# muzishen/IMAGDressing

Hardware: AMD Instinct MI355X
Metric: 512x512 50-step images/sec (whole node) (higher is better)
Workload: dtype bf16

## Files before the change

imagdressing_amd/_lib.py:

```python
from __future__ import annotations

import ctypes as C
import os

_HERE = os.path.dirname(os.path.abspath(__file__))
LIB_PATH = os.environ.get("IMD_LIB_PATH") or os.path.join(_HERE, "libimagdressing_hip.so")

ABI_VERSION = 9

u16p = C.POINTER(C.c_uint16)
f32p = C.POINTER(C.c_float)


class _Sized(C.Structure):

    def __init__(self, *args, **kw):
        super().__init__(*args, **kw)
        self.struct_bytes = C.sizeof(self)


class HeadsDest(C.Structure):
    _fields_ = [("ptr", C.c_void_p), ("kind", C.c_int), ("DP", C.c_int), ("L", C.c_int), ("scale", C.c_float)]


class ConvGemmParams(_Sized):
    _fields_ = [("struct_bytes", C.c_uint32), 
        ("x", C.c_void_p), ("w", C.c_void_p), ("out", C.c_void_p),
        ("M", C.c_int), ("N", C.c_int), ("K", C.c_int),
        ("Cin", C.c_int), ("taps", C.c_int), ("Hin", C.c_int), ("Win", C.c_int), ("Hout", C.c_int),
        ("Wout", C.c_int), ("stride", C.c_int), ("ups", C.c_int),
        ("x_pix_stride", C.c_int), ("out_ld", C.c_int), ("res_ld", C.c_int),
        ("bias", C.c_void_p), ("rowvec", C.c_void_p), ("rowvec_stride", C.c_int),
        ("res", C.c_void_p), ("out_scale", C.c_float), ("act", C.c_int), ("out_f32", C.c_int),
        ("mode", C.c_int), ("hC", C.c_int), ("hH", C.c_int), ("hD", C.c_int),
        ("hd", HeadsDest * 3), ("dtype", C.c_int), ("split_k", C.c_int), ("splitk_ws", C.c_void_p),
        ("x_bytes", C.c_uint32), ("w_bytes", C.c_uint32), ("flags", C.c_int),
        ("gn_a", C.c_void_p), ("gn_b", C.c_void_p), ("gn_silu", C.c_int), ("pad_br_only", C.c_int),
        ("splitk_counters", C.c_void_p),
        ("gn_stats_out", C.c_void_p), ("gn_stats_groups", C.c_int),
        ("gn_in_partial", C.c_void_p), ("gn_in_gamma", C.c_void_p), ("gn_in_beta", C.c_void_p),
        ("gn_in_nparts", C.c_int), ("gn_in_groups", C.c_int), ("gn_in_silu", C.c_int), ("gn_in_eps", C.c_float),
        ("gn_out_gamma", C.c_void_p), ("gn_out_beta", C.c_void_p), ("gn_out_eps", C.c_float), ("gn_out_silu", C.c_int), ("gn_out_groups", C.c_int), ("res_rows", C.c_int),
    ]


class FfParams(_Sized):
    _fields_ = [("struct_bytes", C.c_uint32), ("x", C.c_void_p), ("w1", C.c_void_p), ("b1", C.c_void_p), ("w2", C.c_void_p), ("b2", C.c_void_p), ("out", C.c_void_p),
                ("M", C.c_int), ("C", C.c_int), ("inner", C.c_int), ("x_ld", C.c_int), ("out_ld", C.c_int), ("ln", C.c_int),
                ("ln_eps", C.c_float), ("dtype", C.c_int)]


class XattnParams(_Sized):
    _fields_ = [("struct_bytes", C.c_uint32), ("x", C.c_void_p), ("w", C.c_void_p), ("bq", C.c_void_p), ("bo", C.c_void_p), ("kv", C.c_void_p),
                ("out", C.c_void_p), ("M", C.c_int), ("C", C.c_int), ("heads", C.c_int), ("L", C.c_int), ("rows_per_image", C.c_int),
                ("kv_bdiv", C.c_int), ("text_rows", C.c_int), ("x_ld", C.c_int), ("out_ld", C.c_int), ("q_scale", C.c_float),
                ("ln_eps", C.c_float), ("dtype", C.c_int)]


class AttnParams(_Sized):
    _fields_ = [("struct_bytes", C.c_uint32), 
        ("q", C.c_void_p), ("k1", C.c_void_p), ("v1t", C.c_void_p), ("k2", C.c_void_p), ("v2t", C.c_void_p),
        ("scale2", C.c_void_p), ("out", C.c_void_p),
        ("B", C.c_int), ("H", C.c_int), ("N", C.c_int), ("D", C.c_int),
        ("L1", C.c_int), ("L1P", C.c_int), ("kv1_bdiv", C.c_int),
        ("L2", C.c_int), ("L2P", C.c_int), ("kv2_bdiv", C.c_int),
        ("out_ld", C.c_int), ("dtype", C.c_int), ("flags", C.c_int), ("causal", C.c_int), ("k_pad_one", C.c_int),
        ("proj_w", C.c_void_p), ("proj_b", C.c_void_p), ("proj_res", C.c_void_p), ("proj_out", C.c_void_p),
        ("proj_res_ld", C.c_int), ("proj_out_ld", C.c_int), ("proj_counters", C.c_void_p),
        ("out_dup", C.c_void_p), ("phase2_out", C.c_void_p), ("phase2_rows", C.c_int),
    ]


class GroupNormParams(_Sized):
    _fields_ = [("struct_bytes", C.c_uint32), 
        ("x", C.c_void_p), ("y", C.c_void_p), ("gamma", C.c_void_p), ("beta", C.c_void_p), ("partial", C.c_void_p),
# ... 31 lines not shown
        ("z_n", C.c_float), ("b_img", C.c_float), ("b_noise", C.c_float), ("in_scale", C.c_float),
        ("store", C.c_int),
        ("noise", C.c_void_p), ("mask", C.c_void_p), ("z_img", C.c_void_p), ("blend_noise", C.c_void_p),
        ("coefs", C.c_void_p),
    ]


SYMBOLS = {
    "imd_abi_version": (C.c_int, []),
    "imd_last_error": (C.c_char_p, []),
    "imd_device_check": (C.c_int, [C.c_int]),
    "imd_conv_gemm": (C.c_int, [C.POINTER(ConvGemmParams), C.c_int, C.c_void_p]),
    "imd_conv_gemm_auto_cfg": (C.c_int, [C.c_int, C.c_int]),
    "imd_conv_gemm_auto_split": (C.c_int, [C.c_int, C.c_int, C.c_int, C.c_int]),
    "imd_attention": (C.c_int, [C.POINTER(AttnParams), C.c_void_p]),
    "imd_attention_dup_supported": (C.c_int, [C.c_int, C.c_int, C.c_int]),
    "imd_attention_phase_split_supported": (C.c_int, [C.c_int]),
    "imd_attention_fp8": (C.c_int, [C.POINTER(AttnParams), C.c_int, C.c_int, C.c_int, C.c_void_p]),
    "imd_attn_quantize_fp8": (C.c_int, [C.c_void_p, C.c_void_p, C.c_int, C.c_long, C.c_int, C.c_int, C.c_float, C.c_int, C.c_void_p]),
    "imd_set_tuning": (C.c_int, [C.c_int, C.c_int]),
    "imd_get_tuning": (C.c_int, [C.c_int]),
    "imd_attn_padded_dims": (C.c_int, [C.c_int, C.POINTER(C.c_int), C.POINTER(C.c_int)]),
    "imd_groupnorm": (C.c_int, [C.POINTER(GroupNormParams), C.c_void_p]),
    "imd_groupnorm_coeffs": (C.c_int, [C.POINTER(GroupNormParams), C.c_void_p, C.c_void_p, C.c_void_p]),
    "imd_conv_patch_supported": (C.c_int, [C.POINTER(ConvGemmParams)]),
    "imd_conv_patch2_supported": (C.c_int, [C.POINTER(ConvGemmParams)]),
    "imd_conv_patch3_supported": (C.c_int, [C.POINTER(ConvGemmParams)]),
    "imd_conv_patch4_supported": (C.c_int, [C.POINTER(ConvGemmParams)]),
    "imd_conv_img_supported": (C.c_int, [C.POINTER(ConvGemmParams)]),
    "imd_conv_patch_stats_parts": (C.c_int, [C.POINTER(ConvGemmParams)]),
    "imd_conv_gemm_stats_parts": (C.c_int, [C.POINTER(ConvGemmParams), C.c_int]),
    "imd_conv_gemm_gn_out_supported": (C.c_int, [C.POINTER(ConvGemmParams)]),
    "imd_row_linear_gn_in_supported": (C.c_int, [C.POINTER(ConvGemmParams), C.c_int]),
    "imd_gemm_dma_supported": (C.c_int, [C.POINTER(ConvGemmParams)]),
    "imd_row_linear": (C.c_int, [C.POINTER(ConvGemmParams), C.c_int, C.c_float, C.c_void_p]),
    "imd_row_linear_supported": (C.c_int, [C.POINTER(ConvGemmParams)]),
    "imd_ff_geglu": (C.c_int, [C.POINTER(FfParams), C.c_void_p]),
    "imd_text_xattn320": (C.c_int, [C.POINTER(XattnParams), C.c_void_p]),
    "imd_text_xattn320_supported": (C.c_int, [C.POINTER(XattnParams)]),
    "imd_conv_ups_phase": (C.c_int, [C.POINTER(ConvGemmParams), C.c_void_p]),
    "imd_conv_ups_phase_supported": (C.c_int, [C.POINTER(ConvGemmParams)]),
    "imd_groupnorm_workspace_floats": (C.c_int, [C.c_int, C.c_int, C.c_int, C.c_int]),
    "imd_layernorm": (C.c_int, [C.POINTER(LayerNormParams), C.c_void_p]),
    "imd_softmax_rows": (C.c_int, [C.c_void_p, C.c_int, C.c_void_p, C.c_int, C.c_int, C.c_int, C.c_int, C.c_void_p]),
    "imd_ddim_cfg_step": (C.c_int, [C.POINTER(DdimParams), C.c_void_p]),
    "imd_ddim_cfg_step_rows": (C.c_int, [C.POINTER(DdimParams), C.c_void_p, C.c_void_p]),
    "imd_sampler_step": (C.c_int, [C.POINTER(SamplerParams), C.c_void_p]),
    "imd_timestep_embedding": (C.c_int, [C.c_void_p, C.c_void_p, C.c_int, C.c_int, C.c_void_p]),
    "imd_add": (C.c_int, [C.c_void_p, C.c_int, C.c_void_p, C.c_int, C.c_void_p, C.c_int, C.c_long, C.c_int, C.c_float, C.c_int, C.c_void_p]),
    "imd_embed_tokens": (C.c_int, [C.c_void_p, C.c_int, C.c_void_p, C.c_int, C.c_void_p, C.c_void_p, C.c_long, C.c_int, C.c_int, C.c_void_p]),
    "imd_vit_assemble": (C.c_int, [C.c_void_p, C.c_void_p, C.c_void_p, C.c_void_p, C.c_int, C.c_int, C.c_int, C.c_int, C.c_void_p]),
    "imd_lincomb": (C.c_int, [C.POINTER(C.c_void_p), C.POINTER(C.c_float), C.c_int, C.c_void_p, C.c_long, C.c_void_p]),
    "imd_copy2d": (C.c_int, [C.c_void_p, C.c_int, C.c_void_p, C.c_int, C.c_long, C.c_int, C.c_void_p]),
    "imd_concat2": (C.c_int, [C.c_void_p, C.c_int, C.c_void_p, C.c_int, C.c_void_p, C.c_void_p, C.c_long, C.c_long, C.c_int, C.c_void_p]),
    "imd_concat2_gn_stats": (C.c_int, [C.c_void_p, C.c_int, C.c_void_p, C.c_int, C.c_void_p, C.c_void_p, C.c_int, C.c_int, C.c_int, C.c_int,
                                       C.c_void_p, C.c_int, C.c_void_p]),
    "imd_groupnorm_parts": (C.c_int, [C.c_int, C.c_int, C.c_int]),
    "imd_f32_to_16": (C.c_int, [C.c_void_p, C.c_void_p, C.c_long, C.c_int, C.c_void_p]),
}

_lib = None


class ImdError(RuntimeError):
    pass

# ... 22 lines not shown
```

imagdressing_amd/adapter/attention_processor.py:

```python
from __future__ import annotations

import math
from typing import Dict, Optional, Tuple

import torch
import torch.nn as nn

from .. import ops

bf16 = torch.bfloat16
LOG2E = math.log2(math.e)


class LoRALinearLayer(nn.Module):

    def __init__(self, in_features, out_features, rank=4, network_alpha=None):
        super().__init__()
        self.down = nn.Linear(in_features, rank, bias=False)
        self.up = nn.Linear(rank, out_features, bias=False)
        self.network_alpha = network_alpha
        self.rank = rank
        nn.init.normal_(self.down.weight, std=1 / rank)
        nn.init.zeros_(self.up.weight)

# ... 34 lines not shown
_16BIT = (torch.bfloat16, torch.float16)


def _compute_dtype(attn, hidden_states: torch.Tensor, attention_mask=None):
    if attention_mask is not None:
        raise NotImplementedError("attention_mask is always None on the IMAGDressing path (SURVEY appendix 3); masks are not implemented")
    if getattr(attn, "spatial_norm", None) is not None or getattr(attn, "group_norm", None) is not None \
            or getattr(attn, "norm_cross", None):
        raise NotImplementedError("attn.spatial_norm / group_norm / norm_cross are None for every SD1.5 attention layer; "
                                  "modules that set them are not supported by the fused processors")
    wd = attn.to_q.weight.dtype
    if wd in _16BIT:
        return wd
    return hidden_states.dtype if hidden_states.dtype in _16BIT else torch.float16


def _layer_weights(attn, which: str, dtype, device) -> torch.Tensor:
    mods = [attn.to_out[0] if n == "to_out" else getattr(attn, n) for n in _W_PARTS[which]]
    srcs = [m.bias if which == "bo" else m.weight for m in mods]
    if srcs[0] is None:
        return None
    want = torch.float32 if which == "bo" else dtype
    if len(srcs) == 1 and srcs[0].dtype == want and srcs[0].device == device and srcs[0].is_contiguous():
        return srcs[0].detach()
    cache = attn.__dict__.setdefault("_imd_wcache", {})
    key = (_version_key(*srcs), want, str(device))
    ent = cache.get(which)
    if ent is None or ent[0] != key or not all(a is b for a, b in zip(ent[1], srcs)):
        t = torch.cat([t.detach().to(device=device, dtype=want) for t in srcs], 0).contiguous()
        ent = cache[which] = (key, tuple(srcs), t)
    return ent[2]


def _ln_folded_q(attn, gamma: torch.Tensor, beta: torch.Tensor, dtype, device, which: str = "q"):
    mods = [getattr(attn, n) for n in _W_PARTS[which]]
    srcs = tuple(m.weight for m in mods) + (gamma, beta)
    cache = attn.__dict__.setdefault("_imd_wcache", {})
    key = (_version_key(*srcs), dtype, str(device))
    ent = cache.get(which + "_ln")
    if ent is None or ent[0] != key or not all(a is b for a, b in zip(ent[1], srcs)):
        w = torch.cat([m.weight.detach().to(device=device, dtype=dtype) for m in mods], 0)
        ent = cache[which + "_ln"] = (key, srcs, ops.fold_layernorm_affine(w, None, gamma.to(device), beta.to(device)))
    return ent[2]


def _qkv_ln_ok(x: torch.Tensor) -> bool:
    return x.shape[-1] == 320 and x.shape[1] % 128 == 0 and ops.FUSED_LN


FUSED_LN_CHANNELS = (320, 640, 1280)


def _as_tokens(hidden_states: torch.Tensor, dtype):
    shape4 = None
    if hidden_states.dim() == 4:
        b, c, h, w = hidden_states.shape
        shape4 = (b, c, h, w)
        hidden_states = hidden_states.view(b, c, h * w).transpose(1, 2)
    if not hidden_states.is_cuda:
        from .._lib import ImdError
        raise ImdError("imagdressing_amd processors run on MI355X only: hidden_states is on " + str(hidden_states.device))
    return hidden_states.to(dtype).contiguous(), shape4


def _restore(out, shape4, like):
    if shape4 is not None:
        b, c, h, w = shape4
        out = out.transpose(-1, -2).reshape(b, c, h, w)
    return out


def _project_kv(tokens: torch.Tensor, wkv: torch.Tensor, heads: int):
    Bk, Lk, Kd = tokens.shape
    Cc = wkv.shape[0] // 2
    D = Cc // heads
    dpk, dpv = ops.attn_padded_dims(D)
    LP = ops.pad64(Lk)
    k = ops.k_buffer((Bk, heads, Lk, dpk), D, wkv.dtype, tokens.device)
    vt = torch.zeros(Bk, heads, dpv, LP, dtype=wkv.dtype, device=tokens.device)
    ops.conv_gemm(tokens.view(Bk * Lk, Kd), wkv, M=Bk * Lk, N=2 * Cc, Cin=Kd, Hin=Lk, Win=1, Hout=Lk, Wout=1,
                  heads=dict(C=Cc, H=heads, D=D, dests=[(k, 0, dpk, Lk, 1.0), (vt, 1, dpv, LP, 1.0)]))
    return k, vt, Lk, LP


_FP8_KV: Dict[int, tuple] = {}
ops._clear_hooks.append(_FP8_KV.clear)


def _fp8_kv(kv, cache: bool):
    k, vt = kv[0], kv[1]
    e = ops.FP8_EXPS
    if cache:
        hit = _FP8_KV.get(id(k))
        if hit is not None and hit[0] is k and hit[1] == (e["q"], e["k"], e["v"]):
            return hit[2], hit[3]
    k8 = ops.quantize_fp8_rows(k, e["k"], pad_val=float(2 ** (e["q"] + e["k"])))
    v8 = ops.quantize_fp8_vt(vt, e["v"])
    if cache:
        if len(_FP8_KV) > 64:
            _FP8_KV.clear()
        _FP8_KV[id(k)] = (k, (e["q"], e["k"], e["v"]), k8, v8)
    return k8, v8


def _fused_attention(x: torch.Tensor, heads: int, *, wq_or_qkv: torch.Tensor, self_attn: bool,
                     kv1=None, kv1_bdiv: int = 1, kv2=None, kv2_bdiv: int = 1, scale2: Optional[torch.Tensor] = None,
                     wo: torch.Tensor, bo: Optional[torch.Tensor], residual: Optional[torch.Tensor],
                     q_ln: Optional[tuple] = None, pair_half: bool = False, phase2_rows: int = 0) -> torch.Tensor:
    B, N, Cc = x.shape
    D = Cc // heads
    dpk, dpv = ops.attn_padded_dims(D)
    dev, dt = x.device, x.dtype
    qscale = D ** -0.5 * LOG2E
    if (ops.FUSED_XATTN and not self_attn and q_ln is not None and kv1 is not None and kv2 is None and not pair_half
            and ops.text_xattn_supported(Cc, heads, N, kv1[2]) and not ops.ATTN_FP8 and not ops.FUSED_OUT_PROJ
            and residual is not None and residual.data_ptr() == x.data_ptr() and residual.shape == x.shape
            and residual.dtype == dt and residual.is_contiguous()):
        return ops.text_xattn(x, ops.pack_text_xattn(q_ln[0], q_ln[1], wo, bo), ops.pack_text_kv(kv1[0], kv1[1], kv1[2]),
                              Lk=kv1[2], kv_bdiv=kv1_bdiv, ln_eps=q_ln[2], q_scale=qscale)
    q = ops.workspace("attn_q", (B, heads, N, dpk), dt, dev)
    x2 = x.view(B * N, Cc)
    if self_attn:
        LP = ops.pad64(N)
        k = ops.k_buffer((B, heads, N, dpk), D, dt, dev, tag="attn_k")
        vt = ops.workspace("attn_vt", (B, heads, dpv, LP), dt, dev)
        dests = dict(C=Cc, H=heads, D=D, dests=[(q, 0, dpk, N, qscale), (k, 0, dpk, N, 1.0), (vt, 1, dpv, LP, 1.0)])
        if q_ln is not None:
            ops.conv_gemm(x2, q_ln[0], M=B * N, N=3 * Cc, Cin=Cc, Hin=N, Win=1, Hout=N, Wout=1, bias=q_ln[1], ln_eps=q_ln[2], heads=dests)
        else:
            ops.conv_gemm(x2, wq_or_qkv, M=B * N, N=3 * Cc, Cin=Cc, Hin=N, Win=1, Hout=N, Wout=1, heads=dests)
        kv1, kv1_bdiv = (k, vt, N, LP), 1
    elif q_ln is not None:
        ops.conv_gemm(x2, q_ln[0], M=B * N, N=Cc, Cin=Cc, Hin=N, Win=1, Hout=N, Wout=1, bias=q_ln[1], ln_eps=q_ln[2],
                      heads=dict(C=Cc, H=heads, D=D, dests=[(q, 0, dpk, N, qscale)]))
    else:
        ops.conv_gemm(x2, wq_or_qkv, M=B * N, N=Cc, Cin=Cc, Hin=N, Win=1, Hout=N, Wout=1,
                      heads=dict(C=Cc, H=heads, D=D, dests=[(q, 0, dpk, N, qscale)]))
    o = torch.empty(B, N, Cc, dtype=dt, device=dev)
    if ops.ATTN_FP8 and D == 40:
        e = ops.FP8_EXPS
        q8 = ops.quantize_fp8_rows(q, e["q"])
        k18, v18 = _fp8_kv(kv1, cache=not self_attn)
        kw = {}
        if kv2 is not None and scale2 is not None:
            k28, v28 = _fp8_kv(kv2, cache=True)
            kw = dict(k2=k28, v2t=v28, L2=kv2[2], L2P=kv2[3], kv2_bdiv=kv2_bdiv, scale2=scale2)
        ops.attention_fp8(q8, k18, v18, o, B=B, H=heads, N=N, L1=kv1[2], L1P=kv1[3], kv1_bdiv=kv1_bdiv, **kw)
        res2 = None if residual is None else residual.view(B * N, Cc)
        return ops.linear(o.view(B * N, Cc), wo, bo, res=res2).view(B, N, Cc)
    kw = {}
    if kv2 is not None and scale2 is not None:
        kw = dict(k2=kv2[0], v2t=kv2[1], L2=kv2[2], L2P=kv2[3], kv2_bdiv=kv2_bdiv, scale2=scale2)
    if ops.FUSED_OUT_PROJ and ops.attention_proj_supported(heads, N, D):
        out = torch.empty(B, N, Cc, dtype=dt, device=dev)
        return ops.attention(q, kv1[0], kv1[1], o, B=B, H=heads, N=N, D=D, L1=kv1[2], L1P=kv1[3], kv1_bdiv=kv1_bdiv, k_pad_one=True,
                             proj=(wo, bo, residual, out), **kw)
    if pair_half:
        o = torch.empty(2 * B, N, Cc, dtype=dt, device=dev)
        ops.attention(q, kv1[0], kv1[1], o[:B], B=B, H=heads, N=N, D=D, L1=kv1[2], L1P=kv1[3], kv1_bdiv=kv1_bdiv, k_pad_one=True,
                      out_dup=o[B:], **kw)
        res2 = None if residual is None else residual.reshape(-1, Cc)
        return ops.linear(o.view(2 * B * N, Cc), wo, bo, res=res2).view(2 * B, N, Cc)
    ops.attention(q, kv1[0], kv1[1], o, B=B, H=heads, N=N, D=D, L1=kv1[2], L1P=kv1[3], kv1_bdiv=kv1_bdiv, k_pad_one=True, phase2_rows=phase2_rows if kw else 0, **kw)
    res2 = None if residual is None else residual.view(B * N, Cc)
    return ops.linear(o.view(B * N, Cc), wo, bo, res=res2).view(B, N, Cc)


class _FusedBase:
    fused_residual = True

    @staticmethod
    def _ehs_bdiv(B: int, ehs: torch.Tensor) -> int:
        Be = ehs.shape[0]
        if B % Be:
            raise ValueError(f"encoder_hidden_states batch {Be} does not divide hidden_states batch {B}")
        return B // Be

    @staticmethod
    def _finish(attn, out, residual_given, like, shape4, ln_fused=False):
        if getattr(attn, "residual_connection", False) and not residual_given:
            if ln_fused:
                raise NotImplementedError("attn.residual_connection together with the engine's fused LayerNorm (imd_layernorm)")
            out = ops.add(out, _as_tokens(like, out.dtype)[0])
        if getattr(attn, "rescale_output_factor", 1.0) != 1.0:
            raise NotImplementedError("rescale_output_factor != 1 is not used by SD1.5")
        out = _restore(out, shape4, like)
        return out if out.dtype == like.dtype else out.to(like.dtype)


class AttnProcessor2_0(_FusedBase):

    fused_layernorm = True

    def __init__(self, cache_entries: int = 256):
        self._text = _TensorCache(capacity=cache_entries)

    def __call__(self, attn, hidden_states, encoder_hidden_states=None, attention_mask=None, temb=None, scale=1.0,
                 imd_residual=None, imd_layernorm=None, **kwargs):
        dt = _compute_dtype(attn, hidden_states, attention_mask)
        x, shape4 = _as_tokens(hidden_states, dt)
        dev = x.device
        wo, bo = _layer_weights(attn, "o", dt, dev), _layer_weights(attn, "bo", dt, dev)
        q_ln = None
        if imd_layernorm is not None:
            g, be, eps = imd_layernorm
            if encoder_hidden_states is not None and x.shape[-1] in FUSED_LN_CHANNELS:
                q_ln = _ln_folded_q(attn, g, be, dt, dev) + (eps,)
            elif encoder_hidden_states is None and _qkv_ln_ok(x):
                q_ln = _ln_folded_q(attn, g, be, dt, dev, "qkv") + (eps,)
            else:
                x = ops.layer_norm(x, g, be, eps)
        if encoder_hidden_states is None:
            out = _fused_attention(x, attn.heads, wq_or_qkv=_layer_weights(attn, "qkv", dt, dev), self_attn=True, wo=wo, bo=bo,
                                   residual=imd_residual, q_ln=q_ln)
        else:
            srcs = (encoder_hidden_states, attn.to_k.weight, attn.to_v.weight)
            kv = self._text.get(srcs, extra=(dt,))
            if kv is None:
                e = encoder_hidden_states.to(device=dev, dtype=dt).contiguous()
                kv = self._text.put(srcs, _project_kv(e, _layer_weights(attn, "kv", dt, dev), attn.heads), extra=(dt,))
            out = _fused_attention(x, attn.heads, wq_or_qkv=_layer_weights(attn, "q", dt, dev), self_attn=False, kv1=kv,
                                   kv1_bdiv=self._ehs_bdiv(x.shape[0], encoder_hidden_states), wo=wo, bo=bo,
                                   residual=imd_residual, q_ln=q_ln)
        return self._finish(attn, out, imd_residual is not None, hidden_states, shape4, ln_fused=imd_layernorm is not None)


class CacheAttnProcessor2_0(AttnProcessor2_0):
    fused_layernorm = False

    def __init__(self):
        super().__init__()
        self.cache = {}

    def __call__(self, attn, hidden_states, encoder_hidden_states=None, attention_mask=None, temb=None, scale=1.0,
                 **kwargs):
        self.cache["hidden_states"] = hidden_states
        return super().__call__(attn, hidden_states, encoder_hidden_states=encoder_hidden_states, **kwargs)


class _RefMixin:

    def _init_ref(self, name, hidden_size, cross_attention_dim, scale):
        self.name = name
        self.hidden_size = hidden_size
        self.cross_attention_dim = cross_attention_dim
        self.to_k_ref = nn.Linear(cross_attention_dim or hidden_size, hidden_size, bias=False)
        self.to_v_ref = nn.Linear(cross_attention_dim or hidden_size, hidden_size, bias=False)
        self.scale = scale
        self._wref = _TensorCache()
        self._garment = _TensorCache()
        self._scale2 = _TensorCache()
        self._scale2_plain: Dict = {}

    def _garment_kv(self, ref: torch.Tensor, heads: int, device, dtype):
        wsrc = (self.to_k_ref.weight, self.to_v_ref.weight)
        kv = self._garment.get((ref,) + wsrc, extra=(dtype,))
        if kv is None:
            w = self._wref.get(wsrc, extra=(dtype,))
            if w is None:
                w = self._wref.put(wsrc, torch.cat([t.detach().to(device=device, dtype=dtype) for t in wsrc], 0).contiguous(),
                                   extra=(dtype,))
            r = ref.detach().to(device=device, dtype=dtype).contiguous()
            if r.dim() != 3:
                raise ValueError(f"sa_hidden_states[{self.name!r}] must be [Bg, M, C], got {tuple(ref.shape)}")
            kv = self._garment.put((ref,) + wsrc, _project_kv(r, w, heads), extra=(dtype,))
        return kv

    def _garment_bdiv(self, B: int, ref: torch.Tensor) -> int:
        Bg = ref.shape[0]
        if Bg < 1 or B % Bg:
            raise ValueError(f"sa_hidden_states[{self.name!r}] has batch {Bg}, which does not divide hidden_states batch {B}")
        return B // Bg

    def _branch_weights(self, B: int, mask: Optional[torch.Tensor], device) -> torch.Tensor:
        s = float(self.scale)
        if mask is None:
            t = self._scale2_plain.get((B, s, str(device)))
            if t is None:
                t = torch.full((B,), s, dtype=torch.float32, device=device)
                self._scale2_plain = {(B, s, str(device)): t}
            return t
        t = self._scale2.get((mask,), extra=(s,))
        if t is None:
            t = self._scale2.put((mask,), (mask.to(device=device, dtype=torch.float32) * s).contiguous(), extra=(s,))
        return t


class RefSAttnProcessor2_0(nn.Module, _FusedBase, _RefMixin):
    fused_layernorm = True
    fused_pair_half = True

    def __init__(self, name, hidden_size, cross_attention_dim=None, scale=1.0):
        super().__init__()
        self._init_ref(name, hidden_size, cross_attention_dim, scale)

    def _weights(self, attn, dt, dev):
        return _layer_weights(attn, "qkv", dt, dev), _layer_weights(attn, "o", dt, dev), _layer_weights(attn, "bo", dt, dev)

    def __call__(self, attn, hidden_states, encoder_hidden_states=None, attention_mask=None, temb=None, scale=1.0,
                 num_images_per_prompt=1, cond_hidden_states=None, sa_hidden_states=None, sa_batch_mask=None,
                 imd_residual=None, imd_layernorm=None, imd_pair_half=False, **kwargs):
        if encoder_hidden_states is not None:
            raise NotImplementedError(f"{type(self).__name__} is a self-attention (attn1) processor")
        dt = _compute_dtype(attn, hidden_states, attention_mask)
        x, shape4 = _as_tokens(hidden_states, dt)
        wqkv, wo, bo = self._weights(attn, dt, x.device)
        q_ln = None
        if imd_layernorm is not None:
            g, be, eps = imd_layernorm
            if _qkv_ln_ok(x):
                q_ln = _ln_folded_q(attn, g, be, dt, x.device, "qkv") + (eps,)
            else:
                x = ops.layer_norm(x, g, be, eps)
        kv2 = s2 = None
        bdiv2 = 1
        if sa_hidden_states is not None:
            ref = sa_hidden_states[self.name]
            kv2 = self._garment_kv(ref, attn.heads, x.device, x.dtype)
            cond_rows = x.shape[0] // 2 if (kwargs.get("sa_pair_layout") and not imd_pair_half and x.shape[0] % 2 == 0) else x.shape[0]
            bdiv2 = self._garment_bdiv(cond_rows, ref)
            s2 = self._branch_weights(x.shape[0] * (2 if imd_pair_half else 1), sa_batch_mask, x.device)
        if imd_pair_half and (kv2 is None or imd_residual is None or shape4 is not None):
            raise ValueError("imd_pair_half needs sa_hidden_states, the block residual and token-major hidden states (engine-internal)")
        pr = x.shape[0] // 2 if (kwargs.get("sa_pair_layout") and sa_batch_mask is not None and kv2 is not None and not imd_pair_half and x.shape[0] % 2 == 0) else 0
        out = _fused_attention(x, attn.heads, wq_or_qkv=wqkv, self_attn=True, kv2=kv2, kv2_bdiv=bdiv2,
                               scale2=s2, wo=wo, bo=bo, residual=imd_residual, q_ln=q_ln, pair_half=bool(imd_pair_half), phase2_rows=pr)
        return self._finish(attn, out, imd_residual is not None, hidden_states, shape4, ln_fused=imd_layernorm is not None)


class _LoraFold:

    def _init_lora(self, hidden_size, kdim, rank, network_alpha, lora_scale):
        self.rank = rank
        self.lora_scale = lora_scale
        self.to_q_lora = LoRALinearLayer(hidden_size, hidden_size, rank, network_alpha)
        self.to_k_lora = LoRALinearLayer(kdim, hidden_size, rank, network_alpha)
        self.to_v_lora = LoRALinearLayer(kdim, hidden_size, rank, network_alpha)
        self.to_out_lora = LoRALinearLayer(hidden_size, hidden_size, rank, network_alpha)
        self._folded = _TensorCache()

    def _fold(self, attn, device, dtype):
        ls = float(self.lora_scale)
        srcs = tuple(l.weight for lo in (self.to_q_lora, self.to_k_lora, self.to_v_lora, self.to_out_lora)
                     for l in (lo.down, lo.up)) + (attn.to_q.weight, attn.to_k.weight, attn.to_v.weight, attn.to_out[0].weight)
        w = self._folded.get(srcs, extra=(ls, dtype, str(device)))
        if w is None:
            def eff(base, lora):
                base = base.detach().to(device)
                if ls == 0.0:
                    return base.to(dtype).contiguous()
                return (base.float() + ls * lora.delta().to(device)).to(dtype).contiguous()
            wq, wk, wv = eff(attn.to_q.weight, self.to_q_lora), eff(attn.to_k.weight, self.to_k_lora), eff(attn.to_v.weight, self.to_v_lora)
            wo = eff(attn.to_out[0].weight, self.to_out_lora)
            w = self._folded.put(srcs, dict(q=wq, kv=torch.cat([wk, wv], 0).contiguous(),
                                            qkv=(torch.cat([wq, wk, wv], 0).contiguous() if wk.shape[1] == wq.shape[1] else None),
                                            o=wo), extra=(ls, dtype, str(device)))
        return w


# ... 1 lines not shown

    def __init__(self, name, hidden_size, cross_attention_dim=None, scale=1.0, rank=128, network_alpha=None, lora_scale=1.0):
        super().__init__()
        self._init_ref(name, hidden_size, cross_attention_dim, scale)
        self._init_lora(hidden_size, cross_attention_dim or hidden_size, rank, network_alpha, lora_scale)

    def _weights(self, attn, dt, dev):
        w = self._fold(attn, dev, dt)
        return w["qkv"], w["o"], _layer_weights(attn, "bo", dt, dev)

    __call__ = RefSAttnProcessor2_0.__call__
    fused_pair_half = True


class LoraRefSAttnProcessor2_0(_LoraRefSBase):
    """attention_processor.py:391-511 (used by inference_IMAGdressing_ipa_controlnetpose.py:88-94)."""


class RefLoraSAttnProcessor2_0(_LoraRefSBase):
    """Same arithmetic under the name ``app.py:90`` uses (attention_processor.py:1006-1128).  As in the
    reference, ``pipe.set_scale`` does not match this class (it checks LoraRefSAttnProcessor2_0)."""


class CAttnProcessor2_0(nn.Module, _FusedBase):

    def __init__(self, name, hidden_size, cross_attention_dim=None):
        super().__init__()
        self.name = name
        self.hidden_size = hidden_size
        self.cross_attention_dim = cross_attention_dim
        self._plain = AttnProcessor2_0(cache_entries=4)

    fused_layernorm = True

    def __call__(self, attn, hidden_states, encoder_hidden_states=None, attention_mask=None, temb=None, scale=1.0,
                 cond_hidden_states=None, sa_hidden_states=None, imd_residual=None, imd_layernorm=None, **kwargs):
        return self._plain(attn, hidden_states, encoder_hidden_states=encoder_hidden_states, imd_residual=imd_residual,
                           imd_layernorm=imd_layernorm)


class _IPBase(nn.Module, _FusedBase, _LoraFold):

    def __init__(self, hidden_size, cross_attention_dim=None, rank=4, network_alpha=None, lora_scale=1.0, scale=1.0,
                 num_tokens=4):
        super().__init__()
        self.num_tokens = num_tokens
        self.hidden_size = hidden_size
        self.cross_attention_dim = cross_attention_dim
        self.scale = scale
        self._init_lora(hidden_size, cross_attention_dim or hidden_size, rank, network_alpha, lora_scale)
        self.to_k_ip = nn.Linear(cross_attention_dim or hidden_size, hidden_size, bias=False)
        self.to_v_ip = nn.Linear(cross_attention_dim or hidden_size, hidden_size, bias=False)
        self._kv = _TensorCache()
        self._wip = _TensorCache()
        self._s2: Dict = {}

    def _weights(self, attn, dt, dev):
        w = self._fold(attn, dev, dt)
        return w["q"], w["kv"], w["o"]

    def __call__(self, attn, hidden_states, encoder_hidden_states=None, attention_mask=None, scale=1.0, temb=None,
                 *args, imd_residual=None, **kwargs):
        if encoder_hidden_states is None:
            raise NotImplementedError(f"{type(self).__name__} is a cross-attention (attn2) processor")
        dt = _compute_dtype(attn, hidden_states, attention_mask)
        x, shape4 = _as_tokens(hidden_states, dt)
        wq, wkv, wo = self._weights(attn, dt, x.device)
        wsrc = (self.to_k_ip.weight, self.to_v_ip.weight)
        ls = float(getattr(self, "lora_scale", 0.0))
        ksrc = (encoder_hidden_states, attn.to_k.weight, attn.to_v.weight) + wsrc
        kvs = self._kv.get(ksrc, extra=(ls, x.dtype))
# ... 132 lines not shown
```

imagdressing_amd/csrc/capi.cpp:

```cpp
#include <atomic>
#include <mutex>
#include <stdarg.h>
#include <stdio.h>
#include <string.h>

#include "imd_kernels.h"

namespace {
thread_local char g_err[512] = "";
}

int imd_set_error(const char* fmt, ...) {
    va_list ap;
    va_start(ap, fmt);
    vsnprintf(g_err, sizeof(g_err), fmt, ap);
    va_end(ap);
    return 1;
}

int imd_check_launch(const char* what) {
    hipError_t e = hipGetLastError();
    if (e != hipSuccess) return imd_set_error("%s: launch failed: %s", what, hipGetErrorString(e));
    return 0;
}
// ... 134 lines not shown
    if (dpv) *dpv = imd_attn_dpv(D);
    return 0;
}

int imd_groupnorm(const imd_groupnorm_params* p, void* stream) {
    IMD_REQUIRE(p != nullptr, "groupnorm: null params");
    IMD_REQUIRE_SIZE(p, "groupnorm");
    IMD_REQUIRE(p->x && p->y && p->gamma && p->beta && p->partial, "groupnorm: null pointer");
    return imd_launch_groupnorm(*p, (hipStream_t)stream);
}

int imd_groupnorm_coeffs(const imd_groupnorm_params* p, float* coef_a, float* coef_b, void* stream) {
    IMD_REQUIRE(p != nullptr, "groupnorm_coeffs: null params");
    IMD_REQUIRE_SIZE(p, "groupnorm_coeffs");
    IMD_REQUIRE(p->x && p->gamma && p->beta && p->partial && coef_a && coef_b, "groupnorm_coeffs: null pointer");
    return imd_launch_groupnorm_coeffs(*p, coef_a, coef_b, (hipStream_t)stream);
}

static bool sized(const imd_conv_gemm_params* p) { return p && p->struct_bytes == sizeof(*p); }
static int query(const imd_conv_gemm_params* p, bool (*pred)(const imd_conv_gemm_params&)) {
    if (!sized(p)) return 0;
    imd_conv_gemm_params q = *p;
    if (!imd_conv_gemm_fill_extents(q)) return 0;
    return pred(q) ? 1 : 0;
}
int imd_conv_patch_supported(const imd_conv_gemm_params* p) { return query(p, static_cast<bool (*)(const imd_conv_gemm_params&)>(imd_conv_patch_supported)); }
int imd_conv_patch2_supported(const imd_conv_gemm_params* p) { return query(p, static_cast<bool (*)(const imd_conv_gemm_params&)>(imd_conv_patch2_supported)); }
int imd_conv_patch3_supported(const imd_conv_gemm_params* p) { return query(p, static_cast<bool (*)(const imd_conv_gemm_params&)>(imd_conv_patch3_supported)); }
int imd_conv_patch4_supported(const imd_conv_gemm_params* p) { return query(p, static_cast<bool (*)(const imd_conv_gemm_params&)>(imd_conv_patch4_supported)); }
int imd_conv_img_supported(const imd_conv_gemm_params* p) { return query(p, static_cast<bool (*)(const imd_conv_gemm_params&)>(imd_conv_img_supported)); }
int imd_conv_patch_stats_parts(const imd_conv_gemm_params* p) { return sized(p) ? imd_conv_patch_stats_parts_of(*p) : 0; }
int imd_conv_gemm_stats_parts(const imd_conv_gemm_params* p, int cfg) { return sized(p) ? imd_conv_gemm_stats_parts_of(*p, cfg) : 0; }
int imd_row_linear_gn_in_supported(const imd_conv_gemm_params* p, int cfg) { return (sized(p) && p->gn_in_partial != nullptr && imd_row_linear_gn_in_supported_of(*p, cfg)) ? 1 : 0; }
int imd_conv_gemm_gn_out_supported(const imd_conv_gemm_params* p) { return (sized(p) && imd_conv_gemm_gn_out_supported_of(*p, -1)) ? 1 : 0; }
int imd_gemm_dma_supported(const imd_conv_gemm_params* p) { return query(p, static_cast<bool (*)(const imd_conv_gemm_params&)>(imd_gemm_dma_supported)); }

int imd_row_linear_supported(const imd_conv_gemm_params* p) { return (sized(p) && (imd_row_linear_supported(*p) || imd_row_linear_k640_supported(*p) || imd_row_linear_k1280_supported(*p) || imd_row_qkv_supported(*p))) ? 1 : 0; }

int imd_row_linear(const imd_conv_gemm_params* p, int ln, float ln_eps, void* stream) {
    IMD_REQUIRE(p != nullptr, "row_linear: null params");
    IMD_REQUIRE_SIZE(p, "row_linear");
    IMD_REQUIRE(p->x && p->w, "row_linear: null input/weight pointer");
    IMD_REQUIRE(p->mode == IMD_OUT_HEADS || p->out != nullptr, "row_linear: null output pointer");
    IMD_REQUIRE(p->Hout > 0 && p->Wout > 0 && p->M > 0 && p->M % (p->Hout * p->Wout) == 0, "row_linear: bad geometry");
    if (p->mode == IMD_OUT_HEADS) {
        IMD_REQUIRE(p->hC > 0 && p->hH > 0 && p->hD > 0 && p->hC == p->hH * p->hD && p->N % p->hC == 0 && p->N / p->hC <= 3 && p->hD % 8 == 0,
                    "row_linear: bad head split C=%d H=%d D=%d", p->hC, p->hH, p->hD);
        IMD_REQUIRE(!p->out_f32, "row_linear: head-split output excludes fp32 output");
    }
    IMD_REQUIRE(!ln || ln_eps > 0.f, "row_linear: LayerNorm needs eps > 0");
    if (p->K == 320 && p->N == 960 && p->mode == IMD_OUT_HEADS) {
        IMD_REQUIRE(p->gn_in_partial == nullptr, "row_linear: the fused q / k / v projection has no GroupNorm prologue (gn_in_*)");
        return imd_launch_row_qkv(*p, ln, ln_eps, (hipStream_t)stream);
    }
    if (p->K == 640) return imd_launch_row_linear_k640(*p, ln, ln_eps, (hipStream_t)stream);
    if (p->K == 1280) return imd_launch_row_linear_k1280(*p, ln, ln_eps, (hipStream_t)stream);
    return imd_launch_row_linear(*p, ln, ln_eps, (hipStream_t)stream);
}

int imd_ff_geglu(const imd_ff_params* p, void* stream) {
    IMD_REQUIRE(p != nullptr, "ff_geglu: null params");
    IMD_REQUIRE_SIZE(p, "ff_geglu");
    IMD_REQUIRE(p->x && p->w1 && p->b1 && p->w2 && p->b2 && p->out, "ff_geglu: null pointer");
    IMD_REQUIRE(!p->ln || p->ln_eps > 0.f, "ff_geglu: LayerNorm needs eps > 0");
    return imd_launch_ff_geglu(*p, (hipStream_t)stream);
}

int imd_text_xattn320_supported(const imd_xattn_params* p) {
    return (p && p->struct_bytes == sizeof(*p) && imd_text_xattn320_supported_of(*p)) ? 1 : 0;
}

int imd_text_xattn320(const imd_xattn_params* p, void* stream) {
    IMD_REQUIRE(p != nullptr, "text_xattn320: null params");
    IMD_REQUIRE_SIZE(p, "text_xattn320");
    IMD_REQUIRE(p->x && p->w && p->bq && p->bo && p->kv && p->out, "text_xattn320: null pointer");
    return imd_launch_text_xattn320(*p, (hipStream_t)stream);
}

int imd_conv_ups_phase_supported(const imd_conv_gemm_params* p) { return (sized(p) && imd_conv_ups_phase_supported_of(*p)) ? 1 : 0; }

int imd_conv_ups_phase(const imd_conv_gemm_params* p, void* stream) {
    IMD_REQUIRE(p != nullptr, "conv_ups_phase: null params");
    IMD_REQUIRE_SIZE(p, "conv_ups_phase");
    IMD_REQUIRE(p->x && p->w && p->out, "conv_ups_phase: null input / weight / output pointer");
    return imd_launch_conv_ups_phase(*p, (hipStream_t)stream);
}

int imd_layernorm(const imd_layernorm_params* p, void* stream) {
    IMD_REQUIRE(p != nullptr, "layernorm: null params");
    IMD_REQUIRE_SIZE(p, "layernorm");
    IMD_REQUIRE(p->x && p->y && p->gamma && p->beta, "layernorm: null pointer");
    return imd_launch_layernorm(*p, (hipStream_t)stream);
}

int imd_embed_tokens(const uint16_t* table, int vocab, const uint16_t* pos, int T, const int64_t* ids, uint16_t* out, long rows, int C,
                     int dtype, void* stream) {
    IMD_REQUIRE(table && pos && ids && out, "embed_tokens: null pointer");
    return imd_launch_embed_tokens(table, vocab, pos, T, ids, out, rows, C, dtype, (hipStream_t)stream);
}

int imd_vit_assemble(const uint16_t* patches, const uint16_t* cls, const uint16_t* pos, uint16_t* out, int B, int P, int C, int dtype,
                     void* stream) {
    IMD_REQUIRE(patches && cls && pos && out, "vit_assemble: null pointer");
    return imd_launch_vit_assemble(patches, cls, pos, out, B, P, C, dtype, (hipStream_t)stream);
}

int imd_lincomb(const float* const* xs, const float* coefs, int n, float* out, long numel, void* stream) {
    IMD_REQUIRE(xs && coefs && out, "lincomb: null pointer");
    return imd_launch_lincomb(xs, coefs, n, out, numel, (hipStream_t)stream);
}

int imd_softmax_rows(const float* s, int s_ld, uint16_t* p, int p_ld, int rows, int cols, int dtype, void* stream) {
    IMD_REQUIRE(s && p, "softmax_rows: null pointer");
    return imd_launch_softmax_rows(s, s_ld, p, p_ld, rows, cols, dtype, (hipStream_t)stream);
}

int imd_ddim_cfg_step(const imd_ddim_params* p, void* stream) {
// ... 57 lines not shown
```

imagdressing_amd/csrc/conv_gemm.hip:

```cpp
#include "gemm_common.h"

namespace {

template <int BM, int BN, int BK, int WAVES_M> struct TileCfg {
    static constexpr int STRIDE = BK * 2 + 16;
    static constexpr int MAIN = 2 * (BM + BN) * STRIDE;
    static constexpr int CLD = BN + 4;
    static constexpr int EROWS = BM / WAVES_M;
    static constexpr int EPI = EROWS * CLD * 4;
    static constexpr int LDS = MAIN > EPI ? MAIN : EPI;
};

template <bool F16, int BM, int BN, int BK, int WAVES_M, int WAVES_N, int DEPTH>
__global__ __launch_bounds__(WAVES_M * WAVES_N * 64, (WAVES_M * WAVES_N == 4) ? 2 : 1) void conv_gemm_kernel(const ConvGemmParams p) {
    constexpr int NT = WAVES_M * WAVES_N * 64;
    using E = El<F16>;
    using T = TileCfg<BM, BN, BK, WAVES_M>;
    constexpr int TM = BM / WAVES_M / 32;
    constexpr int TN = BN / WAVES_N / 32;
    constexpr int STRIDE = T::STRIDE;
    constexpr int VPR = BK / 8;
    constexpr int RSTEP = NT / VPR;
    constexpr int A_VECS = BM / RSTEP;
    constexpr int W_VECS = BN / RSTEP;
// ... 568 lines not shown
    ConvGemmParams p = p_in;
    if (p.split_k < 1) p.split_k = 1;
    if (cfg < 0) cfg = imd_conv_gemm_choose_cfg(p.M, p.N);
    const TileConfig* t = tile_config(cfg);
    if (p.split_k > 1) {
        if (t != nullptr && t->finish_always) p.splitk_counters = nullptr;
        return splitk_stats_parts_of(p);
    }
    switch (t != nullptr ? t->stats : ST_NONE) {
        case ST_PATCH3_W4: return imd_conv_patch3_stats_parts_of(p, 4);
        case ST_PATCH3_W8: return imd_conv_patch3_stats_parts_of(p, 8);
        case ST_PATCH: return imd_conv_patch_stats_parts_of(p);
        case ST_TILE: {
            const int HW = p.Hout * p.Wout, G = p.gn_stats_groups;
            if (p.out_f32 || p.mode != OUT_ROWMAJOR || p.act == ACT_GEGLU || G <= 0 || G > 64 || p.N % G || (p.N / G) < 8 || (p.N % 4) || HW <= 0 || HW % t->bm || p.M % HW) return 0;
            return (HW / t->bm) * ((p.N + t->bn - 1) / t->bn);
        }
        default: return 0;
    }
}

bool imd_row_linear_gn_in_supported_of(const ConvGemmParams& p, int cfg) {
    if (p.gn_in_partial == nullptr) return true;
    ConvGemmParams q = p;
    q.split_k = 1;
    switch (cfg) {
        case 12: return imd_row_linear_supported(q) && gn_in_ok(q, 320, 128);
        case 13: return imd_row_linear_k640_supported(q) && gn_in_ok(q, 640, 128);
        case 14: return imd_row_linear_k1280_supported(q) && gn_in_ok(q, 1280, 64);
        default: return false;
    }
}

bool imd_conv_gemm_gn_out_supported_of(const ConvGemmParams& p_in, int cfg) {
    ConvGemmParams p = p_in;
    (void)cfg;
    p.splitk_counters = nullptr;
    return splitk_gn_out_supported(p);
}

int imd_conv_gemm_choose_cfg(int M, int N) {
    const long b128 = (long)((M + 127) / 128) * ((N + 127) / 128);
    if (b128 < 96) return 2;
    if (N <= 64) return 1;
    if (b128 >= 700) return 4;
    return 0;
}

int imd_conv_gemm_choose_split(int M, int N, int K, int cfg) {
    int bm = 128, bn = 128;
    tile_dims(cfg, &bm, &bn);
    const long blocks = (long)((M + bm - 1) / bm) * ((N + bn - 1) / bn);
    const int ktiles = (K + 63) / 64;
    if (blocks >= 200 || ktiles < 32) return 1;
    long s = (448 + blocks - 1) / blocks;
    if (s > ktiles / 16) s = ktiles / 16;
    if (s > 8) s = 8;
    return s < 1 ? 1 : (int)s;
}

bool imd_conv_gemm_fill_extents(ConvGemmParams& p) {
    if (p.Hout <= 0 || p.Wout <= 0 || p.M <= 0) return false;
    const size_t npix = (size_t)(p.M / (p.Hout * p.Wout)) * p.Hin * p.Win;
    if (npix == 0) return false;
    const size_t xb = ((npix - 1) * (size_t)p.x_pix_stride + p.Cin) * 2, wb = (size_t)p.N * p.K * 2;
    if (xb >= 0xffffffffull || wb >= 0xffffffffull) return false;
// ... 32 lines not shown
    }
#ifdef IMD_ABLATIONS
    p.flags |= gf & 224;
#endif
    if (p.split_k <= 1 || (t != nullptr && t->finish_always)) p.splitk_counters = nullptr;
    if (p.gn_stats_out != nullptr && imd_conv_gemm_stats_parts_of(p, cfg) == 0)
        return imd_set_error("conv_gemm: gn_stats_out needs tile config 5 / 22 / 23 / 29 or a register-staged tile (0..4, 7) with H W %% its rows == 0, without K slices, or any K-sliced launch with a separate finish; a row-major 16-bit "
                             "output and 1 <= groups <= 64 with N %% groups == 0 and N / groups >= 8 (got cfg=%d split_k=%d groups=%d N=%d); ask "
                             "imd_conv_gemm_stats_parts() first", cfg, p.split_k, p.gn_stats_groups, p.N);
    if (p.gn_out_gamma != nullptr && !imd_conv_gemm_gn_out_supported_of(p, cfg))
        return imd_set_error("conv_gemm: gn_out_* needs K slices with a separate finish launch, a row-major 16-bit output without residual / activation / scale / "
                             "gn_stats_out, 4 | N / groups and H W N / groups <= %d (got cfg=%d split_k=%d groups=%d N=%d); ask imd_conv_gemm_gn_out_supported() first",
                             4 * FG_THREADS * FG_MAXU, cfg, p.split_k, p.gn_out_groups, p.N);
    if (p.gn_out_gamma != nullptr) p.splitk_counters = nullptr;
    if (p.splitk_counters != nullptr) {
        int bm = 128, bn = 128;
        tile_dims(cfg, &bm, &bn);
        const long tiles = (t != nullptr && t->stats == ST_PATCH) ? (long)(p.M / (p.Hout * p.Wout)) * ((p.Hout + 7) / 8) * ((p.Wout + 15) / 16) * ((p.N + 127) / 128)
                                                                  : (long)((p.M + bm - 1) / bm) * ((p.N + bn - 1) / bn);
        if (tiles > IMD_SPLITK_COUNTERS || (size_t)p.M * p.N * 4 >= 0x80000000ull) p.splitk_counters = nullptr;
    }
    if (p.split_k > 1) {
        if (p.mode == OUT_HEADS || p.act == ACT_GEGLU) return imd_set_error("conv_gemm: split-K supports row-major epilogues only");
        if (!p.splitk_ws) return imd_set_error("conv_gemm: split_k = %d needs a workspace", p.split_k);
    }
    if (p.dtype != IMD_DTYPE_BF16 && p.dtype != IMD_DTYPE_F16) return imd_set_error("conv_gemm: unknown dtype %d", p.dtype);
    if ((p.gn_a != nullptr) != (p.gn_b != nullptr)) return imd_set_error("conv_gemm: gn_a and gn_b must be given together");
    if (p.gn_a != nullptr && cfg != 5) return imd_set_error("conv_gemm: the fused GroupNorm prologue needs tile config 5 (got %d)", cfg);
    if (p.res_rows != 0 && cfg != 12)
        return imd_set_error("conv_gemm: a periodic residual (res_rows = %d) exists in the K = 320 row-resident projection only (tile config 12, got %d)", p.res_rows, cfg);
    if (p.gn_in_partial != nullptr && !imd_row_linear_gn_in_supported_of(p, cfg))
        return imd_set_error("conv_gemm: gn_in_* (GroupNorm of the input rows) exists in the row-resident projections only (tile configs 12 / 13 / 14 with H W a multiple of "
                             "their row block; got cfg=%d K=%d HW=%d): ask imd_row_linear_gn_in_supported() first", cfg, p.K, p.Hout * p.Wout);
    if (t == nullptr) return imd_set_error("conv_gemm: unknown tile config %d", cfg);
    if (t->taps != 0 && t->taps != p.taps) return imd_set_error("conv_gemm: tile config %d does not take taps = %d", cfg, p.taps);
    if (t->slices_only && p.split_k <= 1) return imd_set_error("conv_gemm: tile config %d writes K-slice slabs only (split_k >= 2)", cfg);
    const int rc = t->launch(p, s);
    if (rc || p.split_k <= 1 || p.splitk_counters != nullptr) return rc;
    return launch_splitk_finish(p, s, t->finish);
}
```

imagdressing_amd/csrc/gemm_common.h:

```cpp
#pragma once
#include "common.h"
#include "imd_kernels.h"

namespace {

typedef __attribute__((__vector_size__(4 * sizeof(uint32_t)))) uint32_t v4u;

__device__ __forceinline__ uint4 buf_load16(const __amdgpu_buffer_rsrc_t& rs, uint32_t byte_off) {
    const v4u v = __builtin_amdgcn_raw_buffer_load_b128(rs, (int)byte_off, 0, 0);
    return make_uint4(v[0], v[1], v[2], v[3]);
}
__device__ __forceinline__ uint2 buf_load8(const __amdgpu_buffer_rsrc_t& rs, uint32_t byte_off) {
    typedef __attribute__((__vector_size__(2 * sizeof(uint32_t)))) uint32_t v2u;
    const v2u v = __builtin_amdgcn_raw_buffer_load_b64(rs, (int)byte_off, 0, 0);
    return make_uint2(v[0], v[1]);
}
__device__ __forceinline__ uint4 buf_load16_nl1(const __amdgpu_buffer_rsrc_t& rs, uint32_t byte_off) {
    const v4u v = __builtin_amdgcn_raw_buffer_load_b128(rs, (int)byte_off, 0, 16);
    return make_uint4(v[0], v[1], v[2], v[3]);
}

constexpr uint32_t OOB = 0xffffffffu;

__device__ __forceinline__ void xcd_tile_order(int flags, int m_tiles, int n_tiles, int& tile_m, int& tile_n) {
// ... 92 lines not shown
            const int g = c / cpg;
            const float ga = r.gam[i] * s_rstd[g];
            s_a[c] = ga;
            s_sh[c] = r.bet[i] - s_mean[g] * ga;
        }
    }
    __syncthreads();
    a = s_a; sh = s_sh;
}

template <bool F16>
__device__ __forceinline__ uint4 gn_in_apply8(const uint4& raw, const float* a, const float* sh, int k0, bool silu) {
    const float4 a0 = *reinterpret_cast<const float4*>(a + k0), a1 = *reinterpret_cast<const float4*>(a + k0 + 4);
    const float4 s0 = *reinterpret_cast<const float4*>(sh + k0), s1 = *reinterpret_cast<const float4*>(sh + k0 + 4);
    const float av[8] = {a0.x, a0.y, a0.z, a0.w, a1.x, a1.y, a1.z, a1.w}, sv[8] = {s0.x, s0.y, s0.z, s0.w, s1.x, s1.y, s1.z, s1.w};
    float f[8];
    unpack8<F16>(raw, f);
#pragma unroll
    for (int e = 0; e < 8; ++e) {
        float y = f[e] * av[e] + sv[e];
        if (silu) y = silu_f(y);
        f[e] = y;
    }
    return pack8<F16>(f);
}

inline bool gn_in_ok(const ConvGemmParams& p, int K, int rows) {
    if (p.gn_in_partial == nullptr) return true;
    const int HW = p.Hout * p.Wout;
    return p.mode == OUT_ROWMAJOR && p.res == nullptr && p.gn_in_gamma != nullptr && p.gn_in_beta != nullptr && p.gn_in_groups > 0 && p.gn_in_groups <= 64 && (K % p.gn_in_groups) == 0 &&
           p.gn_in_nparts > 0 && p.gn_in_nparts <= 4096 && HW > 0 && (HW % rows) == 0 && (p.M % HW) == 0 && p.K == K;
}

__device__ __forceinline__ void load_col_addends(const ConvGemmParams& p, int bi, int n, int nv, float4& a0, float4& a1) {
    a0 = make_float4(0, 0, 0, 0); a1 = a0;
    const bool full = nv == 8;
    if (p.bias) {
        a0 = *reinterpret_cast<const float4*>(p.bias + n);
        if (full) a1 = *reinterpret_cast<const float4*>(p.bias + n + 4);
    }
    if (p.rowvec && bi >= 0) {
        const float* rv = p.rowvec + (size_t)bi * p.rowvec_stride + n;
        const float4 r0 = *reinterpret_cast<const float4*>(rv);
        a0.x += r0.x; a0.y += r0.y; a0.z += r0.z; a0.w += r0.w;
        if (full) { const float4 r1 = *reinterpret_cast<const float4*>(rv + 4); a1.x += r1.x; a1.y += r1.y; a1.z += r1.z; a1.w += r1.w; }
    }
}

template <bool F16>
__device__ __forceinline__ void epilogue8(const ConvGemmParams& p, float* v, int m, int n, int nv, int HWo, bool use_pre = false,
                                          float4 pre0 = float4{0, 0, 0, 0}, float4 pre1 = float4{0, 0, 0, 0}, bool use_rpre = false,
                                          uint4 rpre = uint4{0, 0, 0, 0}, uint4* pk_out = nullptr) {
    using E = El<F16>;
    const int bi = m / HWo;
    float4 b0 = make_float4(0, 0, 0, 0), b1 = b0, r0 = b0, r1 = b0;
    uint4 rr = make_uint4(0, 0, 0, 0);
    const bool full = nv == 8;
    if (use_pre) { b0 = pre0; b1 = pre1; }
    else load_col_addends(p, bi, n, nv, b0, b1);
    if (p.res) {
        if (use_rpre) rr = rpre;
        else {
            const bf16_t* rp = p.res + (size_t)m * p.res_ld + n;
            if (full) rr = *reinterpret_cast<const uint4*>(rp);
            else { const uint2 t = *reinterpret_cast<const uint2*>(rp); rr.x = t.x; rr.y = t.y; }
        }
    }
    v[0] += b0.x + r0.x; v[1] += b0.y + r0.y; v[2] += b0.z + r0.z; v[3] += b0.w + r0.w;
    v[4] += b1.x + r1.x; v[5] += b1.y + r1.y; v[6] += b1.z + r1.z; v[7] += b1.w + r1.w;
    if (p.out_scale != 1.0f) {
#pragma unroll
        for (int e = 0; e < 8; ++e) v[e] *= p.out_scale;
    }
    if (p.res) {
        float f[8];
        unpack8<F16>(rr, f);
#pragma unroll
        for (int e = 0; e < 8; ++e) v[e] += f[e];
    }
    if (p.act == ACT_SILU) {
#pragma unroll
        for (int e = 0; e < 8; ++e) v[e] = silu_f(v[e]);
    } else if (p.act == ACT_GELU) {
#pragma unroll
        for (int e = 0; e < 8; ++e) v[e] = gelu_erf_f(v[e]);
    } else if (p.act == ACT_QUICK_GELU) {
#pragma unroll
// ... 91 lines not shown
```

imagdressing_amd/csrc/gemm_dma.hip:

```cpp
#include "gemm_common.h"
#include "lds_dma.h"

namespace {

constexpr int GD_BM = 256, GD_BN = 256, GD_BK = 64;
constexpr int GD_ROWB = GD_BK * 2;
constexpr int GD_A = GD_BM * GD_ROWB, GD_W = GD_BN * GD_ROWB, GD_STAGE = GD_A + GD_W;
constexpr int GD_LDS = 2 * GD_STAGE;
constexpr int GD_CLD = GD_BN + 4, GD_EROWS = 64;

template <bool F16>
__global__ __launch_bounds__(512, 1) void gemm_dma_kernel(const ConvGemmParams p) {
    using E = El<F16>;
    extern __shared__ __attribute__((aligned(16))) char smem[];
    const int tid = threadIdx.x;
    const int lane = tid & 63;
    const int wave = __builtin_amdgcn_readfirstlane(tid >> 6);
    const int hi = lane >> 5, col = lane & 31;
    const int wm0 = (wave >> 1) * 64, wn0 = (wave & 1) * 128;

    const int n_tiles = (p.N + GD_BN - 1) / GD_BN;
    int tile_m, tile_n;
    xcd_tile_order(p.flags, (p.M + GD_BM - 1) / GD_BM, n_tiles, tile_m, tile_n);
    const int m0 = tile_m * GD_BM, n0 = tile_n * GD_BN;
    const int nk = p.K / GD_BK;

    const v4i_t ds_x = raw_rsrc(p.x, p.x_bytes), ds_w = raw_rsrc(p.w, p.w_bytes);
    uint32_t soff[8];
#pragma unroll
    for (int j = 0; j < 8; ++j) {
        const int id = j * 8 + wave;
        const bool isw = j >= 4;
        const int q = (id & 31) * 64 + lane;
        const int row = q >> 3, pos = q & 7;
        const int pc = pos ^ ((row >> 1) & 7);
        if (isw) soff[j] = (n0 + row < p.N) ? (uint32_t)(((size_t)(n0 + row) * p.K + pc * 8) * 2) : OOB;
        else soff[j] = (m0 + row < p.M) ? (uint32_t)(((size_t)(m0 + row) * p.x_pix_stride + pc * 8) * 2) : OOB;
    }
    const uint32_t lds0 = (uint32_t)(uintptr_t)smem;
    auto stage = [&](int kt) {
        const uint32_t base = lds0 + (uint32_t)((kt & 1) * GD_STAGE);
#pragma unroll
        for (int j = 0; j < 8; ++j) {
            const int id = j * 8 + wave;
// ... 45 lines not shown
    float4 col_pre0 = make_float4(0, 0, 0, 0), col_pre1 = col_pre0;
    bool use_col_pre = false;
    if (!colmajor && (p.bias || p.rowvec)) {
        const int bi_lo = m0 / HWo, bi_hi = (min(m0 + GD_BM, p.M) - 1) / HWo;
        const int n = n0 + (tid % CPR) * 8;
        if ((p.rowvec == nullptr || bi_lo == bi_hi) && n < p.N) {
            load_col_addends(p, p.rowvec ? bi_lo : -1, n, (n + 8 <= p.N) ? 8 : 4, col_pre0, col_pre1);
            use_col_pre = true;
        }
    }
#pragma unroll 1
    for (int wr = 0; wr < 4; ++wr) {
        if ((wave >> 1) == wr) {
#pragma unroll
            for (int b = 0; b < 2; ++b)
#pragma unroll
                for (int a = 0; a < 4; ++a)
#pragma unroll
                    for (int j = 0; j < 4; ++j) {
                        float* dst = Cs + (b * 32 + col) * GD_CLD + wn0 + a * 32 + 8 * j + 4 * hi;
                        *reinterpret_cast<float4*>(dst) = make_float4(acc[a][b][4 * j], acc[a][b][4 * j + 1], acc[a][b][4 * j + 2], acc[a][b][4 * j + 3]);
                    }
        }
        __syncthreads();
        for (int c = tid; c < CHUNKS; c += 512) {
            int row, cc;
            if (colmajor) { cc = (c / GD_EROWS) * 8; row = c - (c / GD_EROWS) * GD_EROWS; }
            else { row = c / CPR; cc = (c - row * CPR) * 8; }
            const int m = m0 + wr * GD_EROWS + row, n = n0 + cc;
            if (m >= p.M || n >= p.N) continue;
            const float4 v0 = *reinterpret_cast<const float4*>(Cs + row * GD_CLD + cc);
            const float4 v1 = *reinterpret_cast<const float4*>(Cs + row * GD_CLD + cc + 4);
            float v[8] = {v0.x, v0.y, v0.z, v0.w, v1.x, v1.y, v1.z, v1.w};
            epilogue8<F16>(p, v, m, n, (n + 8 <= p.N) ? 8 : 4, HWo, use_col_pre, col_pre0, col_pre1);
        }
        if (wr + 1 < 4) __syncthreads();
    }
}

constexpr int G1_BM = 128, G1_BN = 128, G1_BK = 32;
constexpr int G1_STAGE = (G1_BM + G1_BN) * G1_BK * 2;
constexpr int G1_CLD = G1_BN + 4, G1_EROWS = 64;
static_assert(3 * G1_STAGE >= G1_EROWS * G1_CLD * 4, "epilogue tile must fit");

template <bool F16, bool GATHER, int G1_NST, int BK = 32>
__global__ __launch_bounds__(256, (G1_NST * (G1_BM + G1_BN) * BK * 2 <= 49152) ? 3 : (G1_NST * (G1_BM + G1_BN) * BK * 2 <= 65536) ? 2 : 1)
void gemm_dma128_kernel(const ConvGemmParams p) {
    using E = El<F16>;
    constexpr int ROWB = BK * 2, LPR = ROWB / 16;
    constexpr int STAGE = (G1_BM + G1_BN) * ROWB;
    constexpr int PPW = G1_BM * ROWB / 1024 / 4;
    constexpr int NP = 2 * PPW;
    constexpr int G1_KEEP = (G1_NST - 2) * NP;
    extern __shared__ __attribute__((aligned(16))) char smem[];
    const int tid = threadIdx.x;
    const int lane = tid & 63;
    const int wave = __builtin_amdgcn_readfirstlane(tid >> 6);
    const int hi = lane >> 5, col = lane & 31;
    const int wm0 = (wave >> 1) * 64, wn0 = (wave & 1) * 64;

    const int n_tiles = (p.N + G1_BN - 1) / G1_BN;
    int tile_m, tile_n;
    xcd_tile_order(p.flags, (p.M + G1_BM - 1) / G1_BM, n_tiles, tile_m, tile_n);
    const int m0 = tile_m * G1_BM, n0 = tile_n * G1_BN;
    const int nk_total = p.K / BK;
    const int per = (nk_total + p.split_k - 1) / p.split_k;
    const int kt0 = blockIdx.y * per;
// ... 134 lines not shown
            const float4 v1 = *reinterpret_cast<const float4*>(Cs + row * G1_CLD + cc + 4);
            if (slab) {
                slab_store8(slab, (size_t)m * p.N + n, v0, v1, n + 8 <= p.N, false);
            } else {
                float v[8] = {v0.x, v0.y, v0.z, v0.w, v1.x, v1.y, v1.z, v1.w};
                epilogue8<F16>(p, v, m, n, (n + 8 <= p.N) ? 8 : 4, HWo, use_col_pre, col_pre0, col_pre1);
            }
        }
        if (wr == 0) __syncthreads();
    }
}

}

bool imd_conv_dma_supported(const ConvGemmParams& p) {
    return p.taps == 9 && (p.stride == 1 || p.stride == 2) && (p.Cin % G1_BK) == 0 && p.K == 9 * p.Cin && p.gn_a == nullptr &&
           (p.x_pix_stride % 8) == 0 && (!p.ups || p.stride == 1);
}

template <bool GATHER, int NST, int BK = 32>
static int launch_dma128(const ConvGemmParams& p, hipStream_t s, const char* what) {
    constexpr int LDS = NST * (G1_BM + G1_BN) * BK * 2;
    static_assert(LDS >= G1_EROWS * G1_CLD * 4, "epilogue tile must fit");
    const bool h = p.dtype == IMD_DTYPE_F16;
    typedef void (*kern_t)(const ConvGemmParams);
    const kern_t kern = h ? gemm_dma128_kernel<true, GATHER, NST, BK> : gemm_dma128_kernel<false, GATHER, NST, BK>;
    if (int rc_attr = imd_lds_attr(reinterpret_cast<const void*>(kern), LDS, what)) return rc_attr;
    const long mt = (p.M + G1_BM - 1) / G1_BM, nt = (p.N + G1_BN - 1) / G1_BN;
    hipLaunchKernelGGL(kern, dim3((unsigned)(mt * nt), (unsigned)p.split_k), dim3(256), LDS, s, p);
    return imd_check_launch(what);
}

int imd_launch_gemm_dma128(const ConvGemmParams& p, int stages, int bk, hipStream_t s) {
    if (!((bk == 32 && (stages == 3 || stages == 4)) || (bk == 64 && (stages == 2 || stages == 3))))
        return imd_set_error("gemm_dma128: %d ring stages of %d-element K chunks (3 | 4 of 32, 2 | 3 of 64)", stages, bk);
    if (bk == 64) {
        if (p.taps == 9) {
            if (!imd_conv_dma_supported(p) || (p.Cin % 64)) return imd_set_error("conv_dma (128-byte rows): needs a 3x3 convolution with Cin %% 64 == 0 (got Cin=%d stride=%d)", p.Cin, p.stride);
            return stages == 2 ? launch_dma128<true, 2, 64>(p, s, "conv_dma128 (BK 64)") : launch_dma128<true, 3, 64>(p, s, "conv_dma128 (BK 64, 3 stages)");
        }
        ConvGemmParams p1 = p;
        p1.split_k = 1;
        if (!imd_gemm_dma_supported(p1)) return imd_set_error("gemm_dma128: needs a plain linear layer with K %% 64 == 0 (got K=%d taps=%d)", p.K, p.taps);
        return stages == 2 ? launch_dma128<false, 2, 64>(p, s, "gemm_dma128 (BK 64)") : launch_dma128<false, 3, 64>(p, s, "gemm_dma128 (BK 64, 3 stages)");
    }
    if (p.taps == 9) {
        if (!imd_conv_dma_supported(p)) return imd_set_error("conv_dma: needs a 3x3 convolution with Cin %% 32 == 0 (got Cin=%d stride=%d)", p.Cin, p.stride);
        return stages == 3 ? launch_dma128<true, 3>(p, s, "conv_dma128") : launch_dma128<true, 4>(p, s, "conv_dma128 (4 stages)");
    }
    ConvGemmParams p1 = p;
    p1.split_k = 1;
    if (!imd_gemm_dma_supported(p1)) return imd_set_error("gemm_dma128: needs a plain linear layer with K %% 64 == 0 (got K=%d taps=%d)", p.K, p.taps);
    return stages == 3 ? launch_dma128<false, 3>(p, s, "gemm_dma128") : launch_dma128<false, 4>(p, s, "gemm_dma128 (4 stages)");
}

bool imd_gemm_dma_supported(const ConvGemmParams& p) {
    return p.taps == 1 && p.stride == 1 && !p.ups && p.Hin == p.Hout && p.Win == p.Wout && p.Cin == p.K && (p.K % GD_BK) == 0 &&
           p.split_k <= 1 && p.gn_a == nullptr && (p.x_pix_stride % 8) == 0;
}

int imd_launch_gemm_dma(const ConvGemmParams& p, hipStream_t s) {
    if (!imd_gemm_dma_supported(p)) return imd_set_error("gemm_dma: needs a plain linear layer with K %% 64 == 0 and no K split (got K=%d taps=%d split=%d)", p.K, p.taps, p.split_k);
    const bool h = p.dtype == IMD_DTYPE_F16;
    const void* kern = h ? reinterpret_cast<const void*>(gemm_dma_kernel<true>) : reinterpret_cast<const void*>(gemm_dma_kernel<false>);
    if (int rc_attr = imd_lds_attr(kern, GD_LDS, "gemm_dma")) return rc_attr;
    const long mt = (p.M + GD_BM - 1) / GD_BM, nt = (p.N + GD_BN - 1) / GD_BN;
    if (h) hipLaunchKernelGGL(gemm_dma_kernel<true>, dim3((unsigned)(mt * nt)), dim3(512), GD_LDS, s, p);
    else hipLaunchKernelGGL(gemm_dma_kernel<false>, dim3((unsigned)(mt * nt)), dim3(512), GD_LDS, s, p);
    return imd_check_launch("gemm_dma");
}
```

imagdressing_amd/csrc/gemm_dma256.hip:

```cpp
#include "gemm_common.h"
#include "lds_dma.h"

namespace {

constexpr int G2_BK = 64, G2_ROWB = G2_BK * 2;

struct G2Item { int m0, n0, kt0, nk, slice; };

__device__ __forceinline__ void g2_decode(const ConvGemmParams& p, unsigned w, unsigned items, int m_tiles, int n_tiles, int bm, int bn, int per, int nk_total,
                                          G2Item& o) {
    if (p.flags & 12) {
        const unsigned k = w & 7u, slot = w >> 3, q8 = items >> 3, r8 = items & 7u;
        w = (k < r8 ? k * (q8 + 1) : r8 * (q8 + 1) + (k - r8) * q8) + slot;
    }
    const unsigned tiles = (unsigned)(m_tiles * n_tiles);
    const unsigned slice = w / tiles;
    const unsigned t = w - slice * tiles;
    int tm, tn;
    if (p.flags & 8) { tn = (int)(t / (unsigned)m_tiles); tm = (int)(t - (unsigned)tn * m_tiles); }
    else if ((p.flags & 4) && (p.flags & 16)) {
        constexpr unsigned GM = 8;
        const unsigned per_group = GM * (unsigned)n_tiles;
        const unsigned g = t / per_group, r = t - g * per_group;
        const unsigned rows = min(GM, (unsigned)m_tiles - g * GM);
        tn = (int)(r / rows);
        tm = (int)(g * GM + (r - (unsigned)tn * rows));
    } else { tm = (int)(t / (unsigned)n_tiles); tn = (int)(t - (unsigned)tm * n_tiles); }
    o.m0 = tm * bm; o.n0 = tn * bn; o.slice = (int)slice;
    o.kt0 = (int)slice * per;
    o.nk = min(nk_total, o.kt0 + per) - o.kt0;
}


template <int BM> struct G2Waves { static constexpr int NCW = BM / 32, NPROD = BM == 192 ? 4 : BM / 64; };
template <bool F16, int BM, int BN, int NST, bool PRE, bool RES>
__global__ __launch_bounds__((G2Waves<BM>::NCW + G2Waves<BM>::NPROD) * 64, 3) void gemm_dma256_kernel
(const ConvGemmParams p) {
    using E = El<F16>;
    constexpr int NCW = G2Waves<BM>::NCW, G2_NPROD = G2Waves<BM>::NPROD;
    constexpr int G2_A = BM * G2_ROWB;
    constexpr int APIECES = BM / 8;
    constexpr int W_BYTES = BN * G2_ROWB;
    constexpr int STAGE = G2_A + W_BYTES;
    constexpr int PIECES = APIECES + BN / 8;
    constexpr int PP = PIECES / G2_NPROD;
    static_assert(PIECES % G2_NPROD == 0 && APIECES % G2_NPROD == 0 && (NST - 1) * PP < 64, "pieces in flight per producer wave must fit the 6-bit vmcnt");
    constexpr int KEEP = (NST - 2) * PP;
    constexpr int WN = BN / 2, NA = WN / 32;
    extern __shared__ __attribute__((aligned(16))) char smem[];
    const int tid = threadIdx.x;
    const int lane = tid & 63;
    const int wave = __builtin_amdgcn_readfirstlane(tid >> 6);
    const bool producer = wave >= NCW;

    const int m_tiles = (p.M + BM - 1) / BM, n_tiles = (p.N + BN - 1) / BN;
    const unsigned items = (unsigned)(m_tiles * n_tiles) * (unsigned)p.split_k;
    const int nk_total = p.K / G2_BK;
    const int per = (nk_total + p.split_k - 1) / p.split_k;
    const int HWo = p.Hout * p.Wout;
#ifdef IMD_ABLATIONS
    const bool abl_noepi = (p.flags & 32) != 0;
    const bool abl_nowait = (p.flags & 64) != 0;
    const bool abl_nomfma = (p.flags & 128) != 0;
#else
    constexpr bool abl_noepi = false, abl_nowait = false, abl_nomfma = false;
#endif
    if (blockIdx.x >= items) return;

    if (producer) {
        const int pw = wave - NCW;
        const v4i_t ds_x = raw_rsrc(p.x, p.x_bytes), ds_w = raw_rsrc(p.w, p.w_bytes);
// ... 66 lines not shown
                for (int r = 0; r < 16; ++r) acc[a][b][r] = 0.f;
    };
    zero_acc();
    int fo[G2_BK / 16];
#pragma unroll
    for (int kk = 0; kk < G2_BK / 16; ++kk) fo[kk] = col * G2_ROWB + (((2 * kk + hi) ^ ((col >> 1) & 7)) << 4);

    __syncthreads();
    int slot = 0;
    constexpr bool pre_ok = PRE;
    for (unsigned w = blockIdx.x; w < items; w += gridDim.x) {
        G2Item ci;
        g2_decode(p, w, items, m_tiles, n_tiles, BM, BN, per, nk_total, ci);
        auto step = [&]() __attribute__((always_inline)) {
            if (!abl_nomfma) {
                const char* Xs = smem + slot * STAGE + wm0 * G2_ROWB;
                const char* Ws = smem + slot * STAGE + G2_A + wn0 * G2_ROWB;
#pragma unroll
                for (int kk = 0; kk < G2_BK / 16; ++kk) {
                    uint4 wf[NA], xf[2];
#pragma unroll
                    for (int a = 0; a < NA; ++a) wf[a] = *reinterpret_cast<const uint4*>(Ws + a * 32 * G2_ROWB + fo[kk]);
#pragma unroll
                    for (int b = 0; b < 2; ++b) xf[b] = *reinterpret_cast<const uint4*>(Xs + b * 32 * G2_ROWB + fo[kk]);
#pragma unroll
                    for (int a = 0; a < NA; ++a)
#pragma unroll
                        for (int b = 0; b < 2; ++b) acc[a][b] = E::mfma(wf[a], xf[b], acc[a][b]);
                }
            }
            slot = slot == NST - 1 ? 0 : slot + 1;
            if (!abl_nowait) __syncthreads();
        };
#pragma unroll 1
        for (int kt = 0; kt < ci.nk - 1; ++kt) step();
        float4 bn[NA][4];
        uint4 rp[NA][2], rq[NA][2];
        auto load_bias = [&]() __attribute__((always_inline)) {
#pragma unroll
            for (int a = 0; a < NA; ++a)
#pragma unroll
                for (int j = 0; j < 4; ++j) {
                    const int nb = ci.n0 + wn0 + a * 32 + 8 * j + 4 * hi;
                    bn[a][j] = (p.bias != nullptr && nb < p.N) ? *reinterpret_cast<const float4*>(p.bias + nb) : make_float4(0, 0, 0, 0);
                }
        };
        float4 bias_l = make_float4(0, 0, 0, 0);
        if (pre_ok && !abl_noepi) {
            if (!RES) load_bias();
            else if (lane < 16) {
                const int nb = ci.n0 + wn0 + 4 * lane;
                if (p.bias != nullptr && nb < p.N) bias_l = *reinterpret_cast<const float4*>(p.bias + nb);
            }
#pragma unroll
            for (int a = 0; a < NA; ++a)
#pragma unroll
                for (int t = 0; t < 2; ++t) {
                    const int n = ci.n0 + wn0 + a * 32 + 16 * t + 8 * hi;
                    const int m = ci.m0 + wm0 + col;
                    rp[a][t] = make_uint4(0, 0, 0, 0);
                    if (RES && m < p.M && n + 8 <= p.N) rp[a][t] = *reinterpret_cast<const uint4*>(p.res + (size_t)m * p.res_ld + n);
                }
        }
        step();
        if (!abl_noepi) {
            float* slab = (p.split_k > 1) ? p.splitk_ws + (size_t)ci.slice * p.M * p.N : nullptr;
            if (pre_ok) {
                float* bias_s = reinterpret_cast<float*>(smem + NST * STAGE + wave * 2048);
                if (RES && lane < 16) *reinterpret_cast<float4*>(bias_s + 4 * lane) = bias_l;
#pragma unroll
                for (int a = 0; a < NA; ++a)
#pragma unroll
                    for (int j = 0; j < 4; ++j) {
                        const float4 bj = RES ? *reinterpret_cast<const float4*>(bias_s + a * 32 + 8 * j + 4 * hi) : bn[a][j];
#pragma unroll
                        for (int b = 0; b < 2; ++b) {
                            acc[a][b][4 * j] += bj.x; acc[a][b][4 * j + 1] += bj.y; acc[a][b][4 * j + 2] += bj.z; acc[a][b][4 * j + 3] += bj.w;
                        }
                    }
            }
            if constexpr (RES) {
                uint4 pk0[NA][2];
                auto finish = [&](int a, int b, int t, const uint4& rr) __attribute__((always_inline)) {
                    float v[8];
#pragma unroll
                    for (int e = 0; e < 4; ++e) {
                        const auto r = __builtin_amdgcn_permlane32_swap(__float_as_uint(acc[a][b][8 * t + e]), __float_as_uint(acc[a][b][8 * t + 4 + e]), false, false);
                        v[e] = __uint_as_float(r[0]); v[4 + e] = __uint_as_float(r[1]);
                    }
                    uint4 pk = make_uint4(0, 0, 0, 0);
                    epilogue8<F16>(p, v, ci.m0 + wm0 + b * 32 + col, ci.n0 + wn0 + a * 32 + 16 * t + 8 * hi, 8, HWo, true, make_float4(0, 0, 0, 0), make_float4(0, 0, 0, 0), true, rr, &pk);
                    return pk;
                };
#pragma unroll
                for (int a = 0; a < NA; ++a)
#pragma unroll
                    for (int t = 0; t < 2; ++t) pk0[a][t] = finish(a, 0, t, rp[a][t]);
                const int m1 = ci.m0 + wm0 + 32 + col;
#pragma unroll
                for (int a = 0; a < NA; ++a)
#pragma unroll
// ... 74 lines not shown
                    }
                }
            } else {
#pragma unroll
            for (int b = 0; b < 2; ++b) {
                const int m = ci.m0 + wm0 + b * 32 + col;
#pragma unroll
                for (int a = 0; a < NA; ++a) {
#pragma unroll
                    for (int t = 0; t < 2; ++t) {
                        float v[8];
#pragma unroll
                        for (int e = 0; e < 4; ++e) {
                            const auto r = __builtin_amdgcn_permlane32_swap(__float_as_uint(acc[a][b][8 * t + e]), __float_as_uint(acc[a][b][8 * t + 4 + e]), false, false);
                            v[e] = __uint_as_float(r[0]); v[4 + e] = __uint_as_float(r[1]);
                        }
                        const int n = ci.n0 + wn0 + a * 32 + 16 * t + 8 * hi;
                        if (m < p.M && n < p.N) {
                            const int nv = (n + 8 <= p.N) ? 8 : 4;
                            if (slab) slab_store8(slab, (size_t)m * p.N + n, make_float4(v[0], v[1], v[2], v[3]), make_float4(v[4], v[5], v[6], v[7]), nv == 8, false);
                            else if (pre_ok) epilogue8<F16>(p, v, m, n, nv, HWo, true, make_float4(0, 0, 0, 0), make_float4(0, 0, 0, 0));
                            else epilogue8<F16>(p, v, m, n, nv, HWo);
                        }
                    }
                }
            }
            }
            }
        }
        zero_acc();
    }
}

template <int BM, int BN, int NST, bool PRE, bool RES>
int launch_dma256_v(const ConvGemmParams& p, bool persistent, hipStream_t s, const char* what) {
    constexpr int LDS = NST * (BM + BN) * G2_ROWB + (BM / 32) * 2048;
    constexpr int WG_PER_CU = BM >= 192 ? 1 : 2;
    static_assert(LDS * WG_PER_CU <= 160 * 1024, "ring + transpose areas must fit the CU's LDS");
    const bool h = p.dtype == IMD_DTYPE_F16;
    typedef void (*kern_t)(const ConvGemmParams);
    const kern_t kern = h ? gemm_dma256_kernel<true, BM, BN, NST, PRE, RES> : gemm_dma256_kernel<false, BM, BN, NST, PRE, RES>;
    if (int rc_attr = imd_lds_attr(reinterpret_cast<const void*>(kern), LDS, what)) return rc_attr;
    const int n_cu = imd_cu_count8();
    if (n_cu < 0) return imd_set_error("%s: cannot query the device", what);
    const long items = (long)((p.M + BM - 1) / BM) * ((p.N + BN - 1) / BN) * p.split_k;
    const long slots = (long)n_cu * WG_PER_CU;
    const long grid = persistent ? (items < slots ? items : slots) : items;
    hipLaunchKernelGGL(kern, dim3((unsigned)grid), dim3((G2Waves<BM>::NCW + G2Waves<BM>::NPROD) * 64), LDS, s, p);
    return imd_check_launch(what);
}

template <int BM, int BN, int NST>
int launch_dma256(const ConvGemmParams& p, bool persistent, hipStream_t s, const char* what) {
    const bool pre = p.rowvec == nullptr && p.split_k <= 1, res = p.res != nullptr;
    if (!pre || (res && (p.mode != OUT_ROWMAJOR || p.out_f32 || p.act == ACT_GEGLU || (p.N % BN) != 0 || (p.res_ld % 8) != 0 || (p.out_ld % 8) != 0)))
        return launch_dma256_v<BM, BN, NST, false, false>(p, persistent, s, what);
    return res ? launch_dma256_v<BM, BN, NST, true, true>(p, persistent, s, what) : launch_dma256_v<BM, BN, NST, true, false>(p, persistent, s, what);
}

}

int imd_launch_gemm_dma256(const ConvGemmParams& p, int form, hipStream_t s) {
    ConvGemmParams p1 = p;
    p1.split_k = 1;
    if (!imd_gemm_dma_supported(p1)) return imd_set_error("gemm_dma256: needs a plain linear layer with K %% 64 == 0 (got K=%d taps=%d)", p.K, p.taps);
    const int nk_total = p.K / G2_BK, per = (nk_total + p.split_k - 1) / p.split_k;
    if (p.split_k > 1 && (long)(p.split_k - 1) * per >= nk_total) return imd_set_error("gemm_dma256: %d K slices over %d K tiles leave a slice empty", p.split_k, nk_total);
    switch (form) {
        case 0: return launch_dma256<256, 128, 3>(p, true, s, "gemm_dma256 (256x128, persistent)");
        case 1: return launch_dma256<256, 128, 3>(p, false, s, "gemm_dma256 (256x128)");
        case 2: return launch_dma256<192, 128, 3>(p, true, s, "gemm_dma256 (192x128, persistent)");
        default: return imd_set_error("gemm_dma256: unknown form %d", form);
    }
}
```

imagdressing_amd/csrc/imd_kernels.h:

```cpp
#pragma once
#include <hip/hip_runtime.h>
#include <stdint.h>

#include "../../include/imagdressing_hip.h"

typedef uint16_t bf16_t;
typedef imd_heads_dest HeadsDest;
typedef imd_conv_gemm_params ConvGemmParams;
typedef imd_attn_params AttnParams;
typedef imd_groupnorm_params GroupNormParams;
typedef imd_layernorm_params LayerNormParams;
typedef imd_ddim_params DdimParams;
typedef imd_sampler_params SamplerParams;

enum { ACT_NONE = IMD_ACT_NONE, ACT_SILU = IMD_ACT_SILU, ACT_GEGLU = IMD_ACT_GEGLU, ACT_GELU = IMD_ACT_GELU, ACT_QUICK_GELU = IMD_ACT_QUICK_GELU };
enum { OUT_ROWMAJOR = IMD_OUT_ROWMAJOR, OUT_HEADS = IMD_OUT_HEADS };

int imd_set_error(const char* fmt, ...);
int imd_check_launch(const char* what);
int imd_lds_attr(const void* kern, int bytes, const char* what);
int imd_cu_count8();

int imd_conv_gemm_choose_cfg(int M, int N);
int imd_conv_gemm_choose_split(int M, int N, int K, int cfg);
int imd_launch_conv_gemm(const ConvGemmParams& p, int cfg, hipStream_t s);
bool imd_conv_gemm_fill_extents(ConvGemmParams& p);
bool imd_conv_patch_supported(const ConvGemmParams& p);
bool imd_conv_patch2_supported(const ConvGemmParams& p);
int imd_launch_conv_patch2(const ConvGemmParams& p, hipStream_t s);
bool imd_conv_patch3_supported(const ConvGemmParams& p);
int imd_launch_conv_patch3(const ConvGemmParams& p, hipStream_t s);
bool imd_conv_patch4_supported(const ConvGemmParams& p);
int imd_launch_conv_patch4(const ConvGemmParams& p, hipStream_t s);
int imd_conv_patch3_stats_parts_of(const ConvGemmParams& p, int nw);
bool imd_conv_patch64_supported(const ConvGemmParams& p);
int imd_launch_conv_patch64(const ConvGemmParams& p, hipStream_t s);
bool imd_conv_ups_phase_supported_of(const ConvGemmParams& p);
int imd_launch_conv_ups_phase(const ConvGemmParams& p, hipStream_t s);
bool imd_conv_img_supported(const ConvGemmParams& p);
int imd_launch_conv_img(const ConvGemmParams& p, hipStream_t s);
int imd_conv_patch_stats_parts_of(const ConvGemmParams& p);
int imd_conv_gemm_stats_parts_of(const ConvGemmParams& p, int cfg);
bool imd_conv_gemm_gn_out_supported_of(const ConvGemmParams& p, int cfg);
bool imd_row_linear_gn_in_supported_of(const ConvGemmParams& p, int cfg);
int imd_launch_conv_patch(const ConvGemmParams& p, hipStream_t s);
bool imd_row_linear_supported(const ConvGemmParams& p);
int imd_launch_row_linear(const ConvGemmParams& p, int ln, float ln_eps, hipStream_t s);
bool imd_row_linear_k640_supported(const ConvGemmParams& p);
int imd_launch_row_linear_k640(const ConvGemmParams& p, int ln, float ln_eps, hipStream_t s);
bool imd_row_linear_k1280_supported(const ConvGemmParams& p);
int imd_launch_row_linear_k1280(const ConvGemmParams& p, int ln, float ln_eps, hipStream_t s);
bool imd_row_qkv_supported(const ConvGemmParams& p);
int imd_launch_row_qkv(const ConvGemmParams& p, int ln, float ln_eps, hipStream_t s);
bool imd_gemm_dma_supported(const ConvGemmParams& p);
int imd_launch_gemm_dma(const ConvGemmParams& p, hipStream_t s);
int imd_launch_gemm_dma128(const ConvGemmParams& p, int stages, int bk, hipStream_t s);
int imd_launch_gemm_dma256(const ConvGemmParams& p, int form, hipStream_t s);
bool imd_conv_dma_supported(const ConvGemmParams& p);
int imd_launch_ff_geglu(const imd_ff_params& p, hipStream_t s);
bool imd_text_xattn320_supported_of(const imd_xattn_params& p);
int imd_launch_text_xattn320(const imd_xattn_params& p, hipStream_t s);
int imd_launch_attention(const AttnParams& p, hipStream_t s);
int imd_launch_attention_d40(const AttnParams& p, int variant, hipStream_t s);
int imd_launch_attention_fp8(const AttnParams& p, int eq, int ek, int ev, hipStream_t s);
int imd_launch_attn_quantize_fp8(const bf16_t* src, unsigned char* dst, int kind, long rows_or_groups, int LP, int exp2_scale,
                                 float pad_val, int dtype, hipStream_t s);
extern int g_attn_qw40;
extern int g_attn_xcd;
#ifdef IMD_ATTN_SWEEP
extern int g_attn_v80, g_attn_v160;
#endif
extern int g_gemm_flags;
int imd_attn_dpk(int D);
int imd_attn_dpv(int D);
int imd_launch_groupnorm(const GroupNormParams& p, hipStream_t s);
int imd_launch_groupnorm_coeffs(const GroupNormParams& p, float* ca, float* cb, hipStream_t s);
int imd_groupnorm_parts_of(int B, int HW, int C);
// ... 16 lines not shown
```

imagdressing_amd/csrc/row_linear_k1280.hip:

```cpp
#include "gemm_common.h"
#include "lds_dma.h"

namespace {

constexpr int R12_K = 1280, R12_KQ = 320;
constexpr int R12_STEPS = R12_KQ / 32;
constexpr int R12_ROWB = R12_K * 2;
constexpr int R12_CHUNK = 16 * R12_ROWB;
constexpr int R12_RING = 3;
constexpr int R12_NG = 160;
constexpr int R12_NC = R12_NG / 16;
constexpr int R12_OFF_RED = R12_RING * R12_CHUNK;
constexpr int R12_OFF_BIAS = R12_OFF_RED + 2 * 16 * 1024;
constexpr int R12_OFF_LN = R12_OFF_BIAS + R12_NG * 4;
constexpr int R12_LDS = R12_OFF_LN + 8 * 64 * 8;

template <bool F16> struct Mfma16;
template <> struct Mfma16<false> {
    static __device__ __forceinline__ f32x4 run(const uint4& a, const uint4& b, f32x4 c) {
        return __builtin_amdgcn_mfma_f32_16x16x32_bf16(__builtin_bit_cast(bf16x8, a), __builtin_bit_cast(bf16x8, b), c, 0, 0, 0);
    }
};
template <> struct Mfma16<true> {
    static __device__ __forceinline__ f32x4 run(const uint4& a, const uint4& b, f32x4 c) {
        return __builtin_amdgcn_mfma_f32_16x16x32_f16(__builtin_bit_cast(f16x8, a), __builtin_bit_cast(f16x8, b), c, 0, 0, 0);
    }
};

template <bool F16, bool LN, bool GN = false>
__global__ __launch_bounds__(512, 1) void row_linear_k1280_kernel(const ConvGemmParams p, const float ln_eps) {
    static_assert(!(LN && GN), "one prologue at a time");
    using E = El<F16>;
    extern __shared__ __attribute__((aligned(16))) char smem[];
    const int tid = threadIdx.x;
    const int lane = tid & 63;
    const int wave = __builtin_amdgcn_readfirstlane(tid >> 6);
    const int g = lane >> 4, col = lane & 15;
    const int tb = wave & 1, kq = wave >> 1;
    const int n_groups = p.N / R12_NG;
    const int xcd = blockIdx.x & 7, slot = blockIdx.x >> 3;
    const int mblk = (slot / n_groups) * 8 + xcd, grp = slot % n_groups;
    if (mblk * 64 >= p.M) return;
    const int m0 = mblk * 64 + tb * 32, n0 = grp * R12_NG;

    GnInReq<R12_K> gnreq;
    if constexpr (GN) gn_in_request<R12_K>(p, (mblk * 64) / (p.Hout * p.Wout), gnreq);
    const __amdgpu_buffer_rsrc_t rs_x = __builtin_amdgcn_make_buffer_rsrc(const_cast<bf16_t*>(p.x), 0, p.x_bytes, 0x00020000);
    uint4 xf[2][R12_STEPS];
#pragma unroll
    for (int th = 0; th < 2; ++th) {
        const int m = m0 + th * 16 + col;
        const uint32_t xoff = (uint32_t)m * (uint32_t)(p.x_pix_stride * 2) + (uint32_t)(kq * (R12_KQ * 2) + g * 16);
#pragma unroll
        for (int s = 0; s < R12_STEPS; ++s) xf[th][s] = buf_load16(rs_x, m < p.M ? xoff + s * 64 : OOB);
    }
    float bias_v = 0.f;
    if (tid < R12_NG && p.bias) bias_v = p.bias[n0 + tid];
    const bool owner = kq < 2;
    const int mo = m0 + (kq & 1) * 16 + col;
    const bool has_res = !GN && owner && p.res != nullptr;
    uint2 rres[R12_NC];
    if (has_res) {
// ... 95 lines not shown
        }
        (void)part;
#pragma unroll
        for (int th = 0; th < 2; ++th)
#pragma unroll
            for (int s = 0; s < R12_STEPS; ++s) asm volatile("" : "+v"(xf[th][s].x), "+v"(xf[th][s].y), "+v"(xf[th][s].z), "+v"(xf[th][s].w));
#pragma unroll
        for (int th = 0; th < 2; ++th) {
            const float shift = -mean[th] * rstd[th];
#pragma unroll
            for (int s = 0; s < R12_STEPS; ++s) {
                float f[8];
                unpack8<F16>(xf[th][s], f);
#pragma unroll
                for (int e = 0; e < 8; ++e) f[e] = fmaf(f[e], rstd[th], shift);
                xf[th][s] = pack8<F16>(f);
            }
        }
    }

    const int HWo = p.Hout * p.Wout;
    const bool heads = !GN && p.mode == OUT_HEADS;
    const __amdgpu_buffer_rsrc_t rs_o = __builtin_amdgcn_make_buffer_rsrc(heads ? (void*)p.hd[0].ptr : p.out, 0, 0x80000000u, 0x00020000);
    uint32_t obase = OOB;
    if (owner && mo < p.M) {
        if (heads) { const int bi = mo / HWo, tok = mo - bi * HWo; obase = (uint32_t)(((size_t)bi * p.hH * p.hd[0].L + tok) * p.hd[0].DP * 2); }
        else obase = (uint32_t)mo * (uint32_t)(p.out_ld * 2);
    }
    float4* red = reinterpret_cast<float4*>(smem + R12_OFF_RED);
    const float* bias_s = reinterpret_cast<const float*>(smem + R12_OFF_BIAS);
    const float osc = heads ? p.out_scale * p.hd[0].scale : p.out_scale;
    f32x4 own;
    own[0] = own[1] = own[2] = own[3] = 0.f;
    auto emit = [&](int c) {
        float4 t = make_float4(own[0], own[1], own[2], own[3]);
#pragma unroll
        for (int k = 0; k < 4; ++k) {
            if (k == kq) continue;
            const float4 o = red[((((c & 1) * 2 + tb) * 4 + k) * 2 + kq) * 64 + lane];
            t.x += o.x; t.y += o.y; t.z += o.z; t.w += o.w;
        }
        const int nl = 16 * c + 4 * g;
        const float4 bb = *reinterpret_cast<const float4*>(bias_s + nl);
        float v0 = (t.x + bb.x) * osc, v1 = (t.y + bb.y) * osc, v2 = (t.z + bb.z) * osc, v3 = (t.w + bb.w) * osc;
        if (has_res) {
            v0 += E::lo(rres[c].x); v1 += E::hi(rres[c].x);
            v2 += E::lo(rres[c].y); v3 += E::hi(rres[c].y);
        }
        const int n = n0 + nl;
        uint32_t off;
        if (heads) { const int h = n / p.hD, dd = n - h * p.hD; off = (uint32_t)((h * p.hd[0].L * p.hd[0].DP + dd) * 2); }
        else off = (uint32_t)(n * 2);
        typedef __attribute__((__vector_size__(2 * sizeof(uint32_t)))) uint32_t v2u;
        const v2u pk = {E::pack2(v0, v1), E::pack2(v2, v3)};
        __builtin_amdgcn_raw_buffer_store_b64(pk, rs_o, (int)(obase == OOB ? OOB : obase + off), 0, 0);
    };

    const uint32_t pb = (uint32_t)(kq * 40 + g), sw = (uint32_t)col;
    const char* wlane = smem + col * R12_ROWB;
#pragma unroll
    for (int c = 0; c <= R12_NC; ++c) {
        dma_wait();
        __syncthreads();
        if (c > 0 && owner) emit(c - 1);
        if (c + 2 < R12_NC) stage(c + 2);
        if (c < R12_NC) {
            f32x4 acc[2];
#pragma unroll
            for (int th = 0; th < 2; ++th) acc[th][0] = acc[th][1] = acc[th][2] = acc[th][3] = 0.f;
            const char* Ws = wlane + (c % R12_RING) * R12_CHUNK;
#pragma unroll
            for (int s = 0; s < R12_STEPS; ++s) {
                const uint4 wf = *reinterpret_cast<const uint4*>(Ws + (((pb + 4 * s) ^ sw) << 4));
                acc[0] = Mfma16<F16>::run(wf, xf[0][s], acc[0]);
                acc[1] = Mfma16<F16>::run(wf, xf[1][s], acc[1]);
            }
#pragma unroll
            for (int th = 0; th < 2; ++th) {
                if (th == kq) own = acc[th];
                else red[((((c & 1) * 2 + tb) * 4 + kq) * 2 + th) * 64 + lane] = make_float4(acc[th][0], acc[th][1], acc[th][2], acc[th][3]);
            }
        }
    }
}

template <bool F16, bool LN, bool GN = false>
int launch_r12(const ConvGemmParams& p, float eps, hipStream_t s) {
    auto kern = row_linear_k1280_kernel<F16, LN, GN>;
    if (int rc_attr = imd_lds_attr(reinterpret_cast<const void*>(kern), R12_LDS, "row_linear_k1280")) return rc_attr;
    const unsigned grid = (unsigned)((((p.M + 63) / 64 + 7) / 8) * 8 * (p.N / R12_NG));
    hipLaunchKernelGGL(kern, dim3(grid), dim3(512), R12_LDS, s, p, eps);
    return imd_check_launch("row_linear_k1280");
}

}

bool imd_row_linear_k1280_supported(const ConvGemmParams& p) {
    const bool direct = p.act == ACT_NONE && !p.out_f32 && p.rowvec == nullptr &&
                        (p.mode == OUT_ROWMAJOR || (p.hd[0].kind == 0 && p.hd[0].ptr != nullptr && p.N == p.hC));
    return direct && p.taps == 1 && p.K == R12_K && p.Cin == R12_K && p.stride == 1 && !p.ups && p.Hin == p.Hout && p.Win == p.Wout &&
           p.N >= R12_NG && (p.N % R12_NG) == 0 && p.split_k <= 1 && p.gn_a == nullptr && (p.x_pix_stride % 8) == 0 &&
           (p.mode != OUT_HEADS || (p.hD % 4) == 0);
}

int imd_launch_row_linear_k1280(const ConvGemmParams& p_in, int ln, float ln_eps, hipStream_t s) {
    ConvGemmParams p = p_in;
    if (p_in.res_rows != 0) return imd_set_error("row_linear_k1280: a periodic residual (res_rows) exists in the K = 320 row-resident projection only");
    if (!imd_row_linear_k1280_supported(p))
        return imd_set_error("row_linear_k1280: needs a plain linear layer with K = 1280, N a multiple of 160 and a bias / scale / residual epilogue "
                             "(got N=%d K=%d taps=%d act=%d)", p.N, p.K, p.taps, p.act);
    if (p.dtype != IMD_DTYPE_BF16 && p.dtype != IMD_DTYPE_F16) return imd_set_error("row_linear_k1280: unknown dtype %d", p.dtype);
    const size_t xb = ((size_t)(p.M - 1) * p.x_pix_stride + p.K) * 2, wb = (size_t)p.N * p.K * 2;
    const size_t ob = p.mode == OUT_HEADS ? (size_t)(p.M / (p.Hout * p.Wout)) * p.hH * p.hd[0].L * p.hd[0].DP * 2 : ((size_t)(p.M - 1) * p.out_ld + p.N) * 2;
    const size_t rb = p.res ? ((size_t)(p.M - 1) * p.res_ld + p.N) * 2 : 0;
    if (xb >= 0xffffffffull || ob >= 0x80000000ull || rb >= 0x80000000ull) return imd_set_error("row_linear_k1280: operand too large");
    p.x_bytes = (uint32_t)xb;
    p.w_bytes = (uint32_t)wb;
    p.split_k = 1;
    p.flags = 0;
    const bool h = p.dtype == IMD_DTYPE_F16;
    if (p.gn_in_partial != nullptr) {
        if (ln || !gn_in_ok(p, R12_K, 64))
            return imd_set_error("row_linear_k1280: gn_in_* needs K = 1280, K %% groups == 0, groups <= 64, H W %% 64 == 0 and no LayerNorm prologue (ask imd_row_linear_gn_in_supported())");
        return h ? launch_r12<true, false, true>(p, ln_eps, s) : launch_r12<false, false, true>(p, ln_eps, s);
    }
    if (ln) return h ? launch_r12<true, true>(p, ln_eps, s) : launch_r12<false, true>(p, ln_eps, s);
    return h ? launch_r12<true, false>(p, ln_eps, s) : launch_r12<false, false>(p, ln_eps, s);
}
```

imagdressing_amd/csrc/row_linear_k640.hip:

```cpp
#include "gemm_common.h"
#include "lds_dma.h"

namespace {

constexpr int R6_K = 640, R6_KH = 320;
constexpr int R6_STEPS = R6_KH / 16;
constexpr int R6_ROWB = R6_K * 2;
constexpr int R6_CHUNK = 32 * R6_ROWB;
constexpr int R6_RING = 3;
constexpr int R6_NG = 160;
constexpr int R6_NC = R6_NG / 32;
constexpr int R6_OFF_RED = R6_RING * R6_CHUNK;
constexpr int R6_OFF_BIAS = R6_OFF_RED + 2 * 8 * 2048;
constexpr int R6_OFF_LN = R6_OFF_BIAS + R6_NG * 4;
constexpr int R6_LDS = R6_OFF_LN + 8 * 64 * 8;

template <bool F16, bool LN, bool GN = false>
__global__ __launch_bounds__(512, 1) void row_linear_k640_kernel(const ConvGemmParams p, const float ln_eps) {
    static_assert(!(LN && GN), "one prologue at a time");
    using E = El<F16>;
    extern __shared__ __attribute__((aligned(16))) char smem[];
    const int tid = threadIdx.x;
    const int lane = tid & 63;
    const int wave = __builtin_amdgcn_readfirstlane(tid >> 6);
    const int hi = lane >> 5, col = lane & 31;
    const int tb = wave & 3, kh = wave >> 2;
    const int n_groups = p.N / R6_NG;
    const int xcd = blockIdx.x & 7, slot = blockIdx.x >> 3;
    const int mblk = (slot / n_groups) * 8 + xcd, grp = slot % n_groups;
    if (mblk * 128 >= p.M) return;
    const int m0 = mblk * 128, n0 = grp * R6_NG;
    const int m = m0 + tb * 32 + col;

    GnInReq<R6_K> gnreq;
    if constexpr (GN) gn_in_request<R6_K>(p, m0 / (p.Hout * p.Wout), gnreq);
    const __amdgpu_buffer_rsrc_t rs_x = __builtin_amdgcn_make_buffer_rsrc(const_cast<bf16_t*>(p.x), 0, p.x_bytes, 0x00020000);
    const uint32_t xoff = (uint32_t)m * (uint32_t)(p.x_pix_stride * 2) + (uint32_t)(kh * (R6_KH * 2) + hi * 16);
    uint4 xf[R6_STEPS];
#pragma unroll
    for (int s = 0; s < R6_STEPS; ++s) xf[s] = buf_load16(rs_x, m < p.M ? xoff + s * 32 : OOB);
    float bias_v = 0.f;
    if (tid < R6_NG && p.bias) bias_v = p.bias[n0 + tid];

    const v4i_t ds_w = raw_rsrc(p.w, p.w_bytes);
    uint32_t woff[5];
#pragma unroll
    for (int j = 0; j < 5; ++j) {
        const int q = (j * 8 + wave) * 64 + lane;
        const int row = q / 80, pos = q - row * 80;
        woff[j] = (uint32_t)((n0 + row) * R6_ROWB + ((pos ^ (row & 15)) << 4));
    }
    const uint32_t lds0 = (uint32_t)(uintptr_t)smem;
// ... 56 lines not shown
#pragma unroll
        for (int s = 0; s < R6_STEPS; ++s) {
            xf[s] = gn_in_apply8<F16>(xf[s], ga, gs, kh * R6_KH + 16 * s + 8 * hi, silu);
            asm volatile("" ::: "memory");
            __builtin_amdgcn_sched_barrier(0);
        }
    }

    const int HWo = p.Hout * p.Wout;
    const bool heads = !GN && p.mode == OUT_HEADS;
    const __amdgpu_buffer_rsrc_t rs_o = __builtin_amdgcn_make_buffer_rsrc(heads ? (void*)p.hd[0].ptr : p.out, 0, 0x80000000u, 0x00020000);
    const __amdgpu_buffer_rsrc_t rs_r = __builtin_amdgcn_make_buffer_rsrc(const_cast<bf16_t*>(p.res), 0, 0x80000000u, 0x00020000);
    uint32_t obase = OOB;
    if (m < p.M) {
        if (heads) { const int bi = m / HWo, tok = m - bi * HWo; obase = (uint32_t)(((size_t)bi * p.hH * p.hd[0].L + tok) * p.hd[0].DP * 2); }
        else obase = (uint32_t)m * (uint32_t)(p.out_ld * 2);
    }
    const bool has_res = !GN && p.res != nullptr;
    const uint32_t roff = (uint32_t)m * (uint32_t)(p.res_ld * 2);
    uint4 rraw[2];
    const bool wide = GN || (p.flags & 1024) != 0;
    auto load_res = [&](int c) {
        if (wide) rraw[c & 1] = buf_load16(rs_r, m < p.M ? roff + (uint32_t)((n0 + 32 * c + 16 * kh + 8 * hi) * 2) : OOB);
        else {
            const uint2 a = buf_load8(rs_r, m < p.M ? roff + (uint32_t)((n0 + 32 * c + 8 * (2 * kh) + 4 * hi) * 2) : OOB);
            const uint2 b = buf_load8(rs_r, m < p.M ? roff + (uint32_t)((n0 + 32 * c + 8 * (2 * kh + 1) + 4 * hi) * 2) : OOB);
            rraw[c & 1] = make_uint4(a.x, a.y, b.x, b.y);
        }
    };
    float4* red = reinterpret_cast<float4*>(smem + R6_OFF_RED);
    const float* bias_s = reinterpret_cast<const float*>(smem + R6_OFF_BIAS);
    const float osc = heads ? p.out_scale * p.hd[0].scale : p.out_scale;
    float own[8];
    auto emit = [&](int c) {
        typedef __attribute__((__vector_size__(2 * sizeof(uint32_t)))) uint32_t v2u;
        typedef __attribute__((__vector_size__(4 * sizeof(uint32_t)))) uint32_t v4u_t;
        v2u pk[2];
        uint2 rres[2];
        if (has_res) {
            uint4 r = rraw[c & 1];
            if (wide) {
                const auto sx = __builtin_amdgcn_permlane32_swap(r.x, r.z, false, false);
                const auto sy = __builtin_amdgcn_permlane32_swap(r.y, r.w, false, false);
                r = make_uint4(sx[0], sy[0], sx[1], sy[1]);
            }
            rres[0] = make_uint2(r.x, r.y); rres[1] = make_uint2(r.z, r.w);
        }
#pragma unroll
        for (int j = 0; j < 2; ++j) {
            const float4 o = red[((c & 1) * 8 + (wave ^ 4)) * 128 + j * 64 + lane];
            const int nl = 32 * c + 8 * (2 * kh + j) + 4 * hi;
            const float4 bb = *reinterpret_cast<const float4*>(bias_s + nl);
            float v0 = (own[4 * j] + o.x + bb.x) * osc, v1 = (own[4 * j + 1] + o.y + bb.y) * osc;
            float v2 = (own[4 * j + 2] + o.z + bb.z) * osc, v3 = (own[4 * j + 3] + o.w + bb.w) * osc;
            if (has_res) {
                v0 += E::lo(rres[j].x); v1 += E::hi(rres[j].x);
                v2 += E::lo(rres[j].y); v3 += E::hi(rres[j].y);
            }
            pk[j] = v2u{E::pack2(v0, v1), E::pack2(v2, v3)};
        }
        auto offset_of = [&](int n) -> uint32_t {
            if (heads) { const int h = n / p.hD, dd = n - h * p.hD; return (uint32_t)((h * p.hd[0].L * p.hd[0].DP + dd) * 2); }
            return (uint32_t)(n * 2);
        };
        if (wide) {
            const auto r0 = __builtin_amdgcn_permlane32_swap(pk[0][0], pk[1][0], false, false);
            const auto r1 = __builtin_amdgcn_permlane32_swap(pk[0][1], pk[1][1], false, false);
            const v4u_t w = {r0[0], r1[0], r0[1], r1[1]};
            __builtin_amdgcn_raw_buffer_store_b128(w, rs_o, (int)(obase == OOB ? OOB : obase + offset_of(n0 + 32 * c + 16 * kh + 8 * hi)), 0, 0);
        } else {
#pragma unroll
            for (int j = 0; j < 2; ++j)
                __builtin_amdgcn_raw_buffer_store_b64(pk[j], rs_o, (int)(obase == OOB ? OOB : obase + offset_of(n0 + 32 * c + 8 * (2 * kh + j) + 4 * hi)), 0, 0);
        }
    };

    const uint32_t pb = (uint32_t)(kh * 40 + hi), sw = (uint32_t)(col & 15);
    const char* wlane = smem + col * R6_ROWB;
#pragma unroll
    for (int c = 0; c <= R6_NC; ++c) {
        dma_wait();
        __syncthreads();
        if (c > 0) emit(c - 1);
        if (c + 2 < R6_NC) stage(c + 2);
        if (c < R6_NC) {
            if (has_res) load_res(c);
            f32x16 acc;
#pragma unroll
            for (int r = 0; r < 16; ++r) acc[r] = 0.f;
            const char* Ws = wlane + (c % R6_RING) * R6_CHUNK;
#pragma unroll
            for (int s = 0; s < R6_STEPS; ++s) {
                const uint4 wf = *reinterpret_cast<const uint4*>(Ws + (((pb + 2 * s) ^ sw) << 4));
                acc = E::mfma(wf, xf[s], acc);
            }
#pragma unroll
            for (int j = 0; j < 2; ++j) {
                const float4 lo = make_float4(acc[4 * j], acc[4 * j + 1], acc[4 * j + 2], acc[4 * j + 3]);
                const float4 hi4 = make_float4(acc[8 + 4 * j], acc[9 + 4 * j], acc[10 + 4 * j], acc[11 + 4 * j]);
                const float4 mine = kh ? hi4 : lo, theirs = kh ? lo : hi4;
                own[4 * j] = mine.x; own[4 * j + 1] = mine.y; own[4 * j + 2] = mine.z; own[4 * j + 3] = mine.w;
                red[((c & 1) * 8 + wave) * 128 + j * 64 + lane] = theirs;
            }
        }
    }
}

template <bool F16, bool LN, bool GN = false>
int launch_r6(const ConvGemmParams& p, float eps, hipStream_t s) {
    auto kern = row_linear_k640_kernel<F16, LN, GN>;
    if (int rc_attr = imd_lds_attr(reinterpret_cast<const void*>(kern), R6_LDS, "row_linear_k640")) return rc_attr;
    const unsigned grid = (unsigned)((((p.M + 127) / 128 + 7) / 8) * 8 * (p.N / R6_NG));
    hipLaunchKernelGGL(kern, dim3(grid), dim3(512), R6_LDS, s, p, eps);
    return imd_check_launch("row_linear_k640");
}

}

bool imd_row_linear_k640_supported(const ConvGemmParams& p) {
    const bool direct = p.act == ACT_NONE && !p.out_f32 && p.rowvec == nullptr &&
                        (p.mode == OUT_ROWMAJOR || (p.hd[0].kind == 0 && p.hd[0].ptr != nullptr && p.N == p.hC));
    return direct && p.taps == 1 && p.K == R6_K && p.Cin == R6_K && p.stride == 1 && !p.ups && p.Hin == p.Hout && p.Win == p.Wout &&
           p.N >= R6_NG && (p.N % R6_NG) == 0 && p.split_k <= 1 && p.gn_a == nullptr && (p.x_pix_stride % 8) == 0 &&
           (p.mode != OUT_HEADS || (p.hD % 4) == 0);
}

int imd_launch_row_linear_k640(const ConvGemmParams& p_in, int ln, float ln_eps, hipStream_t s) {
    ConvGemmParams p = p_in;
    if (p_in.res_rows != 0) return imd_set_error("row_linear_k640: a periodic residual (res_rows) exists in the K = 320 row-resident projection only");
    if (!imd_row_linear_k640_supported(p))
        return imd_set_error("row_linear_k640: needs a plain linear layer with K = 640, N a multiple of 160 and a bias / scale / residual epilogue "
                             "(got N=%d K=%d taps=%d act=%d)", p.N, p.K, p.taps, p.act);
    if (p.dtype != IMD_DTYPE_BF16 && p.dtype != IMD_DTYPE_F16) return imd_set_error("row_linear_k640: unknown dtype %d", p.dtype);
    const size_t xb = ((size_t)(p.M - 1) * p.x_pix_stride + p.K) * 2, wb = (size_t)p.N * p.K * 2;
    const size_t ob = p.mode == OUT_HEADS ? (size_t)(p.M / (p.Hout * p.Wout)) * p.hH * p.hd[0].L * p.hd[0].DP * 2 : ((size_t)(p.M - 1) * p.out_ld + p.N) * 2;
    const size_t rb = p.res ? ((size_t)(p.M - 1) * p.res_ld + p.N) * 2 : 0;
    if (xb >= 0xffffffffull || ob >= 0x80000000ull || rb >= 0x80000000ull) return imd_set_error("row_linear_k640: operand too large");
    p.x_bytes = (uint32_t)xb;
    p.w_bytes = (uint32_t)wb;
    p.split_k = 1;
    p.flags = (g_gemm_flags & 1024) ? 0 : 1024;
    const bool h = p.dtype == IMD_DTYPE_F16;
    if (p.gn_in_partial != nullptr) {
        if (ln || !gn_in_ok(p, R6_K, 128))
            return imd_set_error("row_linear_k640: gn_in_* needs K = 640, K %% groups == 0, groups <= 64, H W %% 128 == 0 and no LayerNorm prologue (ask imd_row_linear_gn_in_supported())");
        return h ? launch_r6<true, false, true>(p, ln_eps, s) : launch_r6<false, false, true>(p, ln_eps, s);
    }
    if (ln) return h ? launch_r6<true, true>(p, ln_eps, s) : launch_r6<false, true>(p, ln_eps, s);
    return h ? launch_r6<true, false>(p, ln_eps, s) : launch_r6<false, false>(p, ln_eps, s);
}
```

imagdressing_amd/ops.py:

```python
from __future__ import annotations

import functools
import ctypes as C
from typing import Dict, Optional, Sequence, Tuple

import torch

from . import _lib as L

ACT_NONE, ACT_SILU, ACT_GEGLU, ACT_GELU, ACT_QUICK_GELU = 0, 1, 2, 3, 4
bf16 = torch.bfloat16
f16 = torch.float16
DTYPE_CODE = {torch.bfloat16: 0, torch.float16: 1}


def _code(t: torch.Tensor, name: str = "tensor") -> int:
    try:
        return DTYPE_CODE[t.dtype]
    except KeyError:
        raise L.ImdError(f"{name}: expected a bfloat16 or float16 tensor, got {t.dtype}") from None


try:
    _raw_stream, _cur_dev = torch._C._cuda_getCurrentRawStream, torch._C._cuda_getDevice
# ... 83 lines not shown
def _count(kind: str, flops: float):
    c = FLOP_COUNTER
    if c is not None:
        c[kind] = c.get(kind, 0.0) + float(flops)


def attn_padded_dims(D: int) -> Tuple[int, int]:
    a, b = C.c_int(), C.c_int()
    L.check(L.load().imd_attn_padded_dims(D, C.byref(a), C.byref(b)))
    return a.value, b.value


def pad64(n: int) -> int:
    return (n + 63) // 64 * 64


PATCH_CONV = True
PATCH_MIN_W = 32
SPLITK_IN_KERNEL = False
FUSED_FF = True
FUSED_FF_MIN_ROWS = 24576
import os as _os
FUSED_GN_STATS = _os.environ.get("IMD_FUSED_GN_STATS", "1") != "0"
CFG_PAIR_DEDUP = _os.environ.get("IMD_CFG_PAIR_DEDUP", "1") != "0"
FUSED_GN_CONV = _os.environ.get("IMD_FUSED_GN_CONV", "0") == "1"
FUSED_GN_FINISH = _os.environ.get("IMD_FUSED_GN_FINISH", "0") == "1"
FUSED_GN_PROJ = _os.environ.get("IMD_FUSED_GN_PROJ", "1") != "0"
FUSED_CONCAT_STATS = _os.environ.get("IMD_FUSED_CONCAT_STATS", "1") != "0"
PERIODIC_RES = _os.environ.get("IMD_PERIODIC_RES", "1") != "0"
GENERIC_GN_STATS = _os.environ.get("IMD_GENERIC_GN_STATS", "0") == "1"
TEMB_TABLE = _os.environ.get("IMD_TEMB_TABLE", "1") != "0"
FUSED_GN_PROJ_CFGS = tuple(int(c) for c in _os.environ.get("IMD_FUSED_GN_PROJ_CFGS", "12,13,14").split(",") if c)
CFG_PAIR_ATTN = _os.environ.get("IMD_CFG_PAIR_ATTN", "1") != "0"
FUSED_LN = True
GEMM_TRACE = None
GEMM_EVENT_HOOK = None
_GEMM_TABLE = None
_CFG_DECISIONS: Dict[Tuple, Tuple[int, int]] = {}

TUNING_PER_CALL = 0x5A000000
ATTN_VARIANT_MAX = 13


import contextvars

_TUNING = contextvars.ContextVar("imd_tuning_scope", default=None)


class tuning_scope:

    def __init__(self, attn_variant=None, attn_xcd=None, gemm_flags=None):
        self.new = dict(attn_variant=attn_variant, attn_xcd=attn_xcd, gemm_flags=gemm_flags)

    def __enter__(self):
        merged = dict(_TUNING.get() or {})
        merged.update({k: v for k, v in self.new.items() if v is not None})
        self.token = _TUNING.set(merged if any(v is not None for v in merged.values()) else None)
        return self

    def __exit__(self, *exc):
        _TUNING.reset(self.token)
        return False


def _gemm_call_flags() -> int:
    t = _TUNING.get()
# ... 136 lines not shown
    gamma, beta, eps, silu, groups = gn_out
    if not (p.split_k > 1 and p.mode == 0 and not p.out_f32 and p.act == ACT_NONE and not p.res and out_scale == 1.0):
        return False
    p.gn_out_gamma, p.gn_out_beta = _dev(gamma, torch.float32, "gn_out gamma"), _dev(beta, torch.float32, "gn_out beta")
    p.gn_out_eps, p.gn_out_silu, p.gn_out_groups = float(eps), int(bool(silu)), int(groups)
    if lib.imd_conv_gemm_gn_out_supported(C.byref(p)):
        p.splitk_counters = None
        return True
    p.gn_out_gamma, p.gn_out_beta, p.gn_out_groups = None, None, 0
    return False


def _attach_stats(p, lib, cfg: int, split_k: int, groups: int, images: int, device):
    if not (cfg in STATS_EPILOGUE_CFGS or split_k > 1 or (GENERIC_GN_STATS and cfg in TILE_STATS_CFGS)):
        return None
    p.gn_stats_groups = groups
    nparts = lib.imd_conv_gemm_stats_parts(C.byref(p), cfg)
    if nparts <= 0:
        p.gn_stats_groups = 0
        return None
    part = torch.empty((images, nparts, groups, 2), dtype=torch.float32, device=device)
    p.gn_stats_out = part.data_ptr()
    return part, nparts, groups


def conv_gemm(
    x: torch.Tensor, w: torch.Tensor, *, M: int, N: int, Cin: int, taps: int = 1,
    Hin: int = 1, Win: int = 1, Hout: int = 1, Wout: int = 1, stride: int = 1, ups: bool = False,
    x_pix_stride: Optional[int] = None, out: Optional[torch.Tensor] = None, out_ld: Optional[int] = None,
    bias: Optional[torch.Tensor] = None, rowvec: Optional[torch.Tensor] = None, rowvec_stride: int = 0,
    rowvec_off: int = 0, res: Optional[torch.Tensor] = None, res_ld: Optional[int] = None, out_scale: float = 1.0,
    act: int = ACT_NONE, out_f32: bool = False, heads: Optional[dict] = None, cfg: int = -1, split_k: int = 0,
    gn: Optional[tuple] = None, pad_br_only: bool = False, ln_eps: Optional[float] = None, gn_stats_groups: int = 0,
    gn_out: Optional[tuple] = None, gn_in: Optional[tuple] = None,
) -> Optional[torch.Tensor]:
    ensure_device(x.device)
    K = taps * Cin
    p, out, res_rows = _marshal(x, w, M, N, K, Cin, taps, Hin, Win, Hout, Wout, stride, ups, x_pix_stride, out, out_ld, bias, rowvec, rowvec_stride, rowvec_off,
                                res, res_ld, out_scale, act, out_f32, heads, pad_br_only)
    _count("gemm_conv", 2.0 * M * N * K)
    lib = L.load()
    if gn is not None:
        p.gn_a, p.gn_b, p.gn_silu = _dev(gn[0], torch.float32, "gn_a"), _dev(gn[1], torch.float32, "gn_b"), int(gn[2])
        if cfg == -1:
            cfg = PATCH_CFG
    if ln_eps is not None:
        if res_rows:
            res = _periodic_residual(p, res, res_rows, K == 320)
        p.split_k = 1
        L.check(lib.imd_row_linear(C.byref(p), 1, float(ln_eps), _stream()))
        return out
    splittable = heads is None and act != ACT_GEGLU
    if GEMM_TRACE is not None:
        GEMM_TRACE.append(dict(M=M, N=N, K=K, Cin=Cin, taps=taps, Hin=Hin, Win=Win, Hout=Hout, Wout=Wout, stride=stride, ups=int(ups), splittable=splittable, dtype=str(x.dtype),
                               bias=bias is not None, rowvec=rowvec is not None, rowvec_stride=rowvec_stride, res=res is not None, res_rows=res_rows, act=act, out_f32=bool(out_f32),
                               heads=None if heads is None else dict(C=heads["C"], H=heads["H"], D=heads["D"],
                                                                     dests=[(t is not None, kind, DP, Ltok, scale) for t, kind, DP, Ltok, scale in heads["dests"]]),
                               gn_stats_groups=gn_stats_groups, x_pix_stride=p.x_pix_stride, out_scale=out_scale, pad_br_only=bool(pad_br_only),
                               out_ld=p.out_ld, res_ld=p.res_ld, gn=gn is not None, gn_in=gn_in is not None, gn_out=gn_out is not None))
    dkey = hit = None
    if cfg == -1 and split_k == 0 and GEMM_TRACE is None:
        hk = None if heads is None else (heads["C"], heads["H"], heads["D"], tuple((t is None, kind, DP, Ltok) for t, kind, DP, Ltok, _ in heads["dests"]))
        dkey = (M, N, K, Cin, taps, stride, int(ups), Hin, Win, Hout, Wout, p.x_pix_stride, p.res_ld, p.out_ld, act, int(out_f32), int(pad_br_only), p.dtype,
                rowvec is None, res is None, bias is None, hk, PATCH_CONV, id(_GEMM_TABLE))
        hit = _CFG_DECISIONS.get(dkey)
    cfg, split_k = hit or _choose_tile(p, lib, cfg, split_k, splittable)
    if hit is None and dkey is not None and len(_CFG_DECISIONS) < 4096:
        _CFG_DECISIONS[dkey] = (cfg, split_k)
    if res_rows:
        res = _periodic_residual(p, res, res_rows, cfg in PERIODIC_RES_CFGS)
    p.split_k = split_k
    xn = None if gn_in is None else _fuse_gn_in(p, lib, x, gn_in, cfg, M, Hout * Wout)
    if split_k > 1:
        p.splitk_ws = splitk_workspace(split_k * M * N, x.device).data_ptr()
        if SPLITK_IN_KERNEL:
            p.splitk_counters = splitk_counters(x.device).data_ptr()
    if gn_out is not None and FUSED_GN_FINISH and _fuse_gn_out(p, lib, gn_out, out_scale):
        L.check(lib.imd_conv_gemm(C.byref(p), cfg, _stream()))
        out._imd_gn_applied = True
        return out
    stats = None
    if gn_stats_groups and FUSED_GN_STATS and heads is None and not out_f32 and act != ACT_GEGLU:
        stats = _attach_stats(p, lib, cfg, split_k, gn_stats_groups, M // (Hout * Wout), x.device)
    if GEMM_EVENT_HOOK is not None:
        e0, e1 = torch.cuda.Event(enable_timing=True), torch.cuda.Event(enable_timing=True)
        e0.record()
        L.check(lib.imd_conv_gemm(C.byref(p), cfg, _stream()))
        e1.record()
        GEMM_EVENT_HOOK.setdefault((f"{M},{N},{K},{taps},{stride},{int(ups)}|{Hout}x{Wout}", cfg, split_k), []).append((e0, e1))
    else:
        L.check(lib.imd_conv_gemm(C.byref(p), cfg, _stream()))
    if stats is not None:
        out._imd_gn_stats = stats
    return out


_splitk_ws: Dict[Tuple, torch.Tensor] = {}
_splitk_cnt: Dict[Tuple, torch.Tensor] = {}


def splitk_counters(device) -> torch.Tensor:
    key = (str(device), _stream())
    t = _splitk_cnt.get(key)
    if t is None:
        t = torch.zeros(16384, dtype=torch.int32, device=device)
        _splitk_cnt[key] = t
    return t


def splitk_workspace(nfloats: int, device) -> torch.Tensor:
    key = (str(device), _stream())
    t = _splitk_ws.get(key)
    if t is None or t.numel() < nfloats:
        t = torch.empty(max(nfloats, 1 << 22), dtype=torch.float32, device=device)
        _splitk_ws[key] = t
    return t


def linear(x2d: torch.Tensor, w: torch.Tensor, bias=None, *, res=None, act=ACT_NONE, out_f32=False, out=None,
           out_ld=None, res_ld=None, cfg=-1, split_k=0, ln_eps=None) -> torch.Tensor:
    M, K = x2d.shape
    N = w.shape[0]
    return conv_gemm(x2d, w, M=M, N=N, Cin=K, bias=bias, res=res, act=act, out_f32=out_f32, out=out,
                     out_ld=out_ld, res_ld=res_ld, cfg=cfg, split_k=split_k, ln_eps=ln_eps)


def fold_layernorm_affine(w: torch.Tensor, bias: Optional[torch.Tensor], gamma: torch.Tensor, beta: torch.Tensor):
    wf = w.float()
    w2 = (wf * gamma.float()[None, :]).to(w.dtype).contiguous()
    b2 = wf @ beta.float()
    if bias is not None:
        b2 = b2 + bias.float()
    return w2, b2.contiguous()


def pack_ff_fused(w1: torch.Tensor, b1: torch.Tensor, w2: torch.Tensor, b2: torch.Tensor, gamma: Optional[torch.Tensor] = None,
                  beta: Optional[torch.Tensor] = None, dtype=None):
    dtype = dtype or w1.dtype
    inner, C = w2.shape[1], w2.shape[0]
    w1f, b1f = w1.float(), b1.float()
    if gamma is not None:
        b1f = b1f + w1f @ beta.float()
        w1f = w1f * gamma.float()[None, :]
    dev = w1.device
    i = torch.arange(32, device=dev)
    jj = (i & 7) + 8 * (i >> 4)
    gate = ((i >> 3) & 1).bool()
    blk = torch.arange(inner // 16, device=dev)
    src = 16 * blk[:, None] + jj[None, :] + torch.where(gate, inner, 0)[None, :]
    w1p = w1f[src.reshape(-1)].to(dtype).contiguous()
    b1p = b1f[src.reshape(-1)].contiguous()
    ks = torch.arange(16, device=dev)
    jk = torch.where(ks < 4, ks, torch.where(ks < 8, ks + 4, torch.where(ks < 12, ks - 4, ks)))
    cols = (16 * torch.arange(inner // 16, device=dev)[:, None] + jk[None, :]).reshape(inner // 32, 32)
    w2p = w2.float()[:, cols].permute(1, 0, 2).to(dtype).contiguous()
    return dict(w1=w1p, b1=b1p, w2=w2p, b2=b2.float().contiguous(), ln=gamma is not None, C=C, inner=inner)


def ff_geglu_fused(x2d: torch.Tensor, packed: dict, ln_eps: float = 1e-5, out: Optional[torch.Tensor] = None) -> torch.Tensor:
    ensure_device(x2d.device)
    M, C_ = x2d.shape
    dt = x2d.dtype
    if out is None:
        out = torch.empty((M, C_), dtype=dt, device=x2d.device)
    p = L.FfParams()
    p.x, p.w1, p.b1 = _dev(x2d, dt, "x"), _dev(packed["w1"], dt, "w1"), _dev(packed["b1"], torch.float32, "b1")
# ... 106 lines not shown
    _XATTN_KV[id(k)] = (k, vt, Lk, img)
    return img


def text_xattn_supported(C_: int, heads: int, N: int, Lk: int) -> bool:
    return C_ == XATTN_C and heads == XATTN_HEADS and N % 128 == 0 and 1 <= Lk <= XATTN_LMAX


def text_xattn(x: torch.Tensor, packed: dict, kv_img: torch.Tensor, *, Lk: int, kv_bdiv: int = 1, ln_eps: float = 1e-5,
               q_scale: Optional[float] = None, out: Optional[torch.Tensor] = None) -> torch.Tensor:
    ensure_device(x.device)
    B, N, C_ = x.shape
    dt = x.dtype
    if out is None:
        out = torch.empty((B, N, C_), dtype=dt, device=x.device)
    if kv_img.dim() != 3 or tuple(kv_img.shape[1:]) != (4, XATTN_CHUNK):
        raise L.ImdError(f"text_xattn: kv_img must be [Bt, 4, {XATTN_CHUNK}], got {tuple(kv_img.shape)}")
    p = L.XattnParams()
    p.x, p.w, p.out = _dev(x, dt, "x"), _dev(packed["w"], dt, "w"), _dev(out, dt, "out")
    p.bq, p.bo, p.kv = _dev(packed["bq"], torch.float32, "bq"), _dev(packed["bo"], torch.float32, "bo"), _dev(kv_img, dt, "kv_img")
    p.M, p.C, p.heads, p.L = B * N, C_, XATTN_HEADS, int(Lk)
    p.rows_per_image, p.kv_bdiv, p.text_rows = N, int(kv_bdiv), kv_img.shape[0]
    p.x_ld = p.out_ld = C_
    p.q_scale = float(XATTN_D ** -0.5 * 1.4426950408889634 if q_scale is None else q_scale)
    p.ln_eps, p.dtype = float(ln_eps), _code(x, "x")
    _count("gemm_conv", 2 * 2.0 * B * N * C_ * C_)
    _count("attention", 4.0 * XATTN_HEADS * N * XATTN_D * B * Lk)
    L.check(L.load().imd_text_xattn320(C.byref(p), _stream()))
    return out


def conv2d_nhwc(x: torch.Tensor, w: torch.Tensor, bias=None, *, taps=9, stride=1, ups=False, rowvec=None,
                rowvec_stride=0, rowvec_off=0, res=None, out_scale=1.0, act=ACT_NONE, out_f32=False, cfg=-1, split_k=0, gn=None,
                pad_br_only=False, gn_stats_groups=0, gn_out=None, gn_in=None) -> torch.Tensor:
    B, H, W, Cin = x.shape
    Cout = w.shape[0]
    Hl, Wl = (2 * H, 2 * W) if ups else (H, W)
    Ho, Wo = ((Hl + stride - 1) // stride, (Wl + stride - 1) // stride)
    M = B * Ho * Wo
    out = conv_gemm(x, w, M=M, N=Cout, Cin=Cin, taps=taps, Hin=H, Win=W, Hout=Ho, Wout=Wo, stride=stride, ups=ups,
                    bias=bias, rowvec=rowvec, rowvec_stride=rowvec_stride, rowvec_off=rowvec_off, res=res, out_scale=out_scale, act=act,
                    out_f32=out_f32, cfg=cfg, split_k=split_k, gn=gn, pad_br_only=pad_br_only, gn_stats_groups=gn_stats_groups, gn_out=gn_out, gn_in=gn_in)
    r = out.view(B, Ho, Wo, -1)
    if getattr(out, "_imd_gn_applied", False):
        r._imd_gn_applied = True
    st = getattr(out, "_imd_gn_stats", None)
    if st is not None:
        r._imd_gn_stats = st
    return r


UPS_PHASE = _os.environ.get("IMD_UPS_PHASE", "1") != "0"
UPS_PHASE_TAPS = (((0,), (1, 2)), ((0, 1), (2,)))
UPS_PHASE_CFG = "ups_phase"
_UPS_W: Dict[Tuple, tuple] = {}
_UPS_OK: Dict[Tuple, bool] = {}
_clear_hooks.append(_UPS_W.clear)
_clear_hooks.append(_UPS_OK.clear)


def _pack_upsample_phase(w: torch.Tensor, dtype=None) -> torch.Tensor:
    N, Cp = w.shape[0], w.shape[1] // 9
    acc_dt = torch.float32 if w.dtype in DTYPE_CODE else w.dtype
    w9 = w.to(acc_dt).view(N, 3, 3, Cp)
    out = torch.zeros(4, N, 4, Cp, dtype=acc_dt, device=w.device)
    for py in range(2):
        for px in range(2):
            for dy in range(2):
                for dx in range(2):
                    for ky in UPS_PHASE_TAPS[py][dy]:
                        for kx in UPS_PHASE_TAPS[px][dx]:
                            out[2 * py + px, :, 2 * dy + dx] += w9[:, ky, kx]
    return out.to(w.dtype if dtype is None else dtype).contiguous()


def pack_upsample_phase(w: torch.Tensor, dtype=None) -> torch.Tensor:
# ... 491 lines not shown
```

imagdressing_amd/unet.py:

```python
from __future__ import annotations

import math
from types import SimpleNamespace
from typing import Dict, List, Optional

import torch

from . import ops
from .hub import PretrainedMixin

FUSED_LN_CHANNELS = (320, 640, 1280)

bf16 = torch.bfloat16

SD15_CONFIG = dict(
    in_channels=4, out_channels=4, block_out_channels=(320, 640, 1280, 1280), layers_per_block=2,
    attention_head_dim=8, cross_attention_dim=768, norm_num_groups=32, sample_size=64,
    down_attn=(True, True, True, False), time_cond_proj_dim=None,
)


def _resnet_shapes(p, cin, cout, temb):
    s = {f"{p}.norm1.weight": (cin,), f"{p}.norm1.bias": (cin,),
         f"{p}.conv1.weight": (cout, cin, 3, 3), f"{p}.conv1.bias": (cout,),
# ... 163 lines not shown

class Attention:

    def __init__(self, sd, prefix, heads, device, dtype=bf16):
        self.heads = heads
        self.dtype = dtype
        self.to_q = LinearOp(sd[f"{prefix}.to_q.weight"], None, device, dtype)
        self.to_k = LinearOp(sd[f"{prefix}.to_k.weight"], None, device, dtype)
        self.to_v = LinearOp(sd[f"{prefix}.to_v.weight"], None, device, dtype)
        self.to_out = [LinearOp(sd[f"{prefix}.to_out.0.weight"], sd[f"{prefix}.to_out.0.bias"], device, dtype), _Identity()]
        self.query_dim = self.to_q.out_features
        self.is_cross = self.to_k.in_features != self.query_dim
        self.spatial_norm = None
        self.group_norm = None
        self.norm_cross = None
        self.residual_connection = False
        self.rescale_output_factor = 1.0
        self.processor = None

    def prepare_attention_mask(self, mask, *a, **k):
        return mask

    def set_processor(self, p):
        self.processor = p

    def __call__(self, hidden_states, encoder_hidden_states=None, residual=None, layernorm=None, **cross_attention_kwargs):
        proc = self.processor
        if layernorm is not None:
            nrm, eps = layernorm
            if (getattr(proc, "fused_layernorm", False) and getattr(proc, "fused_residual", False) and ops.FUSED_LN
                    and (hidden_states.shape[-1] in FUSED_LN_CHANNELS if encoder_hidden_states is not None
                         else hidden_states.shape[-1] == 320)):
                cross_attention_kwargs = dict(cross_attention_kwargs, imd_layernorm=(nrm.weight, nrm.bias, eps))
            else:
                hidden_states = ops.layer_norm(hidden_states, nrm.weight, nrm.bias, eps)
        if getattr(proc, "fused_residual", False):
            return proc(self, hidden_states, encoder_hidden_states=encoder_hidden_states, attention_mask=None,
                        imd_residual=residual, **cross_attention_kwargs)
        out = proc(self, hidden_states, encoder_hidden_states=encoder_hidden_states, attention_mask=None,
                   **cross_attention_kwargs)
        out = out.to(self.dtype).contiguous()
        return out if residual is None else ops.add(out, residual)


class TransformerBlock:
    def __init__(self, sd, p, ch, heads, device, dtype=bf16):
        self.norm1 = NormParams(sd, f"{p}.norm1", device)
        self.norm2 = NormParams(sd, f"{p}.norm2", device)
        self.norm3 = NormParams(sd, f"{p}.norm3", device)
        self.attn1 = Attention(sd, f"{p}.attn1", heads, device, dtype)
        self.attn2 = Attention(sd, f"{p}.attn2", heads, device, dtype)
        w, b = sd[f"{p}.ff.net.0.proj.weight"], sd[f"{p}.ff.net.0.proj.bias"]
        inner = w.shape[0] // 2
        wi = torch.stack([w[:inner], w[inner:]], dim=1).reshape(2 * inner, w.shape[1])
        bi = torch.stack([b[:inner], b[inner:]], dim=1).reshape(2 * inner)
        self.ff_in = LinearOp(wi, bi, device, dtype)
        self.ff_out = LinearOp(sd[f"{p}.ff.net.2.weight"], sd[f"{p}.ff.net.2.bias"], device, dtype)
        self.ff_fused = None
        if ch == 320 and inner == 4 * ch:
            self.ff_fused = ops.pack_ff_fused(w.to(device), b.to(device), sd[f"{p}.ff.net.2.weight"].to(device),
                                              sd[f"{p}.ff.net.2.bias"].to(device), self.norm3.weight, self.norm3.bias, dtype=dtype)

    def __call__(self, h, ehs, cak):
        h = self.attn1(h, encoder_hidden_states=None, residual=h, layernorm=(self.norm1, 1e-5), **cak)
        return self.after_attn1(h, ehs, cak)

    def after_attn1(self, h, ehs, cak):
        h = self.attn2(h, encoder_hidden_states=ehs, residual=h, layernorm=(self.norm2, 1e-5), **cak)
        B, L, Cc = h.shape
        if self.ff_fused is not None and ops.FUSED_FF and B * L >= ops.FUSED_FF_MIN_ROWS:
            return ops.ff_geglu_fused(h.view(B * L, Cc), self.ff_fused, 1e-5).view(B, L, Cc)
        n = ops.layer_norm(h, self.norm3.weight, self.norm3.bias)
        g = ops.linear(n.view(B * L, Cc), self.ff_in.weight, self.ff_in.bias, act=ops.ACT_GEGLU)
        return ops.linear(g, self.ff_out.weight, self.ff_out.bias, res=h.view(B * L, Cc)).view(B, L, Cc)


class Transformer2D:
    def __init__(self, sd, p, ch, heads, groups, device, dtype=bf16):
        self.norm = NormParams(sd, f"{p}.norm", device)
        self.proj_in = ConvOp(sd[f"{p}.proj_in.weight"], sd[f"{p}.proj_in.bias"], device, dtype)
        self.proj_out = ConvOp(sd[f"{p}.proj_out.weight"], sd[f"{p}.proj_out.bias"], device, dtype)
        self.transformer_blocks = [TransformerBlock(sd, f"{p}.transformer_blocks.0", ch, heads, device, dtype)]
        self.groups = groups

    def __call__(self, x, ehs, cak):
        B, H, W, Cc = x.shape
        h = self.proj_in(x, gn_in=(self.norm.weight, self.norm.bias, 1e-6, False, self.groups)).view(B, H * W, Cc)
        for blk in self.transformer_blocks:
            h = blk(h, ehs, cak)
        return self.proj_out(h.view(B, H, W, Cc), res=x, gn_stats_groups=self.groups)

    def pair_half_ok(self, x_half, cak) -> bool:
        blk = self.transformer_blocks[0]
        proc = blk.attn1.processor
        sa = cak.get("sa_hidden_states")
        Bh, H, W, Cc = x_half.shape
        return bool(cak.get("sa_pair_layout") and cak.get("sa_batch_mask") is not None and sa is not None
                    and getattr(proc, "fused_pair_half", False) and getattr(proc, "fused_residual", False)
                    and getattr(proc, "name", None) in sa and not ops.ATTN_FP8 and not ops.FUSED_OUT_PROJ
                    and ops.attention_dup_supported(blk.attn1.heads, H * W, Cc // blk.attn1.heads))

    def call_pair_half(self, x_half, ehs, cak):
        Bh, H, W, Cc = x_half.shape
        blk = self.transformer_blocks[0]
        h = self.proj_in(x_half, gn_in=(self.norm.weight, self.norm.bias, 1e-6, False, self.groups)).view(Bh, H * W, Cc)
        r = h
        h = blk.attn1(h, encoder_hidden_states=None, residual=r, layernorm=(blk.norm1, 1e-5), imd_pair_half=True, **cak)
        h = blk.after_attn1(h, ehs, cak)
        return self.proj_out(h.view(2 * Bh, H, W, Cc), res=x_half)


def _temb_stride(temb_all):
    return temb_all.shape[1] if temb_all.shape[0] > 1 else 0


class ResnetBlock:
    def __init__(self, sd, p, groups, device, temb_slices: list, dtype=bf16):
        self.norm1 = NormParams(sd, f"{p}.norm1", device)
        self.norm2 = NormParams(sd, f"{p}.norm2", device)
        self.conv1 = ConvOp(sd[f"{p}.conv1.weight"], sd[f"{p}.conv1.bias"], device, dtype)
# ... 345 lines not shown
```

include/imagdressing_hip.h:

```cpp
#ifndef IMAGDRESSING_HIP_H
#define IMAGDRESSING_HIP_H

#include <stdint.h>

#ifdef __cplusplus
extern "C" {
#endif

#define IMD_ABI_VERSION 9

enum { IMD_ACT_NONE = 0, IMD_ACT_SILU = 1, IMD_ACT_GEGLU = 2, IMD_ACT_GELU = 3, IMD_ACT_QUICK_GELU = 4  };
enum { IMD_OUT_ROWMAJOR = 0, IMD_OUT_HEADS = 1 };
enum { IMD_DTYPE_BF16 = 0, IMD_DTYPE_F16 = 1 };

typedef struct imd_heads_dest {
    uint16_t* ptr;
    int kind;
    int DP;
    int L;
    float scale;
} imd_heads_dest;

#define IMD_TUNING_PER_CALL 0x5A000000
#define IMD_TUNING_TAG_MASK 0xFF000000u
// ... 10 lines not shown
    const float* bias;
    const float* rowvec;
    int rowvec_stride;
    const uint16_t* res;
    float out_scale;
    int act;
    int out_f32;
    int mode;
    int hC, hH, hD;
    imd_heads_dest hd[3];
    int dtype;
    int split_k;
    float* splitk_ws;
    uint32_t x_bytes, w_bytes;
    int flags;
    const float* gn_a;
    const float* gn_b;
    int gn_silu;
    int pad_br_only;
    int* splitk_counters;
    float* gn_stats_out;
    int gn_stats_groups;
    const float* gn_in_partial;
    const float* gn_in_gamma;
    const float* gn_in_beta;
    int gn_in_nparts, gn_in_groups, gn_in_silu;
    float gn_in_eps;
    const float* gn_out_gamma;
    const float* gn_out_beta;
    float gn_out_eps;
    int gn_out_silu;
    int gn_out_groups;
    int res_rows;
} imd_conv_gemm_params;
#define IMD_SPLITK_COUNTERS 16384

typedef struct imd_attn_params {
    uint32_t struct_bytes;
    const uint16_t* q;
    const uint16_t* k1;
    const uint16_t* v1t;
    const uint16_t* k2;
    const uint16_t* v2t;
    const float* scale2;
    uint16_t* out;
    int B, H, N, D;
    int L1, L1P, kv1_bdiv;
    int L2, L2P, kv2_bdiv;
    int out_ld;
    int dtype;
    int flags;
    int causal;
    int k_pad_one;
    const uint16_t* proj_w;
    const float* proj_b;
    const uint16_t* proj_res;
    uint16_t* proj_out;
    int proj_res_ld, proj_out_ld;
    int* proj_counters;
    uint16_t* out_dup;
    float* phase2_out;
    int phase2_rows;
} imd_attn_params;

typedef struct imd_ff_params {
    uint32_t struct_bytes;
// ... 69 lines not shown
    uint32_t struct_bytes;
    float* z;
    const float* eps;
    uint16_t* x_next;
    float* hist;
    int B, HW, K;
    int dtype;
    float guidance;
    const float* guidance_rows;
    float m_x, m_e, z_x, z_m;
    float z_h[4];
    float z_n, b_img, b_noise, in_scale;
    int store;
    const float* noise;
    const float* mask;
    const float* z_img;
    const float* blend_noise;
    const float* coefs;
} imd_sampler_params;

int imd_abi_version(void);
const char* imd_last_error(void);
int imd_device_check(int device);

int imd_conv_gemm(const imd_conv_gemm_params* p, int cfg, void* stream);
int imd_conv_gemm_auto_cfg(int M, int N);
int imd_conv_gemm_auto_split(int M, int N, int K, int cfg);

int imd_attention(const imd_attn_params* p, void* stream);
int imd_attention_fp8(const imd_attn_params* p, int eq, int ek, int ev, void* stream);
int imd_attn_quantize_fp8(const uint16_t* src, uint8_t* dst, int kind, long count, int LP, int exp2_scale, float pad_val, int dtype,
                          void* stream);
int imd_row_linear_gn_in_supported(const imd_conv_gemm_params* p, int cfg);
int imd_conv_gemm_gn_out_supported(const imd_conv_gemm_params* p);
int imd_attention_dup_supported(int H, int N, int D);
int imd_attention_phase_split_supported(int D);
int imd_attn_padded_dims(int D, int* dpk, int* dpv);
int imd_set_tuning(int knob, int value);
int imd_get_tuning(int knob);

int imd_groupnorm(const imd_groupnorm_params* p, void* stream);
int imd_groupnorm_workspace_floats(int B, int HW, int C, int G);
int imd_groupnorm_coeffs(const imd_groupnorm_params* p, float* coef_a, float* coef_b, void* stream);
int imd_conv_patch_supported(const imd_conv_gemm_params* p);
int imd_conv_patch2_supported(const imd_conv_gemm_params* p);
int imd_conv_patch3_supported(const imd_conv_gemm_params* p);
int imd_conv_patch4_supported(const imd_conv_gemm_params* p);
int imd_conv_img_supported(const imd_conv_gemm_params* p);
int imd_conv_patch_stats_parts(const imd_conv_gemm_params* p);
int imd_conv_gemm_stats_parts(const imd_conv_gemm_params* p, int cfg);
int imd_gemm_dma_supported(const imd_conv_gemm_params* p);

int imd_row_linear(const imd_conv_gemm_params* p, int ln, float ln_eps, void* stream);
int imd_row_linear_supported(const imd_conv_gemm_params* p);

int imd_ff_geglu(const imd_ff_params* p, void* stream);

int imd_text_xattn320(const imd_xattn_params* p, void* stream);
int imd_text_xattn320_supported(const imd_xattn_params* p);

int imd_conv_ups_phase(const imd_conv_gemm_params* p, void* stream);
int imd_conv_ups_phase_supported(const imd_conv_gemm_params* p);

int imd_layernorm(const imd_layernorm_params* p, void* stream);
int imd_softmax_rows(const float* s, int s_ld, uint16_t* p, int p_ld, int rows, int cols, int dtype, void* stream);

// ... 24 lines not shown
```

Measured before the change: 7.124.

## Fuse LayerNorm into GEMM epilogues via producer-emitted row statistics

```diff
diff --git a/imagdressing_amd/_lib.py b/imagdressing_amd/_lib.py
--- a/imagdressing_amd/_lib.py
+++ b/imagdressing_amd/_lib.py
@@ -41,6 +41,7 @@
         ("gn_in_partial", C.c_void_p), ("gn_in_gamma", C.c_void_p), ("gn_in_beta", C.c_void_p),
         ("gn_in_nparts", C.c_int), ("gn_in_groups", C.c_int), ("gn_in_silu", C.c_int), ("gn_in_eps", C.c_float),
         ("gn_out_gamma", C.c_void_p), ("gn_out_beta", C.c_void_p), ("gn_out_eps", C.c_float), ("gn_out_silu", C.c_int), ("gn_out_groups", C.c_int), ("res_rows", C.c_int),
+        ("ln_stats_out", C.c_void_p), ("ln_rows_partial", C.c_void_p), ("ln_rows_colsum", C.c_void_p), ("ln_rows_groups", C.c_int), ("ln_rows_eps", C.c_float),
     ]
 
 
@@ -138,6 +139,8 @@
     "imd_conv_gemm_stats_parts": (C.c_int, [C.POINTER(ConvGemmParams), C.c_int]),
     "imd_conv_gemm_gn_out_supported": (C.c_int, [C.POINTER(ConvGemmParams)]),
     "imd_row_linear_gn_in_supported": (C.c_int, [C.POINTER(ConvGemmParams), C.c_int]),
+    "imd_ln_stats_out_supported": (C.c_int, [C.POINTER(ConvGemmParams), C.c_int]),
+    "imd_ln_rows_supported": (C.c_int, [C.POINTER(ConvGemmParams), C.c_int]),
     "imd_gemm_dma_supported": (C.c_int, [C.POINTER(ConvGemmParams)]),
     "imd_row_linear": (C.c_int, [C.POINTER(ConvGemmParams), C.c_int, C.c_float, C.c_void_p]),
     "imd_row_linear_supported": (C.c_int, [C.POINTER(ConvGemmParams)]),
diff --git a/imagdressing_amd/adapter/attention_processor.py b/imagdressing_amd/adapter/attention_processor.py
--- a/imagdressing_amd/adapter/attention_processor.py
+++ b/imagdressing_amd/adapter/attention_processor.py
@@ -90,16 +90,26 @@
     return ent[2]
 
 
-def _ln_folded_q(attn, gamma: torch.Tensor, beta: torch.Tensor, dtype, device, which: str = "q"):
+def _ln_folded_q(attn, gamma: torch.Tensor, beta: torch.Tensor, dtype, device, which: str = "q", colsum: bool = False):
     mods = [getattr(attn, n) for n in _W_PARTS[which]]
     srcs = tuple(m.weight for m in mods) + (gamma, beta)
     cache = attn.__dict__.setdefault("_imd_wcache", {})
     key = (_version_key(*srcs), dtype, str(device))
-    ent = cache.get(which + "_ln")
+    slot = which + ("_lnrows" if colsum else "_ln")
+    ent = cache.get(slot)
     if ent is None or ent[0] != key or not all(a is b for a, b in zip(ent[1], srcs)):
         w = torch.cat([m.weight.detach().to(device=device, dtype=dtype) for m in mods], 0)
-        ent = cache[which + "_ln"] = (key, srcs, ops.fold_layernorm_affine(w, None, gamma.to(device), beta.to(device)))
+        ent = cache[slot] = (key, srcs, ops.fold_layernorm_affine(w, None, gamma.to(device), beta.to(device), colsum=colsum))
     return ent[2]
+
+
+def _qkv_ln_rows(attn, x: torch.Tensor, hidden_states: torch.Tensor, imd_layernorm, dt, dev):
+    st = ops.ln_rows_stats(hidden_states) if x is hidden_states else None
+    if st is None or ops.ATTN_FP8:
+        return None
+    g, be, eps = imd_layernorm
+    w2, b2, cs = _ln_folded_q(attn, g, be, dt, dev, "qkv", colsum=True)
+    return (w2, b2, eps), (st, cs, g, be)
 
 
 def _qkv_ln_ok(x: torch.Tensor) -> bool:
@@ -164,7 +174,8 @@
 def _fused_attention(x: torch.Tensor, heads: int, *, wq_or_qkv: torch.Tensor, self_attn: bool,
                      kv1=None, kv1_bdiv: int = 1, kv2=None, kv2_bdiv: int = 1, scale2: Optional[torch.Tensor] = None,
                      wo: torch.Tensor, bo: Optional[torch.Tensor], residual: Optional[torch.Tensor],
-                     q_ln: Optional[tuple] = None, pair_half: bool = False, phase2_rows: int = 0) -> torch.Tensor:
+                     q_ln: Optional[tuple] = None, pair_half: bool = False, phase2_rows: int = 0,
+                     ln_rows: Optional[tuple] = None, out_ln_stats: Optional[str] = None) -> torch.Tensor:
     B, N, Cc = x.shape
     D = Cc // heads
     dpk, dpv = ops.attn_padded_dims(D)
@@ -183,7 +194,13 @@
         k = ops.k_buffer((B, heads, N, dpk), D, dt, dev, tag="attn_k")
         vt = ops.workspace("attn_vt", (B, heads, dpv, LP), dt, dev)
         dests = dict(C=Cc, H=heads, D=D, dests=[(q, 0, dpk, N, qscale), (k, 0, dpk, N, 1.0), (vt, 1, dpv, LP, 1.0)])
-        if q_ln is not None:
+        if ln_rows is not None:
+            r = ops.conv_gemm(x2, q_ln[0], M=B * N, N=3 * Cc, Cin=Cc, Hin=N, Win=1, Hout=N, Wout=1, bias=q_ln[1], heads=dests,
+                              ln_rows=(ln_rows[0], q_ln[2], ln_rows[1]))
+            if r is ops.UNSUPPORTED:
+                xn = ops.layer_norm(x, ln_rows[2], ln_rows[3], q_ln[2])
+                ops.conv_gemm(xn.view(B * N, Cc), wq_or_qkv, M=B * N, N=3 * Cc, Cin=Cc, Hin=N, Win=1, Hout=N, Wout=1, heads=dests)
+        elif q_ln is not None:
             ops.conv_gemm(x2, q_ln[0], M=B * N, N=3 * Cc, Cin=Cc, Hin=N, Win=1, Hout=N, Wout=1, bias=q_ln[1], ln_eps=q_ln[2], heads=dests)
         else:
             ops.conv_gemm(x2, wq_or_qkv, M=B * N, N=3 * Cc, Cin=Cc, Hin=N, Win=1, Hout=N, Wout=1, heads=dests)
@@ -221,7 +238,8 @@
         return ops.linear(o.view(2 * B * N, Cc), wo, bo, res=res2).view(2 * B, N, Cc)
     ops.attention(q, kv1[0], kv1[1], o, B=B, H=heads, N=N, D=D, L1=kv1[2], L1P=kv1[3], kv1_bdiv=kv1_bdiv, k_pad_one=True, phase2_rows=phase2_rows if kw else 0, **kw)
     res2 = None if residual is None else residual.view(B * N, Cc)
-    return ops.linear(o.view(B * N, Cc), wo, bo, res=res2).view(B, N, Cc)
+    y = ops.linear(o.view(B * N, Cc), wo, bo, res=res2, ln_stats=out_ln_stats)
+    return ops.carry_ln_stats(y, y.view(B, N, Cc))
 
 
 class _FusedBase:
@@ -249,28 +267,33 @@
 class AttnProcessor2_0(_FusedBase):
 
     fused_layernorm = True
+    fused_ln_rows = True
+    fused_ln_stats = True
 
     def __init__(self, cache_entries: int = 256):
         self._text = _TensorCache(capacity=cache_entries)
 
     def __call__(self, attn, hidden_states, encoder_hidden_states=None, attention_mask=None, temb=None, scale=1.0,
-                 imd_residual=None, imd_layernorm=None, **kwargs):
+                 imd_residual=None, imd_layernorm=None, imd_ln_stats=None, **kwargs):
         dt = _compute_dtype(attn, hidden_states, attention_mask)
         x, shape4 = _as_tokens(hidden_states, dt)
         dev = x.device
         wo, bo = _layer_weights(attn, "o", dt, dev), _layer_weights(attn, "bo", dt, dev)
-        q_ln = None
+        q_ln = ln_rows = None
         if imd_layernorm is not None:
             g, be, eps = imd_layernorm
+            rows = _qkv_ln_rows(attn, x, hidden_states, imd_layernorm, dt, dev) if encoder_hidden_states is None and not _qkv_ln_ok(x) else None
             if encoder_hidden_states is not None and x.shape[-1] in FUSED_LN_CHANNELS:
                 q_ln = _ln_folded_q(attn, g, be, dt, dev) + (eps,)
             elif encoder_hidden_states is None and _qkv_ln_ok(x):
                 q_ln = _ln_folded_q(attn, g, be, dt, dev, "qkv") + (eps,)
+            elif rows is not None:
+                q_ln, ln_rows = rows
             else:
                 x = ops.layer_norm(x, g, be, eps)
         if encoder_hidden_states is None:
             out = _fused_attention(x, attn.heads, wq_or_qkv=_layer_weights(attn, "qkv", dt, dev), self_attn=True, wo=wo, bo=bo,
-                                   residual=imd_residual, q_ln=q_ln)
+                                   residual=imd_residual, q_ln=q_ln, ln_rows=ln_rows)
         else:
             srcs = (encoder_hidden_states, attn.to_k.weight, attn.to_v.weight)
             kv = self._text.get(srcs, extra=(dt,))
@@ -279,12 +302,13 @@
                 kv = self._text.put(srcs, _project_kv(e, _layer_weights(attn, "kv", dt, dev), attn.heads), extra=(dt,))
             out = _fused_attention(x, attn.heads, wq_or_qkv=_layer_weights(attn, "q", dt, dev), self_attn=False, kv1=kv,
                                    kv1_bdiv=self._ehs_bdiv(x.shape[0], encoder_hidden_states), wo=wo, bo=bo,
-                                   residual=imd_residual, q_ln=q_ln)
+                                   residual=imd_residual, q_ln=q_ln, out_ln_stats=imd_ln_stats if shape4 is None else None)
         return self._finish(attn, out, imd_residual is not None, hidden_states, shape4, ln_fused=imd_layernorm is not None)
 
 
 class CacheAttnProcessor2_0(AttnProcessor2_0):
     fused_layernorm = False
+    fused_ln_rows = False
 
     def __init__(self):
         super().__init__()
@@ -347,6 +371,7 @@
 class RefSAttnProcessor2_0(nn.Module, _FusedBase, _RefMixin):
     fused_layernorm = True
     fused_pair_half = True
+    fused_ln_rows = True
 
     def __init__(self, name, hidden_size, cross_attention_dim=None, scale=1.0):
         super().__init__()
@@ -363,11 +388,14 @@
         dt = _compute_dtype(attn, hidden_states, attention_mask)
         x, shape4 = _as_tokens(hidden_states, dt)
         wqkv, wo, bo = self._weights(attn, dt, x.device)
-        q_ln = None
+        q_ln = ln_rows = None
         if imd_layernorm is not None:
             g, be, eps = imd_layernorm
+            rows = _qkv_ln_rows(attn, x, hidden_states, imd_layernorm, dt, x.device) if type(self) is RefSAttnProcessor2_0 and not _qkv_ln_ok(x) else None
             if _qkv_ln_ok(x):
                 q_ln = _ln_folded_q(attn, g, be, dt, x.device, "qkv") + (eps,)
+            elif rows is not None:
+                q_ln, ln_rows = rows
             else:
                 x = ops.layer_norm(x, g, be, eps)
         kv2 = s2 = None
@@ -382,7 +410,7 @@
             raise ValueError("imd_pair_half needs sa_hidden_states, the block residual and token-major hidden states (engine-internal)")
         pr = x.shape[0] // 2 if (kwargs.get("sa_pair_layout") and sa_batch_mask is not None and kv2 is not None and not imd_pair_half and x.shape[0] % 2 == 0) else 0
         out = _fused_attention(x, attn.heads, wq_or_qkv=wqkv, self_attn=True, kv2=kv2, kv2_bdiv=bdiv2,
-                               scale2=s2, wo=wo, bo=bo, residual=imd_residual, q_ln=q_ln, pair_half=bool(imd_pair_half), phase2_rows=pr)
+                               scale2=s2, wo=wo, bo=bo, residual=imd_residual, q_ln=q_ln, pair_half=bool(imd_pair_half), phase2_rows=pr, ln_rows=ln_rows)
         return self._finish(attn, out, imd_residual is not None, hidden_states, shape4, ln_fused=imd_layernorm is not None)
 
 
@@ -450,11 +478,12 @@
         self._plain = AttnProcessor2_0(cache_entries=4)
 
     fused_layernorm = True
+    fused_ln_stats = True
 
     def __call__(self, attn, hidden_states, encoder_hidden_states=None, attention_mask=None, temb=None, scale=1.0,
-                 cond_hidden_states=None, sa_hidden_states=None, imd_residual=None, imd_layernorm=None, **kwargs):
+                 cond_hidden_states=None, sa_hidden_states=None, imd_residual=None, imd_layernorm=None, imd_ln_stats=None, **kwargs):
         return self._plain(attn, hidden_states, encoder_hidden_states=encoder_hidden_states, imd_residual=imd_residual,
-                           imd_layernorm=imd_layernorm)
+                           imd_layernorm=imd_layernorm, imd_ln_stats=imd_ln_stats)
 
 
 class _IPBase(nn.Module, _FusedBase, _LoraFold):
diff --git a/imagdressing_amd/csrc/capi.cpp b/imagdressing_amd/csrc/capi.cpp
--- a/imagdressing_amd/csrc/capi.cpp
+++ b/imagdressing_amd/csrc/capi.cpp
@@ -190,6 +190,8 @@
 int imd_conv_patch_stats_parts(const imd_conv_gemm_params* p) { return sized(p) ? imd_conv_patch_stats_parts_of(*p) : 0; }
 int imd_conv_gemm_stats_parts(const imd_conv_gemm_params* p, int cfg) { return sized(p) ? imd_conv_gemm_stats_parts_of(*p, cfg) : 0; }
 int imd_row_linear_gn_in_supported(const imd_conv_gemm_params* p, int cfg) { return (sized(p) && p->gn_in_partial != nullptr && imd_row_linear_gn_in_supported_of(*p, cfg)) ? 1 : 0; }
+int imd_ln_stats_out_supported(const imd_conv_gemm_params* p, int cfg) { return (sized(p) && p->ln_stats_out != nullptr && imd_ln_stats_out_supported_of(*p, cfg)) ? 1 : 0; }
+int imd_ln_rows_supported(const imd_conv_gemm_params* p, int cfg) { return (sized(p) && p->ln_rows_partial != nullptr && imd_ln_rows_supported_of(*p, cfg)) ? 1 : 0; }
 int imd_conv_gemm_gn_out_supported(const imd_conv_gemm_params* p) { return (sized(p) && imd_conv_gemm_gn_out_supported_of(*p, -1)) ? 1 : 0; }
 int imd_gemm_dma_supported(const imd_conv_gemm_params* p) { return query(p, static_cast<bool (*)(const imd_conv_gemm_params&)>(imd_gemm_dma_supported)); }
 
@@ -207,6 +209,8 @@
         IMD_REQUIRE(!p->out_f32, "row_linear: head-split output excludes fp32 output");
     }
     IMD_REQUIRE(!ln || ln_eps > 0.f, "row_linear: LayerNorm needs eps > 0");
+    IMD_REQUIRE(p->ln_rows_partial == nullptr, "row_linear: the row-resident projections have no ln_rows_* instantiation (tile configs 16 / 30 / 31 have one)");
+    IMD_REQUIRE(p->ln_stats_out == nullptr || ((p->K == 640 || p->K == 1280) && !ln), "row_linear: ln_stats_out exists in the K = 640 / 1280 projections without a LayerNorm prologue only");
     if (p->K == 320 && p->N == 960 && p->mode == IMD_OUT_HEADS) {
         IMD_REQUIRE(p->gn_in_partial == nullptr, "row_linear: the fused q / k / v projection has no GroupNorm prologue (gn_in_*)");
         return imd_launch_row_qkv(*p, ln, ln_eps, (hipStream_t)stream);
@@ -241,6 +245,7 @@
     IMD_REQUIRE(p != nullptr, "conv_ups_phase: null params");
     IMD_REQUIRE_SIZE(p, "conv_ups_phase");
     IMD_REQUIRE(p->x && p->w && p->out, "conv_ups_phase: null input / weight / output pointer");
+    IMD_REQUIRE(p->ln_stats_out == nullptr && p->ln_rows_partial == nullptr, "conv_ups_phase: no LayerNorm statistics / fold (ln_stats_out, ln_rows_*)");
     return imd_launch_conv_ups_phase(*p, (hipStream_t)stream);
 }
 
diff --git a/imagdressing_amd/csrc/conv_gemm.hip b/imagdressing_amd/csrc/conv_gemm.hip
--- a/imagdressing_amd/csrc/conv_gemm.hip
+++ b/imagdressing_amd/csrc/conv_gemm.hip
@@ -624,6 +624,25 @@
     }
 }
 
+bool imd_ln_stats_out_supported_of(const ConvGemmParams& p, int cfg) {
+    if (p.ln_stats_out == nullptr) return true;
+    ConvGemmParams q = p;
+    q.split_k = 1;
+    if (p.split_k > 1 || p.res_rows != 0 || !ln_stats_out_ok(q)) return false;
+    switch (cfg) {
+        case 13: return imd_row_linear_k640_supported(q) && gn_in_ok(q, 640, 128);
+        case 14: return imd_row_linear_k1280_supported(q) && gn_in_ok(q, 1280, 64);
+        default: return false;
+    }
+}
+
+bool imd_ln_rows_supported_of(const ConvGemmParams& p, int cfg) {
+    if (p.ln_rows_partial == nullptr) return true;
+    ConvGemmParams q = p;
+    if (q.split_k < 1) q.split_k = 1;
+    return (cfg == 16 || cfg == 30 || cfg == 31) && ln_rows_ok(q) && imd_gemm_dma_supported(q);
+}
+
 bool imd_conv_gemm_gn_out_supported_of(const ConvGemmParams& p_in, int cfg) {
     ConvGemmParams p = p_in;
     (void)cfg;
@@ -722,6 +741,13 @@
     if (p.gn_in_partial != nullptr && !imd_row_linear_gn_in_supported_of(p, cfg))
         return imd_set_error("conv_gemm: gn_in_* (GroupNorm of the input rows) exists in the row-resident projections only (tile configs 12 / 13 / 14 with H W a multiple of "
                              "their row block; got cfg=%d K=%d HW=%d): ask imd_row_linear_gn_in_supported() first", cfg, p.K, p.Hout * p.Wout);
+    if (p.ln_stats_out != nullptr && !imd_ln_stats_out_supported_of(p, cfg))
+        return imd_set_error("conv_gemm: ln_stats_out (LayerNorm statistics of the output rows) exists in the K = 640 / 1280 row-resident projections only (tile configs 13 / 14, "
+                             "row-major 16-bit output; got cfg=%d K=%d N=%d): ask imd_ln_stats_out_supported() first", cfg, p.K, p.N);
+    if (p.ln_rows_partial != nullptr && !imd_ln_rows_supported_of(p, cfg))
+        return imd_set_error("conv_gemm: ln_rows_* (LayerNorm of the input rows folded into the epilogue) needs tile config 16 / 30 / 31, K = 640 / 1280 with K / 160 records per row, "
+                             "column sums, eps > 0 and an epilogue without residual / per-batch vector / K slices / fp32 output (got cfg=%d K=%d groups=%d): ask imd_ln_rows_supported() first",
+                             cfg, p.K, p.ln_rows_groups);
     if (t == nullptr) return imd_set_error("conv_gemm: unknown tile config %d", cfg);
     if (t->taps != 0 && t->taps != p.taps) return imd_set_error("conv_gemm: tile config %d does not take taps = %d", cfg, p.taps);
     if (t->slices_only && p.split_k <= 1) return imd_set_error("conv_gemm: tile config %d writes K-slice slabs only (split_k >= 2)", cfg);
diff --git a/imagdressing_amd/csrc/gemm_common.h b/imagdressing_amd/csrc/gemm_common.h
--- a/imagdressing_amd/csrc/gemm_common.h
+++ b/imagdressing_amd/csrc/gemm_common.h
@@ -148,6 +148,62 @@
            p.gn_in_nparts > 0 && p.gn_in_nparts <= 4096 && HW > 0 && (HW % rows) == 0 && (p.M % HW) == 0 && p.K == K;
 }
 
+constexpr int LN_GROUP_N = 160;
+
+template <int G>
+__device__ __forceinline__ float2 ln_chan_combine(const float2* r, float n_each) {
+    float ms = 0.f, m2 = 0.f;
+#pragma unroll
+    for (int g = 0; g < G; ++g) { ms += r[g].x; m2 += r[g].y; }
+    const float mean = ms * (1.0f / G);
+    float dev = 0.f;
+#pragma unroll
+    for (int g = 0; g < G; ++g) { const float d = r[g].x - mean; dev = fmaf(d, d, dev); }
+    return make_float2(mean, fmaf(n_each, dev, m2));
+}
+
+__device__ __forceinline__ float2 ln_shifted_finish(float shift, float sd, float sq, float n) {
+    const float dm = sd * (1.0f / n);
+    return make_float2(shift + dm, fmaxf(fmaf(-sd, dm, sq), 0.f));
+}
+
+struct LnRowsReq { float4 q[4]; };
+__device__ __forceinline__ void ln_rows_request(const ConvGemmParams& p, int m, bool live, LnRowsReq& r) {
+    const float4* rec = reinterpret_cast<const float4*>(p.ln_rows_partial + (size_t)m * p.ln_rows_groups * 2);
+    const bool wide = p.ln_rows_groups == 8;
+#pragma unroll
+    for (int i = 0; i < 4; ++i) r.q[i] = (live && (i < 2 || wide)) ? rec[i] : make_float4(0, 0, 0, 0);
+}
+__device__ __forceinline__ float2 ln_rows_mean_rstd(const ConvGemmParams& p, const LnRowsReq& r) {
+    float2 rec[8];
+#pragma unroll
+    for (int i = 0; i < 4; ++i) { rec[2 * i] = make_float2(r.q[i].x, r.q[i].y); rec[2 * i + 1] = make_float2(r.q[i].z, r.q[i].w); }
+    const float2 t = p.ln_rows_groups == 8 ? ln_chan_combine<8>(rec, (float)LN_GROUP_N) : ln_chan_combine<4>(rec, (float)LN_GROUP_N);
+    return make_float2(t.x, rsqrtf(t.y / (float)p.K + p.ln_rows_eps));
+}
+__device__ __forceinline__ float ln_rows_fold(float v, float mean, float rstd, float s) { return rstd * (v - mean * s); }
+
+__device__ __forceinline__ void ln_rows_fold8(const ConvGemmParams& p, float* v, int m, int n, int nv) {
+    LnRowsReq r;
+    ln_rows_request(p, m, true, r);
+    const float4 s0 = *reinterpret_cast<const float4*>(p.ln_rows_colsum + n);
+    const float4 s1 = nv == 8 ? *reinterpret_cast<const float4*>(p.ln_rows_colsum + n + 4) : make_float4(0, 0, 0, 0);
+    const float2 mr = ln_rows_mean_rstd(p, r);
+    const float sv[8] = {s0.x, s0.y, s0.z, s0.w, s1.x, s1.y, s1.z, s1.w};
+#pragma unroll
+    for (int e = 0; e < 8; ++e) v[e] = ln_rows_fold(v[e], mr.x, mr.y, sv[e]);
+}
+
+inline bool ln_rows_ok(const ConvGemmParams& p) {
+    if (p.ln_rows_partial == nullptr) return true;
+    return (p.K == 640 || p.K == 1280) && p.taps == 1 && p.Cin == p.K && p.ln_rows_groups == p.K / LN_GROUP_N && p.ln_rows_colsum != nullptr && p.ln_rows_eps > 0.f &&
+           p.res == nullptr && p.rowvec == nullptr && p.split_k <= 1 && !p.out_f32 && (p.act == ACT_NONE || p.act == ACT_GEGLU) && (p.N % 8) == 0 &&
+           p.gn_a == nullptr && p.gn_in_partial == nullptr && p.gn_stats_out == nullptr && p.gn_out_gamma == nullptr && p.ln_stats_out == nullptr;
+}
+inline bool ln_stats_out_ok(const ConvGemmParams& p) {
+    return p.ln_stats_out == nullptr || (p.mode == OUT_ROWMAJOR && !p.out_f32 && p.act == ACT_NONE && (p.N % LN_GROUP_N) == 0 && p.ln_rows_partial == nullptr);
+}
+
 __device__ __forceinline__ void load_col_addends(const ConvGemmParams& p, int bi, int n, int nv, float4& a0, float4& a1) {
     a0 = make_float4(0, 0, 0, 0); a1 = a0;
     const bool full = nv == 8;
@@ -163,12 +219,13 @@
     }
 }
 
-template <bool F16>
+template <bool F16, bool LNR = false>
 __device__ __forceinline__ void epilogue8(const ConvGemmParams& p, float* v, int m, int n, int nv, int HWo, bool use_pre = false,
                                           float4 pre0 = float4{0, 0, 0, 0}, float4 pre1 = float4{0, 0, 0, 0}, bool use_rpre = false,
                                           uint4 rpre = uint4{0, 0, 0, 0}, uint4* pk_out = nullptr) {
     using E = El<F16>;
     const int bi = m / HWo;
+    if constexpr (LNR) ln_rows_fold8(p, v, m, n, nv);
     float4 b0 = make_float4(0, 0, 0, 0), b1 = b0, r0 = b0, r1 = b0;
     uint4 rr = make_uint4(0, 0, 0, 0);
     const bool full = nv == 8;
diff --git a/imagdressing_amd/csrc/gemm_dma.hip b/imagdressing_amd/csrc/gemm_dma.hip
--- a/imagdressing_amd/csrc/gemm_dma.hip
+++ b/imagdressing_amd/csrc/gemm_dma.hip
@@ -9,7 +9,7 @@
 constexpr int GD_LDS = 2 * GD_STAGE;
 constexpr int GD_CLD = GD_BN + 4, GD_EROWS = 64;
 
-template <bool F16>
+template <bool F16, bool LNR = false>
 __global__ __launch_bounds__(512, 1) void gemm_dma_kernel(const ConvGemmParams p) {
     using E = El<F16>;
     extern __shared__ __attribute__((aligned(16))) char smem[];
@@ -121,7 +121,7 @@
             const float4 v0 = *reinterpret_cast<const float4*>(Cs + row * GD_CLD + cc);
             const float4 v1 = *reinterpret_cast<const float4*>(Cs + row * GD_CLD + cc + 4);
             float v[8] = {v0.x, v0.y, v0.z, v0.w, v1.x, v1.y, v1.z, v1.w};
-            epilogue8<F16>(p, v, m, n, (n + 8 <= p.N) ? 8 : 4, HWo, use_col_pre, col_pre0, col_pre1);
+            epilogue8<F16, LNR>(p, v, m, n, (n + 8 <= p.N) ? 8 : 4, HWo, use_col_pre, col_pre0, col_pre1);
         }
         if (wr + 1 < 4) __syncthreads();
     }
@@ -322,6 +322,7 @@
 }
 
 int imd_launch_gemm_dma128(const ConvGemmParams& p, int stages, int bk, hipStream_t s) {
+    if (p.ln_rows_partial != nullptr) return imd_set_error("gemm_dma128: no ln_rows_* instantiation (tile configs 16 / 30 / 31 have one)");
     if (!((bk == 32 && (stages == 3 || stages == 4)) || (bk == 64 && (stages == 2 || stages == 3))))
         return imd_set_error("gemm_dma128: %d ring stages of %d-element K chunks (3 | 4 of 32, 2 | 3 of 64)", stages, bk);
     if (bk == 64) {
@@ -351,11 +352,12 @@
 
 int imd_launch_gemm_dma(const ConvGemmParams& p, hipStream_t s) {
     if (!imd_gemm_dma_supported(p)) return imd_set_error("gemm_dma: needs a plain linear layer with K %% 64 == 0 and no K split (got K=%d taps=%d split=%d)", p.K, p.taps, p.split_k);
-    const bool h = p.dtype == IMD_DTYPE_F16;
-    const void* kern = h ? reinterpret_cast<const void*>(gemm_dma_kernel<true>) : reinterpret_cast<const void*>(gemm_dma_kernel<false>);
-    if (int rc_attr = imd_lds_attr(kern, GD_LDS, "gemm_dma")) return rc_attr;
+    if (!ln_rows_ok(p)) return imd_set_error("gemm_dma: ln_rows_* needs K = 640 / 1280 with K / 160 records per row, column sums, eps > 0 and a bias-only epilogue (ask imd_ln_rows_supported())");
+    const bool h = p.dtype == IMD_DTYPE_F16, lnr = p.ln_rows_partial != nullptr;
+    typedef void (*kern_t)(const ConvGemmParams);
+    const kern_t kern = lnr ? (h ? gemm_dma_kernel<true, true> : gemm_dma_kernel<false, true>) : (h ? gemm_dma_kernel<true> : gemm_dma_kernel<false>);
+    if (int rc_attr = imd_lds_attr(reinterpret_cast<const void*>(kern), GD_LDS, "gemm_dma")) return rc_attr;
     const long mt = (p.M + GD_BM - 1) / GD_BM, nt = (p.N + GD_BN - 1) / GD_BN;
-    if (h) hipLaunchKernelGGL(gemm_dma_kernel<true>, dim3((unsigned)(mt * nt)), dim3(512), GD_LDS, s, p);
-    else hipLaunchKernelGGL(gemm_dma_kernel<false>, dim3((unsigned)(mt * nt)), dim3(512), GD_LDS, s, p);
+    hipLaunchKernelGGL(kern, dim3((unsigned)(mt * nt)), dim3(512), GD_LDS, s, p);
     return imd_check_launch("gemm_dma");
 }
diff --git a/imagdressing_amd/csrc/gemm_dma256.hip b/imagdressing_amd/csrc/gemm_dma256.hip
--- a/imagdressing_amd/csrc/gemm_dma256.hip
+++ b/imagdressing_amd/csrc/gemm_dma256.hip
@@ -33,10 +33,11 @@
 
 
 template <int BM> struct G2Waves { static constexpr int NCW = BM / 32, NPROD = BM == 192 ? 4 : BM / 64; };
-template <bool F16, int BM, int BN, int NST, bool PRE, bool RES>
+template <bool F16, int BM, int BN, int NST, bool PRE, bool RES, bool LNR = false>
 __global__ __launch_bounds__((G2Waves<BM>::NCW + G2Waves<BM>::NPROD) * 64, 3) void gemm_dma256_kernel
 (const ConvGemmParams p) {
     using E = El<F16>;
+    static_assert(!LNR || (PRE && !RES), "the LayerNorm fold rides on the prefetching epilogue without a residual");
     constexpr int NCW = G2Waves<BM>::NCW, G2_NPROD = G2Waves<BM>::NPROD;
     constexpr int G2_A = BM * G2_ROWB;
     constexpr int APIECES = BM / 8;
@@ -169,8 +170,19 @@
             slot = slot == NST - 1 ? 0 : slot + 1;
             if (!abl_nowait) __syncthreads();
         };
+        LnRowsReq lnq;
+        float ln_mean[2] = {0.f, 0.f}, ln_rstd[2] = {0.f, 0.f};
+        float4 cs_l = make_float4(0, 0, 0, 0);
+        if constexpr (LNR) ln_rows_request(p, ci.m0 + wm0 + lane, ci.m0 + wm0 + lane < p.M, lnq);
 #pragma unroll 1
         for (int kt = 0; kt < ci.nk - 1; ++kt) step();
+        if constexpr (LNR) {
+            const float2 mr = ln_rows_mean_rstd(p, lnq);
+#pragma unroll
+            for (int b = 0; b < 2; ++b) { ln_mean[b] = __shfl(mr.x, b * 32 + col); ln_rstd[b] = __shfl(mr.y, b * 32 + col); }
+            const int nb = ci.n0 + wn0 + 4 * lane;
+            if (lane < 16 && nb < p.N) cs_l = *reinterpret_cast<const float4*>(p.ln_rows_colsum + nb);
+        }
         float4 bn[NA][4];
         uint4 rp[NA][2], rq[NA][2];
         auto load_bias = [&]() __attribute__((always_inline)) {
@@ -204,6 +216,22 @@
             float* slab = (p.split_k > 1) ? p.splitk_ws + (size_t)ci.slice * p.M * p.N : nullptr;
             if (pre_ok) {
                 float* bias_s = reinterpret_cast<float*>(smem + NST * STAGE + wave * 2048);
+                if constexpr (LNR) {
+                    if (lane < 16) *reinterpret_cast<float4*>(bias_s + 4 * lane) = cs_l;
+#pragma unroll
+                    for (int a = 0; a < NA; ++a)
+#pragma unroll
+                        for (int j = 0; j < 4; ++j) {
+                            const float4 sj = *reinterpret_cast<const float4*>(bias_s + a * 32 + 8 * j + 4 * hi);
+#pragma unroll
+                            for (int b = 0; b < 2; ++b) {
+                                acc[a][b][4 * j] = ln_rows_fold(acc[a][b][4 * j], ln_mean[b], ln_rstd[b], sj.x);
+                                acc[a][b][4 * j + 1] = ln_rows_fold(acc[a][b][4 * j + 1], ln_mean[b], ln_rstd[b], sj.y);
+                                acc[a][b][4 * j + 2] = ln_rows_fold(acc[a][b][4 * j + 2], ln_mean[b], ln_rstd[b], sj.z);
+                                acc[a][b][4 * j + 3] = ln_rows_fold(acc[a][b][4 * j + 3], ln_mean[b], ln_rstd[b], sj.w);
+                            }
+                        }
+                }
                 if (RES && lane < 16) *reinterpret_cast<float4*>(bias_s + 4 * lane) = bias_l;
 #pragma unroll
                 for (int a = 0; a < NA; ++a)
@@ -344,14 +372,14 @@
     }
 }
 
-template <int BM, int BN, int NST, bool PRE, bool RES>
+template <int BM, int BN, int NST, bool PRE, bool RES, bool LNR = false>
 int launch_dma256_v(const ConvGemmParams& p, bool persistent, hipStream_t s, const char* what) {
     constexpr int LDS = NST * (BM + BN) * G2_ROWB + (BM / 32) * 2048;
     constexpr int WG_PER_CU = BM >= 192 ? 1 : 2;
     static_assert(LDS * WG_PER_CU <= 160 * 1024, "ring + transpose areas must fit the CU's LDS");
     const bool h = p.dtype == IMD_DTYPE_F16;
     typedef void (*kern_t)(const ConvGemmParams);
-    const kern_t kern = h ? gemm_dma256_kernel<true, BM, BN, NST, PRE, RES> : gemm_dma256_kernel<false, BM, BN, NST, PRE, RES>;
+    const kern_t kern = h ? gemm_dma256_kernel<true, BM, BN, NST, PRE, RES, LNR> : gemm_dma256_kernel<false, BM, BN, NST, PRE, RES, LNR>;
     if (int rc_attr = imd_lds_attr(reinterpret_cast<const void*>(kern), LDS, what)) return rc_attr;
     const int n_cu = imd_cu_count8();
     if (n_cu < 0) return imd_set_error("%s: cannot query the device", what);
@@ -365,6 +393,12 @@
 template <int BM, int BN, int NST>
 int launch_dma256(const ConvGemmParams& p, bool persistent, hipStream_t s, const char* what) {
     const bool pre = p.rowvec == nullptr && p.split_k <= 1, res = p.res != nullptr;
+    if (p.ln_rows_partial != nullptr) {
+        if constexpr (BM == 256) {
+            if (!ln_rows_ok(p) || !pre || res) return imd_set_error("%s: ln_rows_* needs K = 640 / 1280 with K / 160 records per row, column sums, eps > 0 and a bias-only epilogue (ask imd_ln_rows_supported())", what);
+            return launch_dma256_v<BM, BN, NST, true, false, true>(p, persistent, s, what);
+        } else return imd_set_error("%s: no ln_rows_* instantiation (tile configs 16 / 30 / 31 have one)", what);
+    }
     if (!pre || (res && (p.mode != OUT_ROWMAJOR || p.out_f32 || p.act == ACT_GEGLU || (p.N % BN) != 0 || (p.res_ld % 8) != 0 || (p.out_ld % 8) != 0)))
         return launch_dma256_v<BM, BN, NST, false, false>(p, persistent, s, what);
     return res ? launch_dma256_v<BM, BN, NST, true, true>(p, persistent, s, what) : launch_dma256_v<BM, BN, NST, true, false>(p, persistent, s, what);
diff --git a/imagdressing_amd/csrc/imd_kernels.h b/imagdressing_amd/csrc/imd_kernels.h
--- a/imagdressing_amd/csrc/imd_kernels.h
+++ b/imagdressing_amd/csrc/imd_kernels.h
@@ -43,6 +43,8 @@
 int imd_conv_gemm_stats_parts_of(const ConvGemmParams& p, int cfg);
 bool imd_conv_gemm_gn_out_supported_of(const ConvGemmParams& p, int cfg);
 bool imd_row_linear_gn_in_supported_of(const ConvGemmParams& p, int cfg);
+bool imd_ln_stats_out_supported_of(const ConvGemmParams& p, int cfg);
+bool imd_ln_rows_supported_of(const ConvGemmParams& p, int cfg);
 int imd_launch_conv_patch(const ConvGemmParams& p, hipStream_t s);
 bool imd_row_linear_supported(const ConvGemmParams& p);
 int imd_launch_row_linear(const ConvGemmParams& p, int ln, float ln_eps, hipStream_t s);
diff --git a/imagdressing_amd/csrc/row_linear_k1280.hip b/imagdressing_amd/csrc/row_linear_k1280.hip
--- a/imagdressing_amd/csrc/row_linear_k1280.hip
+++ b/imagdressing_amd/csrc/row_linear_k1280.hip
@@ -27,7 +27,7 @@
     }
 };
 
-template <bool F16, bool LN, bool GN = false>
+template <bool F16, bool LN, bool GN = false, bool ST = false>
 __global__ __launch_bounds__(512, 1) void row_linear_k1280_kernel(const ConvGemmParams p, const float ln_eps) {
     static_assert(!(LN && GN), "one prologue at a time");
     using E = El<F16>;
@@ -189,6 +189,7 @@
     const float osc = heads ? p.out_scale * p.hd[0].scale : p.out_scale;
     f32x4 own;
     own[0] = own[1] = own[2] = own[3] = 0.f;
+    float st_shift = 0.f, st_sd = 0.f, st_sq = 0.f;
     auto emit = [&](int c) {
         float4 t = make_float4(own[0], own[1], own[2], own[3]);
 #pragma unroll
@@ -211,6 +212,12 @@
         typedef __attribute__((__vector_size__(2 * sizeof(uint32_t)))) uint32_t v2u;
         const v2u pk = {E::pack2(v0, v1), E::pack2(v2, v3)};
         __builtin_amdgcn_raw_buffer_store_b64(pk, rs_o, (int)(obase == OOB ? OOB : obase + off), 0, 0);
+        if constexpr (ST) {
+            const float r[4] = {E::lo(pk[0]), E::hi(pk[0]), E::lo(pk[1]), E::hi(pk[1])};
+            if (c == 0) st_shift = r[0];
+#pragma unroll
+            for (int e = 0; e < 4; ++e) { const float d = r[e] - st_shift; st_sd += d; st_sq = fmaf(d, d, st_sq); }
+        }
     };
 
     const uint32_t pb = (uint32_t)(kq * 40 + g), sw = (uint32_t)col;
@@ -239,11 +246,21 @@
             }
         }
     }
-}
-
-template <bool F16, bool LN, bool GN = false>
+    if constexpr (ST) {
+        if (owner) {
+            const float2 mine = ln_shifted_finish(st_shift, st_sd, st_sq, (float)(R12_NG / 4));
+            float2 r[4];
+#pragma unroll
+            for (int k = 0; k < 4; ++k) r[k] = make_float2(__shfl(mine.x, col + 16 * k), __shfl(mine.y, col + 16 * k));
+            const float2 rec = ln_chan_combine<4>(r, (float)(R12_NG / 4));
+            if (g == 0 && mo < p.M) reinterpret_cast<float2*>(p.ln_stats_out)[(size_t)mo * n_groups + grp] = rec;
+        }
+    }
+}
+
+template <bool F16, bool LN, bool GN = false, bool ST = false>
 int launch_r12(const ConvGemmParams& p, float eps, hipStream_t s) {
-    auto kern = row_linear_k1280_kernel<F16, LN, GN>;
+    auto kern = row_linear_k1280_kernel<F16, LN, GN, ST>;
     if (int rc_attr = imd_lds_attr(reinterpret_cast<const void*>(kern), R12_LDS, "row_linear_k1280")) return rc_attr;
     const unsigned grid = (unsigned)((((p.M + 63) / 64 + 7) / 8) * 8 * (p.N / R12_NG));
     hipLaunchKernelGGL(kern, dim3(grid), dim3(512), R12_LDS, s, p, eps);
@@ -276,11 +293,17 @@
     p.split_k = 1;
     p.flags = 0;
     const bool h = p.dtype == IMD_DTYPE_F16;
+    if (p.ln_rows_partial != nullptr) return imd_set_error("row_linear_k1280: no ln_rows_* instantiation (tile configs 16 / 30 / 31 have one)");
+    const bool st = p.ln_stats_out != nullptr;
+    if (st && (ln || !ln_stats_out_ok(p)))
+        return imd_set_error("row_linear_k1280: ln_stats_out needs a row-major 16-bit output and no LayerNorm prologue (ask imd_ln_stats_out_supported())");
     if (p.gn_in_partial != nullptr) {
         if (ln || !gn_in_ok(p, R12_K, 64))
             return imd_set_error("row_linear_k1280: gn_in_* needs K = 1280, K %% groups == 0, groups <= 64, H W %% 64 == 0 and no LayerNorm prologue (ask imd_row_linear_gn_in_supported())");
+        if (st) return h ? launch_r12<true, false, true, true>(p, ln_eps, s) : launch_r12<false, false, true, true>(p, ln_eps, s);
         return h ? launch_r12<true, false, true>(p, ln_eps, s) : launch_r12<false, false, true>(p, ln_eps, s);
     }
+    if (st) return h ? launch_r12<true, false, false, true>(p, ln_eps, s) : launch_r12<false, false, false, true>(p, ln_eps, s);
     if (ln) return h ? launch_r12<true, true>(p, ln_eps, s) : launch_r12<false, true>(p, ln_eps, s);
     return h ? launch_r12<true, false>(p, ln_eps, s) : launch_r12<false, false>(p, ln_eps, s);
 }
diff --git a/imagdressing_amd/csrc/row_linear_k640.hip b/imagdressing_amd/csrc/row_linear_k640.hip
--- a/imagdressing_amd/csrc/row_linear_k640.hip
+++ b/imagdressing_amd/csrc/row_linear_k640.hip
@@ -15,9 +15,10 @@
 constexpr int R6_OFF_LN = R6_OFF_BIAS + R6_NG * 4;
 constexpr int R6_LDS = R6_OFF_LN + 8 * 64 * 8;
 
-template <bool F16, bool LN, bool GN = false>
+template <bool F16, bool LN, bool GN = false, bool ST = false>
 __global__ __launch_bounds__(512, 1) void row_linear_k640_kernel(const ConvGemmParams p, const float ln_eps) {
     static_assert(!(LN && GN), "one prologue at a time");
+    static_assert(!(LN && ST), "the statistic records share the LayerNorm-partial area");
     using E = El<F16>;
     extern __shared__ __attribute__((aligned(16))) char smem[];
     const int tid = threadIdx.x;
@@ -140,6 +141,7 @@
     const float* bias_s = reinterpret_cast<const float*>(smem + R6_OFF_BIAS);
     const float osc = heads ? p.out_scale * p.hd[0].scale : p.out_scale;
     float own[8];
+    float st_shift = 0.f, st_sd = 0.f, st_sq = 0.f;
     auto emit = [&](int c) {
         typedef __attribute__((__vector_size__(2 * sizeof(uint32_t)))) uint32_t v2u;
         typedef __attribute__((__vector_size__(4 * sizeof(uint32_t)))) uint32_t v4u_t;
@@ -166,6 +168,12 @@
                 v2 += E::lo(rres[j].y); v3 += E::hi(rres[j].y);
             }
             pk[j] = v2u{E::pack2(v0, v1), E::pack2(v2, v3)};
+            if constexpr (ST) {
+                const float r[4] = {E::lo(pk[j][0]), E::hi(pk[j][0]), E::lo(pk[j][1]), E::hi(pk[j][1])};
+                if (c == 0 && j == 0) st_shift = r[0];
+#pragma unroll
+                for (int e = 0; e < 4; ++e) { const float d = r[e] - st_shift; st_sd += d; st_sq = fmaf(d, d, st_sq); }
+            }
         }
         auto offset_of = [&](int n) -> uint32_t {
             if (heads) { const int h = n / p.hD, dd = n - h * p.hD; return (uint32_t)((h * p.hd[0].L * p.hd[0].DP + dd) * 2); }
@@ -212,11 +220,21 @@
             }
         }
     }
-}
-
-template <bool F16, bool LN, bool GN = false>
+    if constexpr (ST) {
+        float2* lnx = reinterpret_cast<float2*>(smem + R6_OFF_LN);
+        lnx[wave * 64 + lane] = ln_shifted_finish(st_shift, st_sd, st_sq, (float)(R6_NG / 4));
+        __syncthreads();
+        if (tid < 128 && m0 + tid < p.M) {
+            const int w0 = tid >> 5, l0 = tid & 31;
+            const float2 r[4] = {lnx[w0 * 64 + l0], lnx[w0 * 64 + l0 + 32], lnx[(w0 + 4) * 64 + l0], lnx[(w0 + 4) * 64 + l0 + 32]};
+            reinterpret_cast<float2*>(p.ln_stats_out)[(size_t)(m0 + tid) * n_groups + grp] = ln_chan_combine<4>(r, (float)(R6_NG / 4));
+        }
+    }
+}
+
+template <bool F16, bool LN, bool GN = false, bool ST = false>
 int launch_r6(const ConvGemmParams& p, float eps, hipStream_t s) {
-    auto kern = row_linear_k640_kernel<F16, LN, GN>;
+    auto kern = row_linear_k640_kernel<F16, LN, GN, ST>;
     if (int rc_attr = imd_lds_attr(reinterpret_cast<const void*>(kern), R6_LDS, "row_linear_k640")) return rc_attr;
     const unsigned grid = (unsigned)((((p.M + 127) / 128 + 7) / 8) * 8 * (p.N / R6_NG));
     hipLaunchKernelGGL(kern, dim3(grid), dim3(512), R6_LDS, s, p, eps);
@@ -249,11 +267,17 @@
     p.split_k = 1;
     p.flags = (g_gemm_flags & 1024) ? 0 : 1024;
     const bool h = p.dtype == IMD_DTYPE_F16;
+    if (p.ln_rows_partial != nullptr) return imd_set_error("row_linear_k640: no ln_rows_* instantiation (tile configs 16 / 30 / 31 have one)");
+    const bool st = p.ln_stats_out != nullptr;
+    if (st && (ln || !ln_stats_out_ok(p)))
+        return imd_set_error("row_linear_k640: ln_stats_out needs a row-major 16-bit output and no LayerNorm prologue (ask imd_ln_stats_out_supported())");
     if (p.gn_in_partial != nullptr) {
         if (ln || !gn_in_ok(p, R6_K, 128))
             return imd_set_error("row_linear_k640: gn_in_* needs K = 640, K %% groups == 0, groups <= 64, H W %% 128 == 0 and no LayerNorm prologue (ask imd_row_linear_gn_in_supported())");
+        if (st) return h ? launch_r6<true, false, true, true>(p, ln_eps, s) : launch_r6<false, false, true, true>(p, ln_eps, s);
         return h ? launch_r6<true, false, true>(p, ln_eps, s) : launch_r6<false, false, true>(p, ln_eps, s);
     }
+    if (st) return h ? launch_r6<true, false, false, true>(p, ln_eps, s) : launch_r6<false, false, false, true>(p, ln_eps, s);
     if (ln) return h ? launch_r6<true, true>(p, ln_eps, s) : launch_r6<false, true>(p, ln_eps, s);
     return h ? launch_r6<true, false>(p, ln_eps, s) : launch_r6<false, false>(p, ln_eps, s);
 }
diff --git a/imagdressing_amd/ops.py b/imagdressing_amd/ops.py
--- a/imagdressing_amd/ops.py
+++ b/imagdressing_amd/ops.py
@@ -139,6 +139,12 @@
 TEMB_TABLE = _os.environ.get("IMD_TEMB_TABLE", "1") != "0"
 FUSED_GN_PROJ_CFGS = tuple(int(c) for c in _os.environ.get("IMD_FUSED_GN_PROJ_CFGS", "12,13,14").split(",") if c)
 CFG_PAIR_ATTN = _os.environ.get("IMD_CFG_PAIR_ATTN", "1") != "0"
+FUSED_LN_ROWS = _os.environ.get("IMD_FUSED_LN_ROWS", "0") == "1"
+FUSED_LN_ROWS_CFGS = tuple(int(c) for c in _os.environ.get("IMD_FUSED_LN_ROWS_CFGS", "16,30,31").split(",") if c)
+LN_STATS_CFGS = (13, 14)
+LN_ROWS_CHANNELS = (640, 1280)
+LN_GROUP_N = 160
+UNSUPPORTED = object()
 FUSED_LN = True
 GEMM_TRACE = None
 GEMM_EVENT_HOOK = None
@@ -341,7 +347,7 @@
     rowvec_off: int = 0, res: Optional[torch.Tensor] = None, res_ld: Optional[int] = None, out_scale: float = 1.0,
     act: int = ACT_NONE, out_f32: bool = False, heads: Optional[dict] = None, cfg: int = -1, split_k: int = 0,
     gn: Optional[tuple] = None, pad_br_only: bool = False, ln_eps: Optional[float] = None, gn_stats_groups: int = 0,
-    gn_out: Optional[tuple] = None, gn_in: Optional[tuple] = None,
+    gn_out: Optional[tuple] = None, gn_in: Optional[tuple] = None, ln_stats: Optional[str] = None, ln_rows: Optional[tuple] = None,
 ) -> Optional[torch.Tensor]:
     ensure_device(x.device)
     K = taps * Cin
@@ -379,6 +385,14 @@
     if res_rows:
         res = _periodic_residual(p, res, res_rows, cfg in PERIODIC_RES_CFGS)
     p.split_k = split_k
+    if ln_rows is not None:
+        part, eps_rows, colsum = ln_rows
+        if part.dim() != 3 or part.shape[0] != M or part.shape[2] != 2 or colsum.numel() != N:
+            raise L.ImdError(f"conv_gemm: ln_rows records {tuple(part.shape)} / column sums {tuple(colsum.shape)} do not fit M = {M}, N = {N}")
+        p.ln_rows_partial, p.ln_rows_colsum = _dev(part, torch.float32, "ln_rows records"), _dev(colsum, torch.float32, "ln_rows column sums")
+        p.ln_rows_groups, p.ln_rows_eps = int(part.shape[1]), float(eps_rows)
+        if cfg not in FUSED_LN_ROWS_CFGS or not lib.imd_ln_rows_supported(C.byref(p), cfg):
+            return UNSUPPORTED
     xn = None if gn_in is None else _fuse_gn_in(p, lib, x, gn_in, cfg, M, Hout * Wout)
     if split_k > 1:
         p.splitk_ws = splitk_workspace(split_k * M * N, x.device).data_ptr()
@@ -391,6 +405,12 @@
     stats = None
     if gn_stats_groups and FUSED_GN_STATS and heads is None and not out_f32 and act != ACT_GEGLU:
         stats = _attach_stats(p, lib, cfg, split_k, gn_stats_groups, M // (Hout * Wout), x.device)
+    ln_st = None
+    if ln_stats is not None and FUSED_LN_ROWS and cfg in LN_STATS_CFGS and heads is None and N % LN_GROUP_N == 0:
+        ln_st = workspace("ln_stats_" + ln_stats, (M, N // LN_GROUP_N, 2), torch.float32, x.device)
+        p.ln_stats_out = ln_st.data_ptr()
+        if not lib.imd_ln_stats_out_supported(C.byref(p), cfg):
+            p.ln_stats_out, ln_st = None, None
     if GEMM_EVENT_HOOK is not None:
         e0, e1 = torch.cuda.Event(enable_timing=True), torch.cuda.Event(enable_timing=True)
         e0.record()
@@ -401,6 +421,8 @@
         L.check(lib.imd_conv_gemm(C.byref(p), cfg, _stream()))
     if stats is not None:
         out._imd_gn_stats = stats
+    if ln_st is not None:
+        out._imd_ln_stats = ln_st
     return out
 
 
@@ -427,20 +449,36 @@
 
 
 def linear(x2d: torch.Tensor, w: torch.Tensor, bias=None, *, res=None, act=ACT_NONE, out_f32=False, out=None,
-           out_ld=None, res_ld=None, cfg=-1, split_k=0, ln_eps=None) -> torch.Tensor:
+           out_ld=None, res_ld=None, cfg=-1, split_k=0, ln_eps=None, ln_stats=None, ln_rows=None) -> torch.Tensor:
     M, K = x2d.shape
     N = w.shape[0]
     return conv_gemm(x2d, w, M=M, N=N, Cin=K, bias=bias, res=res, act=act, out_f32=out_f32, out=out,
-                     out_ld=out_ld, res_ld=res_ld, cfg=cfg, split_k=split_k, ln_eps=ln_eps)
-
-
-def fold_layernorm_affine(w: torch.Tensor, bias: Optional[torch.Tensor], gamma: torch.Tensor, beta: torch.Tensor):
+                     out_ld=out_ld, res_ld=res_ld, cfg=cfg, split_k=split_k, ln_eps=ln_eps, ln_stats=ln_stats, ln_rows=ln_rows)
+
+
+def fold_layernorm_affine(w: torch.Tensor, bias: Optional[torch.Tensor], gamma: torch.Tensor, beta: torch.Tensor, colsum: bool = False):
     wf = w.float()
     w2 = (wf * gamma.float()[None, :]).to(w.dtype).contiguous()
     b2 = wf @ beta.float()
     if bias is not None:
         b2 = b2 + bias.float()
+    if colsum:
+        return w2, b2.contiguous(), w2.float().sum(dim=1).contiguous()
     return w2, b2.contiguous()
+
+
+def ln_rows_stats(x: torch.Tensor):
+    st = getattr(x, "_imd_ln_stats", None)
+    if st is None or not FUSED_LN_ROWS or x.shape[-1] not in LN_ROWS_CHANNELS:
+        return None
+    return st if st.shape[0] * x.shape[-1] == x.numel() and st.shape[1] * LN_GROUP_N == x.shape[-1] else None
+
+
+def carry_ln_stats(src: torch.Tensor, dst: torch.Tensor) -> torch.Tensor:
+    st = getattr(src, "_imd_ln_stats", None)
+    if st is not None:
+        dst._imd_ln_stats = st
+    return dst
 
 
 def pack_ff_fused(w1: torch.Tensor, b1: torch.Tensor, w2: torch.Tensor, b2: torch.Tensor, gamma: Optional[torch.Tensor] = None,
@@ -613,7 +651,7 @@
 
 def conv2d_nhwc(x: torch.Tensor, w: torch.Tensor, bias=None, *, taps=9, stride=1, ups=False, rowvec=None,
                 rowvec_stride=0, rowvec_off=0, res=None, out_scale=1.0, act=ACT_NONE, out_f32=False, cfg=-1, split_k=0, gn=None,
-                pad_br_only=False, gn_stats_groups=0, gn_out=None, gn_in=None) -> torch.Tensor:
+                pad_br_only=False, gn_stats_groups=0, gn_out=None, gn_in=None, ln_stats=None) -> torch.Tensor:
     B, H, W, Cin = x.shape
     Cout = w.shape[0]
     Hl, Wl = (2 * H, 2 * W) if ups else (H, W)
@@ -621,8 +659,8 @@
     M = B * Ho * Wo
     out = conv_gemm(x, w, M=M, N=Cout, Cin=Cin, taps=taps, Hin=H, Win=W, Hout=Ho, Wout=Wo, stride=stride, ups=ups,
                     bias=bias, rowvec=rowvec, rowvec_stride=rowvec_stride, rowvec_off=rowvec_off, res=res, out_scale=out_scale, act=act,
-                    out_f32=out_f32, cfg=cfg, split_k=split_k, gn=gn, pad_br_only=pad_br_only, gn_stats_groups=gn_stats_groups, gn_out=gn_out, gn_in=gn_in)
-    r = out.view(B, Ho, Wo, -1)
+                    out_f32=out_f32, cfg=cfg, split_k=split_k, gn=gn, pad_br_only=pad_br_only, gn_stats_groups=gn_stats_groups, gn_out=gn_out, gn_in=gn_in, ln_stats=ln_stats)
+    r = carry_ln_stats(out, out.view(B, Ho, Wo, -1))
     if getattr(out, "_imd_gn_applied", False):
         r._imd_gn_applied = True
     st = getattr(out, "_imd_gn_stats", None)
diff --git a/imagdressing_amd/unet.py b/imagdressing_amd/unet.py
--- a/imagdressing_amd/unet.py
+++ b/imagdressing_amd/unet.py
@@ -219,6 +219,9 @@
                     and (hidden_states.shape[-1] in FUSED_LN_CHANNELS if encoder_hidden_states is not None
                          else hidden_states.shape[-1] == 320)):
                 cross_attention_kwargs = dict(cross_attention_kwargs, imd_layernorm=(nrm.weight, nrm.bias, eps))
+            elif (encoder_hidden_states is None and getattr(proc, "fused_ln_rows", False) and getattr(proc, "fused_residual", False)
+                  and not ops.ATTN_FP8 and ops.ln_rows_stats(hidden_states) is not None):
+                cross_attention_kwargs = dict(cross_attention_kwargs, imd_layernorm=(nrm.weight, nrm.bias, eps))
             else:
                 hidden_states = ops.layer_norm(hidden_states, nrm.weight, nrm.bias, eps)
         if getattr(proc, "fused_residual", False):
@@ -243,6 +246,7 @@
         bi = torch.stack([b[:inner], b[inner:]], dim=1).reshape(2 * inner)
         self.ff_in = LinearOp(wi, bi, device, dtype)
         self.ff_out = LinearOp(sd[f"{p}.ff.net.2.weight"], sd[f"{p}.ff.net.2.bias"], device, dtype)
+        self._ff_in_ln = None
         self.ff_fused = None
         if ch == 320 and inner == 4 * ch:
             self.ff_fused = ops.pack_ff_fused(w.to(device), b.to(device), sd[f"{p}.ff.net.2.weight"].to(device),
@@ -252,13 +256,25 @@
         h = self.attn1(h, encoder_hidden_states=None, residual=h, layernorm=(self.norm1, 1e-5), **cak)
         return self.after_attn1(h, ehs, cak)
 
+    def _ff_in_folded(self):
+        if self._ff_in_ln is None:
+            self._ff_in_ln = ops.fold_layernorm_affine(self.ff_in.weight, self.ff_in.bias, self.norm3.weight, self.norm3.bias, colsum=True)
+        return self._ff_in_ln
+
     def after_attn1(self, h, ehs, cak):
-        h = self.attn2(h, encoder_hidden_states=ehs, residual=h, layernorm=(self.norm2, 1e-5), **cak)
+        want = ops.FUSED_LN_ROWS and h.shape[-1] in ops.LN_ROWS_CHANNELS and getattr(self.attn2.processor, "fused_ln_stats", False) and not ops.ATTN_FP8
+        h = self.attn2(h, encoder_hidden_states=ehs, residual=h, layernorm=(self.norm2, 1e-5), **(dict(cak, imd_ln_stats="norm3") if want else cak))
         B, L, Cc = h.shape
         if self.ff_fused is not None and ops.FUSED_FF and B * L >= ops.FUSED_FF_MIN_ROWS:
             return ops.ff_geglu_fused(h.view(B * L, Cc), self.ff_fused, 1e-5).view(B, L, Cc)
-        n = ops.layer_norm(h, self.norm3.weight, self.norm3.bias)
-        g = ops.linear(n.view(B * L, Cc), self.ff_in.weight, self.ff_in.bias, act=ops.ACT_GEGLU)
+        st = ops.ln_rows_stats(h) if want else None
+        g = ops.UNSUPPORTED
+        if st is not None:
+            w2, b2, cs = self._ff_in_folded()
+            g = ops.linear(h.view(B * L, Cc), w2, b2, act=ops.ACT_GEGLU, ln_rows=(st, 1e-5, cs))
+        if g is ops.UNSUPPORTED:
+            n = ops.layer_norm(h, self.norm3.weight, self.norm3.bias)
+            g = ops.linear(n.view(B * L, Cc), self.ff_in.weight, self.ff_in.bias, act=ops.ACT_GEGLU)
         return ops.linear(g, self.ff_out.weight, self.ff_out.bias, res=h.view(B * L, Cc)).view(B, L, Cc)
 
 
@@ -272,7 +288,9 @@
 
     def __call__(self, x, ehs, cak):
         B, H, W, Cc = x.shape
-        h = self.proj_in(x, gn_in=(self.norm.weight, self.norm.bias, 1e-6, False, self.groups)).view(B, H * W, Cc)
+        want = ops.FUSED_LN_ROWS and Cc in ops.LN_ROWS_CHANNELS and getattr(self.transformer_blocks[0].attn1.processor, "fused_ln_rows", False) and not ops.ATTN_FP8
+        h = self.proj_in(x, gn_in=(self.norm.weight, self.norm.bias, 1e-6, False, self.groups), **({"ln_stats": "norm1"} if want else {}))
+        h = ops.carry_ln_stats(h, h.view(B, H * W, Cc))
         for blk in self.transformer_blocks:
             h = blk(h, ehs, cak)
         return self.proj_out(h.view(B, H, W, Cc), res=x, gn_stats_groups=self.groups)
diff --git a/include/imagdressing_hip.h b/include/imagdressing_hip.h
--- a/include/imagdressing_hip.h
+++ b/include/imagdressing_hip.h
@@ -66,6 +66,11 @@
     int gn_out_silu;
     int gn_out_groups;
     int res_rows;
+    float* ln_stats_out;
+    const float* ln_rows_partial;
+    const float* ln_rows_colsum;
+    int ln_rows_groups;
+    float ln_rows_eps;
 } imd_conv_gemm_params;
 #define IMD_SPLITK_COUNTERS 16384
 
@@ -201,6 +206,8 @@
 int imd_attn_quantize_fp8(const uint16_t* src, uint8_t* dst, int kind, long count, int LP, int exp2_scale, float pad_val, int dtype,
                           void* stream);
 int imd_row_linear_gn_in_supported(const imd_conv_gemm_params* p, int cfg);
+int imd_ln_stats_out_supported(const imd_conv_gemm_params* p, int cfg);
+int imd_ln_rows_supported(const imd_conv_gemm_params* p, int cfg);
 int imd_conv_gemm_gn_out_supported(const imd_conv_gemm_params* p);
 int imd_attention_dup_supported(int H, int N, int D);
 int imd_attention_phase_split_supported(int D);
```

After: 7.131, median of 2. Within noise of the previous version (+0.1%).
